# SinOncology/BreakID

Measured on AMD Instinct MI355X. Metric: M reads/s clustered+split-scanned, higher is better.
Workload: dtype int32/u8 (+f64 sd replay)

## Files before the change

### breakid_amd/abi.py

```python
import ctypes as C

import numpy as np

BK_OK = 0
BK_ERR_ARG, BK_ERR_HIP, BK_ERR_NO_DEVICE, BK_ERR_UNSORTED, BK_ERR_CIGAR, BK_ERR_IO, BK_ERR_LIMIT, BK_ERR_COLLISION = -1, -2, -3, -4, -5, -6, -7, -8
BK_MEM_HOST, BK_MEM_DEVICE = 0, 1
STAGE_SCAN, STAGE_ISO, STAGE_CLUSTERED, STAGE_SPLITS, STAGE_CLUSTERS, STAGE_GROUP_KEYS = range(6)

PAIR = np.dtype([("x", "<u4"), ("y", "<u4"), ("p1_pos", "<u4"), ("p2_pos", "<u4"), ("p1_tid", "<i4"),
                 ("p2_tid", "<i4"), ("p1_flag", "<u2"), ("p2_flag", "<u2"), ("p1_mapq", "u1"), ("p2_mapq", "u1"),
                 ("p1_rev", "u1"), ("p2_rev", "u1"), ("rec", "<u8"), ("id", "<u4"), ("cluster", "<i4"),
                 ("group", "<u4"), ("reserved", "<u4")])
SPLIT = np.dtype([("rec", "<u8"), ("tid", "<i4"), ("pos", "<i4"), ("endpos", "<i4"), ("reserved", "<u4"), ("qhash", "<u8"),
                  ("prim_chr", "<i4"), ("sec_chr", "<i4"), ("prim_start", "<u4"), ("prim_end", "<u4"),
                  ("prim_bp", "<u4"), ("sec_start", "<u4"), ("sec_end", "<u4"), ("sec_bp", "<u4"),
                  ("prim_cigar", "<u8"), ("sec_cigar", "<u8"), ("flags", "<u4"), ("qcheck", "<u4")])
CLUSTER = np.dtype([("group", "<u4"), ("id", "<i4"), ("p1_tid", "<i4"), ("p2_tid", "<i4"), ("p1_mean", "<u4"),
                    ("p2_mean", "<u4"), ("p1_min", "<u4"), ("p1_max", "<u4"), ("p2_min", "<u4"), ("p2_max", "<u4"),
                    ("p1_exact", "<u4"), ("p2_exact", "<i4"), ("n_drp", "<u4"), ("n_sr", "<u4"), ("depth1", "<u4"),
                    ("depth2", "<u4"), ("type_mask", "<u4"), ("flags", "<u4")])
GROUP_KEY = np.dtype([("p1_tid", "<i4"), ("p2_tid", "<i4")])
NORMAL_SUPPORT = np.dtype([("n_drp", "<u4"), ("n_sr", "<u4"), ("depth1", "<u4"), ("depth2", "<u4")])
REF_SUPPORT = np.dtype([("ref_pairs1", "<u4"), ("ref_pairs2", "<u4"), ("ref_reads1", "<u4"), ("ref_reads2", "<u4")])
JUNCTION = np.dtype([("pairs", "<u4", (4,)), ("splits", "<u4", (4,)), ("mapq_sum1", "<u8"), ("mapq_sum2", "<u8")])
assert JUNCTION.itemsize == 48
CLIP_LEFT, CLIP_RIGHT = 0, 1
CLIP_SUPPORT = np.dtype([("at", "<u4", (2, 2)), ("peak_pos", "<u4", (2, 2)), ("peak_n", "<u4", (2, 2)), ("events", "<u4", (2, 2))])
assert CLIP_SUPPORT.itemsize == 64
EV_PAIR, EV_SPLIT = 1, 2
EVIDENCE = np.dtype([("rec", "<u8"), ("qhash", "<u8"), ("qcheck", "<u4"), ("call", "<u4"), ("tid1", "<i4"), ("pos1", "<u4"), ("tid2", "<i4"),
                     ("pos2", "<u4"), ("flag1", "<u2"), ("flag2", "<u2"), ("mapq1", "u1"), ("mapq2", "u1"), ("kind", "u1"), ("sides", "u1")])
READ_KEY = np.dtype([("qhash", "<u8"), ("qcheck", "<u4"), ("tag", "<u4")])
assert EVIDENCE.itemsize == 48 and READ_KEY.itemsize == 16
assert PAIR.itemsize == 56 and SPLIT.itemsize == 88 and CLUSTER.itemsize == 72 and NORMAL_SUPPORT.itemsize == 16 and REF_SUPPORT.itemsize == 16

STAGE_DTYPE = {STAGE_SCAN: PAIR, STAGE_ISO: PAIR, STAGE_CLUSTERED: PAIR, STAGE_SPLITS: SPLIT,
               STAGE_CLUSTERS: CLUSTER, STAGE_GROUP_KEYS: GROUP_KEY}


class Soa(C.Structure):
    _fields_ = [("n", C.c_uint64), ("tid", C.c_void_p), ("pos", C.c_void_p), ("mtid", C.c_void_p),
                ("mpos", C.c_void_p), ("isize", C.c_void_p), ("flag", C.c_void_p), ("mapq", C.c_void_p),
                ("qhash", C.c_void_p), ("cigar_off", C.c_void_p), ("cigar", C.c_void_p),
                ("aux_off", C.c_void_p), ("aux", C.c_void_p), ("n_cigar_words", C.c_uint64),
                ("n_aux_bytes", C.c_uint64), ("qcheck", C.c_void_p), ("side", C.c_void_p)]


class Regions(C.Structure):
    _fields_ = [("tid", C.c_void_p), ("beg", C.c_void_p), ("end", C.c_void_p), ("n", C.c_uint64)]


SOA_COLS = [("tid", np.int32), ("pos", np.int32), ("mtid", np.int32), ("mpos", np.int32), ("isize", np.int32),
            ("flag", np.uint16), ("mapq", np.uint8), ("qhash", np.uint64), ("cigar_off", np.uint32),
            ("cigar", np.uint32), ("aux_off", np.uint32), ("aux", np.uint8)]


SOA_COLS_ALL = SOA_COLS + [("qcheck", np.uint32)]


def soa_from_numpy(cols) -> Soa:
    s = Soa()
    s.n = len(cols["tid"])
    for name, dt in SOA_COLS:
        a = cols[name]
        assert a.dtype == dt and a.flags["C_CONTIGUOUS"], name
        setattr(s, name, a.ctypes.data if a.size else 0)
    assert len(cols["cigar_off"]) == s.n + 1 and len(cols["aux_off"]) == s.n + 1
    s.n_cigar_words = int(cols["cigar_off"][-1]) if s.n else 0
    s.n_aux_bytes = int(cols["aux_off"][-1]) if s.n else 0
    q = cols.get("qcheck")
    if q is not None and s.n:
        assert q.dtype == np.uint32 and q.flags["C_CONTIGUOUS"] and len(q) == s.n
        s.qcheck = q.ctypes.data
    return s


def fetch_array(lib, handle, fn, stage):
    data = C.c_void_p()
    count = C.c_uint64()
    goff = C.POINTER(C.c_uint64)()
    ng = C.c_uint32()
    rc = fn(handle, stage, C.byref(data), C.byref(count), C.byref(goff), C.byref(ng))
    if rc != 0:
        raise RuntimeError("fetch(stage=%d) failed rc=%d" % (stage, rc))
    dt = STAGE_DTYPE[stage]
    n = count.value
    if n:
        buf = (C.c_char * (n * dt.itemsize)).from_address(data.value)
        arr = np.frombuffer(buf, dtype=dt, count=n).copy()
    else:
        arr = np.zeros(0, dt)
    off = None
    if ng.value or bool(goff):
        off = np.ctypeslib.as_array(goff, shape=(ng.value + 1,)).copy() if bool(goff) else None
    return arr, off


class ShardStats(C.Structure):
    _fields_ = [("isize_sum", C.c_uint64), ("isize_n", C.c_uint64), ("sumsq", C.c_double), ("vmax", C.c_uint32),
                ("max_span", C.c_uint32), ("n_cand", C.c_uint64), ("n_split", C.c_uint64)]


BUF_CANDIDATES, BUF_TUPLES, BUF_CLUSTERS = 0, 1, 2


def device_ptrs(cols):
    p = {k: cols[k].data_ptr() for k, _ in SOA_COLS}
    if "qcheck" in cols:
        p["qcheck"] = cols["qcheck"].data_ptr()
    if "side" in cols:
        p["side"] = cols["side"].data_ptr()
    return p
```

### breakid_amd/capi.py

```python
from __future__ import annotations

import ctypes as C
import math
import os
import subprocess

import numpy as np

from . import abi

_HERE = os.path.dirname(os.path.abspath(__file__))
LIB_PATH = os.path.join(_HERE, "libbreakid_hip.so")
_LIB = None


class BreakIDError(RuntimeError):
    def __init__(self, code, msg):
        super().__init__("libbreakid_hip error %d: %s" % (code, msg))
        self.code = code


def build(verbose=False):
    cmd = ["make", "-C", os.path.join(_HERE, "csrc"), "-j8"]
    r = subprocess.run(cmd, capture_output=not verbose, text=True)
    if r.returncode != 0:
        raise RuntimeError("building libbreakid_hip.so failed:\n" + (r.stdout or "")[-4000:] + (r.stderr or "")[-4000:])


EXPORTS = ["bk_init", "bk_prepare_process", "bk_free", "bk_last_error", "bk_set_stream", "bk_sync", "bk_get_stream", "bk_upload_records", "bk_exclude_regions", "bk_isize_stats",
           "bk_discordant_pairs", "bk_mask_and_cluster", "bk_split_evidence", "bk_cluster_summary",
           "bk_split_breakpoints", "bk_normal_support", "bk_ref_support", "bk_genotype_call", "bk_clip_support", "bk_base_depth", "bk_clip_rescue", "bk_junctions", "bk_junction_sides", "bk_vcf_breakend_alt", "bk_evidence", "bk_run", "bk_fetch", "bk_timing", "bk_timing_enable", "bk_timing_touched", "bk_group_stats", "bk_qname_hash", "bk_qname_check",
           "bk_bam_open", "bk_bam_header", "bk_bam_decode", "bk_bam_close", "bk_bam_extract", "bk_bam_names_free", "bk_bam_decode_device", "bk_bam_decode_device_part", "bk_bam_decode_device_ctx", "bk_bam_dev_free", "bk_feed_release_caches", "bk_debug_bgzf_inflate", "bk_debug_std_sort", "bk_sort_forms", "bk_debug_ahc", "bk_debug_points", "bk_debug_cigar", "bk_debug_vote", "bk_debug_region", "bk_shard_begin", "bk_shard_get_stats", "bk_shard_set_stats",
           "bk_shard_sd_local", "bk_shard_sd_finish", "bk_shard_buffer", "bk_shard_set_buffer", "bk_shard_group_sizes",
           "bk_shard_own_groups", "bk_shard_route_candidates", "bk_shard_group_keys", "bk_shard_route_pairs", "bk_shard_group_pairs", "bk_shard_bp_cov", "bk_shard_bp_vote", "bk_shard_bp_vote_slice", "bk_shard_bp_set_voted", "bk_shard_bp_depth", "bk_shard_bp_finish"]


def lib():
    global _LIB
    if _LIB is None:
        if not os.path.exists(LIB_PATH):
            raise BreakIDError(abi.BK_ERR_NO_DEVICE, "libbreakid_hip.so is not built (run __graft_entry__.build()); "
                                                     "there is no CPU fallback")
        try:
            import torch
        except Exception:
            pass
        L = C.CDLL(LIB_PATH)
        vp, u64p, dp = C.c_void_p, C.POINTER(C.c_uint64), C.POINTER(C.c_double)
        L.bk_init.argtypes = [C.c_int, vp, C.POINTER(C.c_char_p), C.c_int, C.POINTER(vp)]
        L.bk_free.argtypes = [vp]
        L.bk_last_error.restype = C.c_char_p
        L.bk_last_error.argtypes = [vp]
        L.bk_set_stream.argtypes = [vp, vp]
        L.bk_sync.argtypes = [vp]
        L.bk_upload_records.argtypes = [vp, C.POINTER(abi.Soa), C.c_int]
        L.bk_exclude_regions.argtypes = [vp, C.POINTER(abi.Regions), u64p]
        L.bk_isize_stats.argtypes = [vp, dp, dp]
        L.bk_discordant_pairs.argtypes = [vp, C.c_int, C.c_double, u64p, C.POINTER(C.c_uint32)]
        L.bk_mask_and_cluster.argtypes = [vp, C.c_double, C.c_int, u64p]
        L.bk_split_evidence.argtypes = [vp, u64p]
        L.bk_cluster_summary.argtypes = [vp, C.c_double, u64p]
        L.bk_split_breakpoints.argtypes = [vp, C.c_double, u64p]
        L.bk_run.argtypes = [vp, C.c_int, C.c_int, dp, u64p]
        L.bk_normal_support.argtypes = [vp, vp, C.c_double, C.POINTER(vp), u64p]
        L.bk_ref_support.argtypes = [vp, vp, C.c_int, C.c_int, C.c_double, C.POINTER(vp), u64p]
        L.bk_genotype_call.argtypes = [C.c_uint32, C.c_uint32, C.POINTER(C.c_uint8), C.POINTER(C.c_uint8), C.POINTER(C.c_float)]
        L.bk_clip_support.argtypes = [vp, vp, C.c_int, C.c_int, C.c_double, C.POINTER(vp), u64p]
        L.bk_base_depth.argtypes = [vp, vp, vp, C.c_uint64, C.POINTER(vp)]
        L.bk_clip_rescue.argtypes = [vp, vp, vp, C.c_uint32] + [C.POINTER(C.c_uint32)] * 4
        L.bk_junctions.argtypes = [vp, C.POINTER(vp), u64p]
        L.bk_junction_sides.argtypes = [vp, C.POINTER(C.c_uint8), C.POINTER(C.c_uint8), C.POINTER(C.c_uint8)]
        L.bk_vcf_breakend_alt.argtypes = [C.c_char, C.c_int, C.c_char_p, C.c_uint32, C.c_int, C.c_char_p, C.c_size_t]
        L.bk_evidence.argtypes = [vp, C.POINTER(vp), u64p, C.POINTER(C.POINTER(C.c_uint64))]
        L.bk_fetch.argtypes = [vp, C.c_int, C.POINTER(vp), u64p, C.POINTER(C.POINTER(C.c_uint64)), C.POINTER(C.c_uint32)]
        L.bk_timing.argtypes = [vp, C.POINTER(C.POINTER(C.c_char_p)), C.POINTER(C.POINTER(C.c_float)),
                                C.POINTER(C.POINTER(C.c_uint64)), C.POINTER(C.c_int)]
        L.bk_timing_enable.argtypes = [vp, C.c_int]
        L.bk_timing_touched.argtypes = [vp, C.POINTER(C.POINTER(C.c_uint64)), C.POINTER(C.c_int)]
        L.bk_debug_std_sort.argtypes = [vp, vp, vp, C.c_uint32, vp]
        L.bk_sort_forms.argtypes = [vp, u64p]
        L.bk_debug_ahc.argtypes = [vp, vp, vp, C.c_uint32, C.c_double, vp, vp, C.POINTER(C.c_uint32)]
        L.bk_debug_points.argtypes = [vp, C.c_int, vp, vp, C.c_uint32, C.c_double, vp, vp, C.POINTER(C.c_uint32)]
        L.bk_debug_cigar.argtypes = [vp, C.c_uint32, vp, vp, vp, vp, vp, vp, vp]
        L.bk_debug_vote.argtypes = [vp, vp, C.c_uint32, vp, C.c_uint32, C.c_int32, C.c_int32, vp]
        L.bk_debug_region.argtypes = [vp, C.c_int32, C.c_uint32, C.c_uint32, C.c_uint64, vp, C.c_uint32, C.POINTER(C.c_uint32), C.POINTER(C.c_uint32),
                                      C.POINTER(C.c_uint32)]
        L.bk_shard_begin.argtypes = [vp, C.c_uint64, C.c_int]
        L.bk_shard_get_stats.argtypes = [vp, C.POINTER(abi.ShardStats)]
        L.bk_shard_set_stats.argtypes = [vp, C.POINTER(abi.ShardStats)]
        L.bk_shard_sd_local.argtypes = [vp, u64p, C.POINTER(vp), u64p]
        L.bk_shard_sd_finish.argtypes = [vp, vp, C.c_uint64, C.c_uint64, dp, dp]
        L.bk_shard_buffer.argtypes = [vp, C.c_int, C.POINTER(vp), u64p, C.POINTER(C.c_uint32)]
        L.bk_shard_set_buffer.argtypes = [vp, C.c_int, vp, C.c_uint64]
        L.bk_shard_group_sizes.argtypes = [vp, C.POINTER(C.POINTER(C.c_uint64)), C.POINTER(C.c_uint32)]
        L.bk_shard_own_groups.argtypes = [vp, vp, C.c_uint32]
        L.bk_shard_route_candidates.argtypes = [vp, C.c_uint32, C.POINTER(vp), C.POINTER(C.POINTER(C.c_uint64))]
        L.bk_shard_group_keys.argtypes = [vp, C.POINTER(C.POINTER(C.c_uint32)), C.POINTER(C.c_uint32)]
        L.bk_shard_route_pairs.argtypes = [vp, vp, C.c_uint32, C.c_uint32, C.POINTER(vp), C.POINTER(C.POINTER(C.c_uint64))]
        L.bk_shard_group_pairs.argtypes = [vp, vp, C.c_uint64, vp, C.c_uint32]
        L.bk_shard_bp_cov.argtypes = [vp, C.c_double, C.POINTER(vp), u64p]
        L.bk_shard_bp_vote.argtypes = [vp, C.c_double, vp]
        L.bk_shard_bp_vote_slice.argtypes = [vp, C.c_double, vp, C.c_uint64, C.c_uint64, C.POINTER(vp), C.POINTER(vp)]
        L.bk_shard_bp_set_voted.argtypes = [vp, vp]
        L.bk_shard_bp_depth.argtypes = [vp, C.POINTER(vp), u64p]
        L.bk_shard_bp_finish.argtypes = [vp, vp]
        L.bk_qname_hash.restype = C.c_uint64
        L.bk_qname_hash.argtypes = [C.c_char_p, C.c_size_t]
        L.bk_qname_check.restype = C.c_uint32
        L.bk_qname_check.argtypes = [C.c_char_p, C.c_size_t]
        L.bk_bam_open.argtypes = [C.c_char_p, C.POINTER(vp), C.c_char_p, C.c_size_t]
        L.bk_bam_header.argtypes = [vp, C.POINTER(C.c_int), C.POINTER(C.POINTER(C.c_char_p)), C.POINTER(C.POINTER(C.c_uint32))]
        L.bk_bam_decode.argtypes = [vp, C.POINTER(abi.Soa), C.c_char_p, C.c_size_t]
        L.bk_bam_close.argtypes = [vp]
        L.bk_bam_extract.argtypes = [C.c_char_p, C.c_char_p, vp, C.c_uint64, C.POINTER(C.c_char_p), C.c_uint64, C.POINTER(vp), u64p, C.c_char_p, C.c_size_t]
        L.bk_bam_names_free.argtypes = [vp]
        L.bk_bam_names_free.restype = None
        L.bk_bam_decode_device.argtypes = [C.c_char_p, C.c_int, C.POINTER(vp), C.POINTER(abi.Soa), C.POINTER(C.c_int), C.POINTER(C.POINTER(C.c_char_p)),
                                           C.POINTER(C.POINTER(C.c_uint32)), C.c_char_p, C.c_size_t]
        L.bk_bam_decode_device_part.argtypes = [C.c_char_p, C.c_int, C.c_int, C.c_int, C.POINTER(vp), C.POINTER(abi.Soa), C.POINTER(C.c_int), C.POINTER(C.POINTER(C.c_char_p)),
                                           C.POINTER(C.POINTER(C.c_uint32)), C.c_char_p, C.c_size_t]
        L.bk_bam_dev_free.argtypes = [vp]
        L.bk_feed_release_caches.argtypes = []
        L.bk_feed_release_caches.restype = None
        L.bk_bam_decode_device_ctx.argtypes = [C.c_char_p, C.c_int, C.c_int, C.POINTER(vp), C.POINTER(vp), C.POINTER(C.c_int), C.POINTER(C.POINTER(C.c_char_p)),
                                               C.POINTER(C.POINTER(C.c_uint32)), C.c_char_p, C.c_size_t]
        L.bk_debug_bgzf_inflate.argtypes = [vp, C.c_uint64, vp, C.c_uint64, C.POINTER(C.c_uint64), C.POINTER(C.c_float), C.c_char_p, C.c_size_t]
        _LIB = L
    return _LIB


MULTI_LIB_PATH = os.path.join(_HERE, "libbreakid_rccl.so")
_MULTI = None
TRANSPORT_AUTO, TRANSPORT_RCCL, TRANSPORT_LOCAL = 0, 1, 2


def multi_lib():
    global _MULTI
    if _MULTI is None:
        lib()
        if not os.path.exists(MULTI_LIB_PATH):
            raise BreakIDError(abi.BK_ERR_NO_DEVICE, "libbreakid_rccl.so is not built (run __graft_entry__.build())")
        M = C.CDLL(MULTI_LIB_PATH)
        vp, dp = C.c_void_p, C.POINTER(C.c_double)
        M.bk_multi_run.argtypes = [C.POINTER(abi.Soa), vp, C.POINTER(C.c_char_p), C.c_int, C.c_int, C.c_int, C.c_int, C.c_int, dp, C.POINTER(C.c_uint64), C.POINTER(vp),
                                   C.c_char_p, C.c_size_t]
        M.bk_multi_stats.argtypes = [vp, dp, dp, C.POINTER(vp), C.POINTER(C.c_uint32)]
        M.bk_multi_free.argtypes = [vp]
        M.bk_multi_free.restype = None
        _MULTI = M
    return _MULTI


def multi_run(contigs, cols, n_gpus, transport=TRANSPORT_LOCAL, qual=20, fast=True):
    M = multi_lib()
    qc = cols.get("qcheck")
    cols = {k: np.ascontiguousarray(cols[k], dtype=dt) for k, dt in abi.SOA_COLS}
    if qc is not None:
        cols["qcheck"] = np.ascontiguousarray(qc, dtype=np.uint32)
    for k in ("cigar", "aux"):
        if cols[k].size == 0:
            cols[k] = np.zeros(1, cols[k].dtype)
    soa = abi.soa_from_numpy(cols)
    lens = np.asarray([l for _, l in contigs], dtype=np.uint32)
    names = (C.c_char_p * len(contigs))(*[n.encode() for n, _ in contigs])
    w, ncl, h = C.c_double(), C.c_uint64(), C.c_void_p()
    err = C.create_string_buffer(512)
    rc = M.bk_multi_run(C.byref(soa), lens.ctypes.data, names, len(contigs), int(n_gpus), int(transport), int(qual), int(fast), C.byref(w), C.byref(ncl), C.byref(h), err, 512)
    if rc != 0:
        raise BreakIDError(rc, err.value.decode())
    try:
        mean, sd = C.c_double(), C.c_double()
        rc = M.bk_multi_stats(h, C.byref(mean), C.byref(sd), None, None)
        if rc != 0:
            raise BreakIDError(rc, "bk_multi_stats")
        L = lib()
        clusters, _ = abi.fetch_array(L, h, lambda hh, st, d, c, g, ng: L.bk_fetch(hh, st, d, c, g, ng), abi.STAGE_CLUSTERS)
        return {"w": w.value, "n_clustered": ncl.value, "mean": mean.value, "sd": sd.value, "clusters": clusters}
    finally:
        M.bk_multi_free(h)


def w_from(mean, sd):
    times = 2
    return times * math.sqrt(times) * (mean + 3 * sd)


def genotype_call(alt, ref):
    gt, gq, vaf = C.c_uint8(), C.c_uint8(), C.c_float()
    rc = lib().bk_genotype_call(int(alt), int(ref), C.byref(gt), C.byref(gq), C.byref(vaf))
    if rc != 0:
        raise BreakIDError(rc, "bk_genotype_call")
    return gt.value, gq.value, np.float32(vaf.value)


def junction_sides(row):
    a = np.zeros(1, abi.JUNCTION)
    a[0] = row
    r1, r2, src = C.c_uint8(), C.c_uint8(), C.c_uint8()
    rc = lib().bk_junction_sides(a.ctypes.data, C.byref(r1), C.byref(r2), C.byref(src))
    if rc != 0:
        raise BreakIDError(rc, "bk_junction_sides")
    return r1.value, r2.value, src.value


def clip_rescue(cluster, junction, clip, min_support=3):
    c, j, s = np.zeros(1, abi.CLUSTER), np.zeros(1, abi.JUNCTION), np.zeros(1, abi.CLIP_SUPPORT)
    c[0], j[0], s[0] = cluster, junction, clip
    out = [C.c_uint32() for _ in range(4)]
    rc = lib().bk_clip_rescue(c.ctypes.data, j.ctypes.data, s.ctypes.data, int(min_support), *[C.byref(o) for o in out])
    if rc < 0:
        raise BreakIDError(rc, "bk_clip_rescue")
    return tuple(o.value for o in out) if rc == 1 else None


def vcf_breakend_alt(ref_base, own_right, mate_chr, mate_pos, mate_right, cap=None):
    chrom = mate_chr.encode()
    if cap is None:
        cap = len(chrom) + 32
    buf = C.create_string_buffer(max(int(cap), 1))
    rc = lib().bk_vcf_breakend_alt(ref_base.encode(), int(bool(own_right)), chrom, int(mate_pos), int(bool(mate_right)), buf, int(cap))
    if rc != 0:
        raise BreakIDError(rc, "bk_vcf_breakend_alt")
    return buf.value.decode()


class Context:

    def __init__(self, contigs, device=0):
        self.L = lib()
        self.contigs = list(contigs)
        lens = np.asarray([l for _, l in contigs], dtype=np.uint32)
        names = (C.c_char_p * len(contigs))(*[n.encode() for n, _ in contigs])
        h = C.c_void_p()
        rc = self.L.bk_init(device, lens.ctypes.data, names, len(contigs), C.byref(h))
        if rc != 0:
            raise BreakIDError(rc, (self.L.bk_last_error(None) or b"").decode())
        self.h = h
        self._keep = None

    def close(self):
        if self.h:
            self.L.bk_free(self.h)
            self.h = None

    def __del__(self):
        try:
            self.close()
        except Exception:
            pass

    def _check(self, rc):
        if rc != 0:
            raise BreakIDError(rc, (self.L.bk_last_error(self.h) or b"").decode())

    def set_stream(self, hip_stream_handle):
        self._check(self.L.bk_set_stream(self.h, C.c_void_p(hip_stream_handle)))

    def sync(self):
        self._check(self.L.bk_sync(self.h))

    def upload(self, cols):
        qc = cols.get("qcheck")
        cols = {k: np.ascontiguousarray(cols[k], dtype=dt) for k, dt in abi.SOA_COLS}
        if qc is not None:
            cols["qcheck"] = np.ascontiguousarray(qc, dtype=np.uint32)
        for k in ("cigar", "aux"):
            if cols[k].size == 0:
                cols[k] = np.zeros(1, cols[k].dtype)
        soa = abi.soa_from_numpy(cols)
        self._keep = (cols, soa)
        self._check(self.L.bk_upload_records(self.h, C.byref(soa), abi.BK_MEM_HOST))

    def attach_device_table(self, table):
        self._keep = table
        self._check(self.L.bk_upload_records(self.h, C.byref(table.soa), abi.BK_MEM_DEVICE))

    def upload_soa(self, handle):
        self._keep = handle
        self._check(self.L.bk_upload_records(self.h, C.byref(handle.soa), abi.BK_MEM_HOST))

    def attach_device(self, ptrs, n, n_cigar_words, n_aux_bytes):
        s = abi.Soa()
        s.n = n
        for name, _ in abi.SOA_COLS:
            setattr(s, name, ptrs[name])
        if ptrs.get("qcheck"):
            s.qcheck = ptrs["qcheck"]
        if ptrs.get("side"):
            s.side = ptrs["side"]
        s.n_cigar_words = n_cigar_words
        s.n_aux_bytes = n_aux_bytes
        self._keep = (ptrs, s)
        self._check(self.L.bk_upload_records(self.h, C.byref(s), abi.BK_MEM_DEVICE))

    def exclude_regions(self, tid, beg, end):
        tid, beg, end = (np.ascontiguousarray(a, np.int32).reshape(-1) for a in (tid, beg, end))
        if not len(tid) == len(beg) == len(end):
            raise ValueError("exclude_regions: tid, beg and end differ in length")
        r = abi.Regions(tid.ctypes.data, beg.ctypes.data, end.ctypes.data, len(tid))
        n = C.c_uint64()
        self._check(self.L.bk_exclude_regions(self.h, C.byref(r), C.byref(n)))
        return n.value

    def isize_stats(self):
        m, s = C.c_double(), C.c_double()
        self._check(self.L.bk_isize_stats(self.h, C.byref(m), C.byref(s)))
        return m.value, s.value

    def shard_begin(self, rec_base, qual=20):
        self._check(self.L.bk_shard_begin(self.h, int(rec_base), int(qual)))

    def shard_get_stats(self):
        st = abi.ShardStats()
        self._check(self.L.bk_shard_get_stats(self.h, C.byref(st)))
        return st

    def shard_set_stats(self, st):
        self._check(self.L.bk_shard_set_stats(self.h, C.byref(st)))

    def shard_sd_local(self):
        lt, ex, nex = C.c_uint64(), C.c_void_p(), C.c_uint64()
        self._check(self.L.bk_shard_sd_local(self.h, C.byref(lt), C.byref(ex), C.byref(nex)))
        return lt.value, ex.value, nex.value

    def shard_sd_finish(self, all_ex_ptr, n_all, l_grand):
        m, s = C.c_double(), C.c_double()
        self._check(self.L.bk_shard_sd_finish(self.h, C.c_void_p(all_ex_ptr or 0), int(n_all), int(l_grand), C.byref(m), C.byref(s)))
        return m.value, s.value

    def discordant_pairs(self, qual, w):
        n, g = C.c_uint64(), C.c_uint32()
        self._check(self.L.bk_discordant_pairs(self.h, qual, w, C.byref(n), C.byref(g)))
        return n.value, g.value

    def mask_and_cluster(self, w, fast):
        n = C.c_uint64()
        self._check(self.L.bk_mask_and_cluster(self.h, w, int(fast), C.byref(n)))
        return n.value

    def split_evidence(self):
        n = C.c_uint64()
        self._check(self.L.bk_split_evidence(self.h, C.byref(n)))
        return n.value

    def cluster_summary(self, w):
        n = C.c_uint64()
        self._check(self.L.bk_cluster_summary(self.h, w, C.byref(n)))
        return n.value

    def split_breakpoints(self, w, count=True):
        n = C.c_uint64()
        self._check(self.L.bk_split_breakpoints(self.h, w, C.byref(n) if count else None))
        return n.value

    def normal_support(self, normal, w):
        data, n = C.c_void_p(), C.c_uint64()
        self._check(self.L.bk_normal_support(self.h, normal.h, w, C.byref(data), C.byref(n)))
        if not n.value:
            return np.zeros(0, abi.NORMAL_SUPPORT)
        buf = (C.c_char * (n.value * abi.NORMAL_SUPPORT.itemsize)).from_address(data.value)
        return np.frombuffer(buf, dtype=abi.NORMAL_SUPPORT, count=n.value).copy()

    def junctions(self):
        data, n = C.c_void_p(), C.c_uint64()
        self._check(self.L.bk_junctions(self.h, C.byref(data), C.byref(n)))
        if not n.value:
            return np.zeros(0, abi.JUNCTION)
        buf = (C.c_char * (n.value * abi.JUNCTION.itemsize)).from_address(data.value)
        return np.frombuffer(buf, dtype=abi.JUNCTION, count=n.value).copy()

    def evidence(self):
        data, n, off = C.c_void_p(), C.c_uint64(), C.POINTER(C.c_uint64)()
        self._check(self.L.bk_evidence(self.h, C.byref(data), C.byref(n), C.byref(off)))
        rows = np.zeros(0, abi.EVIDENCE)
        if n.value:
            buf = (C.c_char * (n.value * abi.EVIDENCE.itemsize)).from_address(data.value)
            rows = np.frombuffer(buf, dtype=abi.EVIDENCE, count=n.value).copy()
        d2, ncl = C.c_void_p(), C.c_uint64()
        self._check(self.L.bk_fetch(self.h, abi.STAGE_CLUSTERS, C.byref(d2), C.byref(ncl), None, None))
        return rows, np.ctypeslib.as_array(off, shape=(ncl.value + 1,)).copy()

    def ref_support(self, records, mapq_min, anchor, w):
        data, n = C.c_void_p(), C.c_uint64()
        self._check(self.L.bk_ref_support(self.h, records.h, int(mapq_min), int(anchor), w, C.byref(data), C.byref(n)))
        if not n.value:
            return np.zeros(0, abi.REF_SUPPORT)
        buf = (C.c_char * (n.value * abi.REF_SUPPORT.itemsize)).from_address(data.value)
        return np.frombuffer(buf, dtype=abi.REF_SUPPORT, count=n.value).copy()

    def clip_support(self, records, mapq_min, min_clip, w):
        data, n = C.c_void_p(), C.c_uint64()
        self._check(self.L.bk_clip_support(self.h, records.h, int(mapq_min), int(min_clip), w, C.byref(data), C.byref(n)))
        if not n.value:
            return np.zeros(0, abi.CLIP_SUPPORT)
        buf = (C.c_char * (n.value * abi.CLIP_SUPPORT.itemsize)).from_address(data.value)
        return np.frombuffer(buf, dtype=abi.CLIP_SUPPORT, count=n.value).copy()

    def base_depth(self, tid, pos):
        tid = np.ascontiguousarray(tid, np.int32)
        pos = np.ascontiguousarray(pos, np.uint32)
        assert tid.shape == pos.shape and tid.ndim == 1
        data = C.c_void_p()
        self._check(self.L.bk_base_depth(self.h, tid.ctypes.data, pos.ctypes.data, len(tid), C.byref(data)))
        if not len(tid):
            return np.zeros(0, np.uint32)
        return np.ctypeslib.as_array(C.cast(data, C.POINTER(C.c_uint32)), shape=(len(tid),)).copy()

    def run(self, qual=20, fast=True):
        w, n = C.c_double(), C.c_uint64()
        self._check(self.L.bk_run(self.h, qual, int(fast), C.byref(w), C.byref(n)))
        return w.value, n.value

    def fetch(self, stage):
        def fn(h, st, d, c, g, ng):
            return self.L.bk_fetch(h, st, d, c, g, ng)
        try:
            return abi.fetch_array(self.L, self.h, fn, stage)
        except RuntimeError:
            self._check(-1 if not self.L.bk_last_error(self.h) else abi.BK_ERR_ARG)
            raise

    def debug_std_sort(self, key, group_off):
        key = np.ascontiguousarray(key, np.uint32)
        group_off = np.ascontiguousarray(group_off, np.uint64)
        perm = np.zeros(len(key), np.uint32)
        self._check(self.L.bk_debug_std_sort(self.h, key.ctypes.data, group_off.ctypes.data, len(group_off) - 1, perm.ctypes.data))
        return perm

    def sort_forms(self):
        out = (C.c_uint64 * 3)()
        self._check(self.L.bk_sort_forms(self.h, out))
        return tuple(int(v) for v in out)

    def debug_ahc(self, x, y, w):
        x = np.ascontiguousarray(x, np.uint32)
        y = np.ascontiguousarray(y, np.uint32)
        n = len(x)
        idx = np.zeros(max(n, 1), np.uint32)
        cl = np.zeros(max(n, 1), np.int32)
        m = C.c_uint32()
        self._check(self.L.bk_debug_ahc(self.h, x.ctypes.data, y.ctypes.data, n, float(w), idx.ctypes.data, cl.ctypes.data, C.byref(m)))
        return idx[:m.value].copy(), cl[:m.value].copy()

    def debug_points(self, mode, x, y, w):
        x = np.ascontiguousarray(x, np.uint32)
        y = np.ascontiguousarray(y, np.uint32)
        n = len(x)
        idx = np.zeros(max(n, 1), np.uint32)
        cl = np.zeros(max(n, 1), np.int32)
        m = C.c_uint32()
        self._check(self.L.bk_debug_points(self.h, {"mask": 0, "iso": 1, "fast": 2}[mode], x.ctypes.data, y.ctypes.data, n, float(w), idx.ctypes.data,
                                           cl.ctypes.data, C.byref(m)))
        return idx[:m.value].copy(), cl[:m.value].copy()

    def debug_cigar(self, rows):
        kind = np.asarray([1 if r[0] == "b" else 0 for r in rows], np.uint8)
        c1 = bytearray()
        o1 = [0]
        for r in rows:
            while r[0] == "b" and len(c1) % 4:
                c1 += b"\0"
                o1[-1] = len(c1)
            c1 += np.asarray(r[1], np.uint32).tobytes() if r[0] == "b" else r[1].encode()
            o1.append(len(c1))
        c2 = bytearray()
        o2 = [0]
        for r in rows:
            c2 += r[2].encode()
            o2.append(len(c2))
        o1a, o2a = np.asarray(o1, np.uint32), np.asarray(o2, np.uint32)
        b1 = np.frombuffer(bytes(c1) + b"\0" * 16, np.uint8)
        b2 = np.frombuffer(bytes(c2) + b"\0" * 16, np.uint8)
        e = np.asarray([r[3] for r in rows], np.int32)
        out = np.zeros((len(rows), 6), np.int32)
        self._check(self.L.bk_debug_cigar(self.h, len(rows), kind.ctypes.data, o1a.ctypes.data, b1.ctypes.data, o2a.ctypes.data, b2.ctypes.data, e.ctypes.data,
                                          out.ctypes.data))
        return out

    def debug_vote(self, s1, s2, p1_tid, p2_tid):
        s1 = np.ascontiguousarray(s1, abi.SPLIT)
        s2 = np.ascontiguousarray(s2, abi.SPLIT)
        out = np.zeros(3, np.int32)
        self._check(self.L.bk_debug_vote(self.h, s1.ctypes.data, len(s1), s2.ctypes.data, len(s2), p1_tid, p2_tid, out.ctypes.data))
        return tuple(int(v) for v in out)

    def debug_region(self, tid, start, end, depth_pos, cap=4096):
        out = np.zeros(cap, abi.SPLIT)
        n, cov, depth = C.c_uint32(), C.c_uint32(), C.c_uint32()
        self._check(self.L.bk_debug_region(self.h, tid, start, end, depth_pos, out.ctypes.data, cap, C.byref(n), C.byref(cov), C.byref(depth)))
        return out[:min(n.value, cap)].copy(), n.value, cov.value, depth.value

    def timing_enable(self, on=True):
        self._check(self.L.bk_timing_enable(self.h, int(on)))

    def timing(self):
        names = C.POINTER(C.c_char_p)()
        ms = C.POINTER(C.c_float)()
        by = C.POINTER(C.c_uint64)()
        n = C.c_int()
        self._check(self.L.bk_timing(self.h, C.byref(names), C.byref(ms), C.byref(by), C.byref(n)))
        return [(names[i].decode(), float(ms[i]), int(by[i])) for i in range(n.value)]

    def timing_touched(self):
        t = C.POINTER(C.c_uint64)()
        n = C.c_int()
        self._check(self.L.bk_timing_touched(self.h, C.byref(t), C.byref(n)))
        return [int(t[i]) for i in range(n.value)]


class DeviceBamTable:

    def __init__(self, L, h, soa, contigs):
        self.L, self.h, self.soa, self.contigs = L, h, soa, contigs

    def close(self):
        if self.h:
            self.L.bk_bam_dev_free(self.h)
            self.h = None


def decode_bam_device(path, device=0):
    L = lib()
    h = C.c_void_p()
    err = C.create_string_buffer(512)
    s = abi.Soa()
    nt = C.c_int()
    names = C.POINTER(C.c_char_p)()
    lens = C.POINTER(C.c_uint32)()
    rc = L.bk_bam_decode_device(path.encode(), device, C.byref(h), C.byref(s), C.byref(nt), C.byref(names), C.byref(lens), err, 512)
    if rc != 0:
        raise BreakIDError(rc, err.value.decode())
    contigs = [(names[i].decode(), int(lens[i])) for i in range(nt.value)]
    return DeviceBamTable(L, h, s, contigs)


def decode_bam_device_part(path, part, parts, device=0):
    L = lib()
    h = C.c_void_p()
    err = C.create_string_buffer(512)
    s = abi.Soa()
    nt = C.c_int()
    names = C.POINTER(C.c_char_p)()
    lens = C.POINTER(C.c_uint32)()
    rc = L.bk_bam_decode_device_part(path.encode(), device, part, parts, C.byref(h), C.byref(s), C.byref(nt), C.byref(names), C.byref(lens), err, 512)
    if rc != 0:
        raise BreakIDError(rc, err.value.decode())
    contigs = [(names[i].decode(), int(lens[i])) for i in range(nt.value)]
    return DeviceBamTable(L, h, s, contigs)


def decode_bam_device_ctx(path, qual=20, device=0):
    L = lib()
    hb, hc = C.c_void_p(), C.c_void_p()
    err = C.create_string_buffer(512)
    nt = C.c_int()
    names = C.POINTER(C.c_char_p)()
    lens = C.POINTER(C.c_uint32)()
    rc = L.bk_bam_decode_device_ctx(path.encode(), device, qual, C.byref(hb), C.byref(hc), C.byref(nt), C.byref(names), C.byref(lens), err, 512)
    if rc != 0:
        raise BreakIDError(rc, err.value.decode())
    contigs = [(names[i].decode(), int(lens[i])) for i in range(nt.value)]
    ctx = Context.__new__(Context)
    ctx.L, ctx.contigs, ctx.h = L, contigs, hc
    table = DeviceBamTable(L, hb, None, contigs)
    ctx._keep = table
    return ctx, table


def bam_extract(in_bam, out_bam, keys, tags):
    keys = np.ascontiguousarray(keys, abi.READ_KEY)
    tag_arr = (C.c_char_p * max(len(tags), 1))(*[t.encode() for t in tags])
    names, n = C.c_void_p(), C.c_uint64()
    err = C.create_string_buffer(512)
    L = lib()
    rc = L.bk_bam_extract(os.fsencode(in_bam), None if out_bam is None else os.fsencode(out_bam), keys.ctypes.data if len(keys) else None, len(keys),
                          tag_arr if len(tags) else None, len(tags), C.byref(names), C.byref(n), err, 512)
    if rc != 0:
        raise BreakIDError(rc, err.value.decode())
    try:
        out, p = [], names.value
        for _ in range(len(keys)):
            t = C.string_at(p)
            out.append(t.decode())
            p += len(t) + 1
    finally:
        L.bk_bam_names_free(names)
    return out, n.value


class BamTable:

    def __init__(self, L, h, soa):
        self.L, self.h, self.soa = L, h, soa
        n = soa.n
        self.nbytes = n * (4 * 5 + 2 + 1 + 8) + (n + 1) * 8 + soa.n_cigar_words * 4 + soa.n_aux_bytes

    def close(self):
        if self.h:
            self.L.bk_bam_close(self.h)
            self.h = None


def decode_bam(path, keep=False):
    L = lib()
    h = C.c_void_p()
    err = C.create_string_buffer(512)
    rc = L.bk_bam_open(path.encode(), C.byref(h), err, 512)
    if rc != 0:
        raise BreakIDError(rc, err.value.decode())
    try:
        nt = C.c_int()
        names = C.POINTER(C.c_char_p)()
        lens = C.POINTER(C.c_uint32)()
        L.bk_bam_header(h, C.byref(nt), C.byref(names), C.byref(lens))
        contigs = [(names[i].decode(), int(lens[i])) for i in range(nt.value)]
        s = abi.Soa()
        rc = L.bk_bam_decode(h, C.byref(s), err, 512)
        if rc != 0:
            raise BreakIDError(rc, err.value.decode())
        n = s.n
        sizes = {"cigar_off": n + 1, "aux_off": n + 1, "cigar": max(1, s.n_cigar_words), "aux": max(1, s.n_aux_bytes)}
        cols = {}
        for name, dt in abi.SOA_COLS_ALL:
            cnt = sizes.get(name, n)
            ptr = getattr(s, name)
            if cnt == 0 or not ptr:
                cols[name] = np.zeros(0, dt)
                continue
            buf = (C.c_char * (cnt * np.dtype(dt).itemsize)).from_address(ptr)
            cols[name] = np.frombuffer(buf, dtype=dt, count=cnt).copy()
        cols["cigar"] = cols["cigar"][: s.n_cigar_words]
        cols["aux"] = cols["aux"][: s.n_aux_bytes]
        if keep:
            t = BamTable(L, h, s)
            h = None
            return contigs, cols, t
        return contigs, cols
    finally:
        if h:
            L.bk_bam_close(h)
```

### breakid_amd/csrc/api.hip

```cpp
#include <algorithm>
#include <cmath>
#include <limits>
#include <cstring>
#include <numeric>

#include "bk_common.h"
#include "prims.h"
#include "stream.h"
#include "join.h"
#include "cluster.h"
#include "bp.h"
#include "normal.h"
#include "genotype.h"
#include "clip.h"
#include "junction.h"
#include "evidence.h"
#include "exclude.h"
#include "ahc.h"
#include "lanes.h"
#include "bgzf_gpu.h"

namespace
{
thread_local std::string g_init_error;

uint64_t fnv64(const std::string &s)
{
  uint64_t h = 0xCBF29CE484222325ull;
  for (unsigned char c : s)
  {
    h ^= c;
    h *= 0x100000001B3ull;
  }
  return h;
}
std::string chrom_id_to_name(int tid)
{
  if (tid == 23) return "chrY";
  if (tid == 22) return "chrX";
  if (tid >= 0 && tid < 22) return "chr" + std::to_string(tid + 1);
  return "";
}

struct StageTimer
{
  std::string name;
  hipEvent_t a = nullptr, b = nullptr;
  uint64_t bytes = 0;
  uint64_t touched = 0;
};
}

struct bk_ctx
{
  int device = 0;
  hipStream_t st = nullptr;
  bool own_stream = true;
  std::string err;
  int nt = 0;
  std::vector<uint32_t> tlen;
  std::vector<std::string> tname;
  std::vector<int32_t> hdr_id_host;
  DevBuf d_tprefix, d_nhash, d_nid, d_own, d_hdr;
  NameTableDev names{};

  bk_soa rec{};
  DevBuf col[13];
  DevBuf d_side;
  DevBuf xcol[13];
  bool have_records = false;
  bool streamed = false;

  DevBuf d_counters, d_sd, d_cand, d_split_raw, d_split, d_sa_list;
  StreamCounters hc{};
  SdState hsd{};
  bool stream_done = false, splits_sorted = false;
  int mapq_min = 20;
  int stream_mapq = -1;
  uint64_t cand_cap = 0, split_cap = 0, sa_cap = 0;
  uint64_t rec_base = 0;
  std::vector<uint64_t> route_counts;
  JoinBufs jb2;
  const Cand *ext_cand = nullptr;
  const bk_split *ext_split = nullptr;
  bk_cluster *ext_clusters = nullptr;
  std::vector<uint8_t> own_groups;
  const Cand *cand_ptr() const { return ext_cand ? ext_cand : d_cand.get<Cand>(); }
  const bk_split *split_raw_ptr() const { return ext_split ? ext_split : d_split_raw.get<bk_split>(); }
  bk_cluster *clusters_ptr() const { return ext_clusters ? ext_clusters : d_clusters.get<bk_cluster>(); }
  SdBufs sdb;
  double mean = 0, sd = 0;
  bool stats_done = false;

  JoinBufs jb;
  JoinResult jr;
  std::vector<uint32_t> gkey_host, glex_host, lex_to_num;
  std::vector<uint64_t> gstart_host;
  DevBuf d_glex, d_lex_to_num;

  ClusterStage stage;
  bool clustered = false;

  BpBufs bb;
  DevBuf d_clusters;
  uint64_t n_clusters = 0;

  bool joined = false, bp_done = false, shard = false;
  double join_w = 0;
  NormalBufs nb;
  std::vector<struct bk_normal_support> f_normal;
  RefBufs rb;
  std::vector<struct bk_ref_support> f_ref;
  ClipBufs cb;
  std::vector<struct bk_clip_support> f_clip;
  DevBuf d_bd_tid, d_bd_pos, d_bd_out, d_bd_samp;
  std::vector<uint32_t> f_base_depth;
  JunctionBufs jnb;
  std::vector<struct bk_junction> f_junction;
  bool summary_map = false;
  EvidenceBufs evb;
  std::vector<struct bk_evidence> f_evidence;
  std::vector<uint64_t> f_ev_off;

  std::vector<bk_pair> f_pairs[3];
  std::vector<uint64_t> f_off[3];
  std::vector<bk_split> f_splits;
  std::vector<bk_cluster> f_clusters;
  std::vector<int32_t> f_gkeys;
  std::vector<bk_group_stat> f_gstats;

  bool timing = false;
  std::vector<StageTimer> timers;
  Timing tout;

  void tick(const char *name, uint64_t bytes, bool begin, uint64_t touched = 0)
  {
    if (!timing) return;
    if (begin)
    {
      StageTimer t;
      t.name = name;
      t.bytes = bytes;
      t.touched = touched;
      HIP_CHECK(hipEventCreate(&t.a));
      HIP_CHECK(hipEventCreate(&t.b));
      HIP_CHECK(hipEventRecord(t.a, st));
      timers.push_back(t);
    }
    else
      HIP_CHECK(hipEventRecord(timers.back().b, st));
  }
};

static RecView rec_view(const bk_ctx *ctx)
{
  RecView r;
  r.n = ctx->rec.n;
  r.tid = ctx->rec.tid; r.pos = ctx->rec.pos; r.flag = ctx->rec.flag; r.mapq = ctx->rec.mapq;
  r.cigar_off = ctx->rec.cigar_off; r.cigar = ctx->rec.cigar;
  r.isize = ctx->rec.isize; r.aux_off = ctx->rec.aux_off;
  return r;
}

namespace
{
struct Scope
{
  bk_ctx *c;
  Scope(bk_ctx *c, const char *name, uint64_t bytes = 0, uint64_t touched = 0) : c(c) { c->tick(name, bytes, true, touched); }
  ~Scope()
  {
    try
    {
      c->tick("", 0, false);
    }
    catch (...)
    {
    }
  }
};

template <class F> int guarded(bk_ctx *ctx, F &&f)
{
  if (!ctx) return BK_ERR_ARG;
  try
  {
    HIP_CHECK(hipSetDevice(ctx->device));
    f();
    return BK_OK;
  }
  catch (const bk_error &e)
  {
    ctx->err = e.msg;
    return e.code;
  }
  catch (const std::exception &e)
  {
    ctx->err = e.what();
    return BK_ERR_HIP;
  }
}

template <class T> void rows_to_host(bk_ctx *ctx, const T *d_rows, uint64_t n, std::vector<T> &out)
{
  out.resize(n);
  if (n) HIP_CHECK(hipMemcpyAsync(out.data(), d_rows, n * sizeof(T), hipMemcpyDeviceToHost, ctx->st));
  HIP_CHECK(hipStreamSynchronize(ctx->st));
}

void build_name_tables(bk_ctx *c)
{
  const int nt = c->nt;
  std::map<std::string, int> ids;
  for (int i = 0; i < nt; ++i)
    if (!ids.count(c->tname[i])) ids[c->tname[i]] = i;
  if (!ids.count("")) ids[""] = nt;
  if (!ids.count("*")) ids["*"] = nt + 1;
  for (int t = 0; t < 24; ++t)
  {
    std::string s = chrom_id_to_name(t);
    if (!ids.count(s)) ids[s] = nt + 2 + t;
  }
  uint32_t cap = 64;
  while (cap < ids.size() * 4) cap <<= 1;
  std::vector<uint64_t> hash(cap, 0);
  std::vector<int32_t> idv(cap, -1);
  for (auto &kv : ids)
  {
    uint64_t h = fnv64(kv.first);
    if (h == 0) h = 1;
    uint32_t slot = (uint32_t) h & (cap - 1);
    while (hash[slot] != 0 && hash[slot] != h) slot = (slot + 1) & (cap - 1);
    if (hash[slot] == 0)
    {
      hash[slot] = h;
      idv[slot] = kv.second;
    }
  }
  std::vector<int32_t> own(std::max(nt, 1));
  for (int t = 0; t < nt; ++t) own[t] = ids[chrom_id_to_name(t)];
  c->hdr_id_host.assign(nt + 1, 0);
  c->hdr_id_host[0] = ids["*"];
  for (int t = 0; t < nt; ++t) c->hdr_id_host[t + 1] = ids[c->tname[t]];
  std::vector<uint32_t> prefix(nt + 1, 0);
  for (int t = 0; t < nt; ++t) prefix[t + 1] = prefix[t] + c->tlen[t];
  HIP_CHECK(hipMemcpy(c->d_nhash.as<uint64_t>(cap), hash.data(), cap * 8, hipMemcpyHostToDevice));
  HIP_CHECK(hipMemcpy(c->d_nid.as<int32_t>(cap), idv.data(), cap * 4, hipMemcpyHostToDevice));
  HIP_CHECK(hipMemcpy(c->d_own.as<int32_t>(own.size()), own.data(), own.size() * 4, hipMemcpyHostToDevice));
  HIP_CHECK(hipMemcpy(c->d_hdr.as<int32_t>(nt + 1), c->hdr_id_host.data(), (nt + 1) * 4, hipMemcpyHostToDevice));
  HIP_CHECK(hipMemcpy(c->d_tprefix.as<uint32_t>(nt + 1), prefix.data(), (nt + 1) * 4, hipMemcpyHostToDevice));
  c->names.hash = c->d_nhash.get<uint64_t>();
  c->names.id = c->d_nid.get<int32_t>();
  c->names.mask = cap - 1;
  c->names.own_id = c->d_own.get<int32_t>();
  c->names.n_targets = nt;
  c->names.empty_id = ids[""];
}

std::string rname(const bk_ctx *c, int tid) { return tid < 0 ? "*" : c->tname[tid]; }

StreamArgs stream_args(bk_ctx *c, uint64_t n)
{
  StreamArgs a{};
  a.n = n;
  a.q_begin = 0;
  a.rec_base = c->rec_base;
  a.tid = c->rec.tid; a.pos = c->rec.pos; a.mtid = c->rec.mtid; a.mpos = c->rec.mpos; a.isize = c->rec.isize;
  a.flag = c->rec.flag; a.mapq = c->rec.mapq; a.qhash = c->rec.qhash; a.qcheck = c->rec.qcheck;
  static const bool no_side = getenv("BREAKID_NO_SIDE") != nullptr;
  a.side = no_side && c->rec.qhash ? nullptr : c->rec.side;
  a.cigar_off = c->rec.cigar_off; a.cigar = c->rec.cigar; a.aux_off = c->rec.aux_off; a.aux = c->rec.aux;
  a.mapq_min = c->mapq_min;
  a.names = c->names;
  a.counters = c->d_counters.get<StreamCounters>();
  a.sd = c->d_sd.get<SdState>();
  a.cand = c->d_cand.get<Cand>();
  a.cand_cap = c->cand_cap;
  a.split = c->d_split_raw.get<bk_split>();
  a.split_cap = c->split_cap;
  a.sa_list = c->d_sa_list.get<uint32_t>();
  a.sa_cap = c->sa_cap;
  return a;
}
void stream_prepare(bk_ctx *c, uint64_t n_expected)
{
  c->streamed = true;
  c->cand_cap = std::max<uint64_t>(c->cand_cap, std::max<uint64_t>(1u << 16, n_expected / 8 + 1024));
  c->split_cap = std::max<uint64_t>(c->split_cap, std::max<uint64_t>(1u << 14, n_expected / 32 + 1024));
  c->sa_cap = std::max<uint64_t>(c->sa_cap, std::max<uint64_t>(1u << 14, n_expected / 16 + 1024));
  StreamCounters *dc = c->d_counters.as<StreamCounters>(1);
  SdState *dsd = c->d_sd.as<SdState>(1);
  HIP_CHECK(hipMemsetAsync(dc, 0, sizeof(StreamCounters), c->st));
  HIP_CHECK(hipMemsetAsync(dsd, 0, sizeof(SdState), c->st));
  (void) c->d_cand.as<Cand>(c->cand_cap);
  (void) c->d_split_raw.as<bk_split>(c->split_cap);
  (void) c->d_sa_list.as<uint32_t>(c->sa_cap);
}
bool stream_finish(bk_ctx *c)
{
  HIP_CHECK(hipMemcpyAsync(&c->hc, c->d_counters.get<StreamCounters>(), sizeof(StreamCounters), hipMemcpyDeviceToHost, c->st));
  HIP_CHECK(hipMemcpyAsync(&c->hsd, c->d_sd.get<SdState>(), sizeof(SdState), hipMemcpyDeviceToHost, c->st));
  HIP_CHECK(hipStreamSynchronize(c->st));
  if (c->hc.n_cand > c->cand_cap || c->hc.n_sa > c->sa_cap)
  {
    c->cand_cap = std::max<uint64_t>(c->cand_cap, c->hc.n_cand + 1024);
    c->sa_cap = std::max<uint64_t>(c->sa_cap, c->hc.n_sa + 1024);
    return false;
  }
  return true;
}
void stream_rare_path(bk_ctx *c)
{
  const uint64_t n = c->rec.n;
  if (c->timing && !c->timers.empty())
  {
    c->timers.back().bytes += 32ull * c->hc.n_cand + 4ull * c->hc.n_sa;
    c->timers.back().touched = 23ull * n + 4ull * c->rec.n_cigar_words + (c->rec.qcheck ? 60ull : 56ull) * c->hc.n_cand + 4ull * c->hc.n_sa;
  }
  if (c->hc.unsorted) throw bk_error(BK_ERR_UNSORTED, "records are not coordinate sorted (the reference requires an indexed, sorted BAM)");
  if (c->hc.n_sa > c->split_cap)
  {
    c->split_cap = c->hc.n_sa + 1024;
    (void) c->d_split_raw.as<bk_split>(c->split_cap);
  }
  StreamArgs a = stream_args(c, n);
  {
    Scope s(c, "k_split_records", c->rec.n_aux_bytes + 4ull * c->hc.n_sa);
    launch_split_records(a, c->hc.n_sa, c->st);
  }
  HIP_CHECK(hipMemcpyAsync(&c->hc, c->d_counters.get<StreamCounters>(), sizeof(StreamCounters), hipMemcpyDeviceToHost, c->st));
  HIP_CHECK(hipStreamSynchronize(c->st));
  if (c->timing && !c->timers.empty())
  {
    c->timers.back().bytes += 48ull * c->hc.n_split;
    c->timers.back().touched = c->timers.back().bytes + 40ull * c->hc.n_sa + 32ull * c->hc.n_split;
  }
  c->stream_done = true;
  c->stream_mapq = c->mapq_min;
  c->splits_sorted = false;
  c->stats_done = false;
}

void run_stream(bk_ctx *c)
{
  if (!c->have_records) throw bk_error(BK_ERR_ARG, "no records uploaded");
  const uint64_t n = c->rec.n;
  for (int attempt = 0; attempt < 3; ++attempt)
  {
    stream_prepare(c, n);
    {
      Scope s(c, "k_stream", 39ull * n + 4ull * c->rec.n_cigar_words);
      launch_stream(stream_args(c, n), c->st);
    }
    if (stream_finish(c)) break;
    if (c->timing && !c->timers.empty()) c->timers.pop_back();
    if (attempt == 2) throw bk_error(BK_ERR_LIMIT, "stream pass: output capacity");
  }
  stream_rare_path(c);
}

void ensure_splits_sorted(bk_ctx *c)
{
  if (c->splits_sorted) return;
  Scope s(c, "split_sort");
  bk_split *sorted = c->d_split.as<bk_split>(c->hc.n_split + 1);
  int bits = 0;
  if (!c->ext_split && c->rec_base == 0)
  {
    bits = 1;
    while (bits < 32 && (1ull << bits) < c->rec.n) ++bits;
  }
  sort_splits(const_cast<bk_split *>(c->split_raw_ptr()), c->hc.n_split, sorted, c->bb, c->st, bits);
  c->splits_sorted = true;
}
}

extern "C" {

void bk_prepare_process()
{
  static std::once_flag once;
  std::call_once(once, [] {
    const char *q = getenv("GPU_MAX_HW_QUEUES");
    stage_set_hw_queues(q ? atoi(q) : 4);
  });
}

int bk_init(int device, const uint32_t *target_len, const char *const *target_name, int n_targets, bk_ctx **out)
{
  {
    bk_prepare_process();
  }
  if (!out || n_targets < 0 || (n_targets && (!target_len || !target_name)))
  {
    g_init_error = "bk_init: bad arguments";
    return BK_ERR_ARG;
  }
  *out = nullptr;
  int ndev = 0;
  if (hipGetDeviceCount(&ndev) != hipSuccess || ndev <= 0 || device < 0 || device >= ndev)
  {
    g_init_error = "bk_init: no HIP device " + std::to_string(device) + " (this library has no CPU path)";
    return BK_ERR_NO_DEVICE;
  }
  hipDeviceProp_t prop;
  if (hipGetDeviceProperties(&prop, device) != hipSuccess || std::string(prop.gcnArchName).rfind("gfx950", 0) != 0)
  {
    g_init_error = std::string("bk_init: device is not gfx950 (") + prop.gcnArchName + "); kernels are built for MI355X only";
    return BK_ERR_NO_DEVICE;
  }
  bk_ctx *c = new bk_ctx();
  c->device = device;
  c->nt = n_targets;
  for (int i = 0; i < n_targets; ++i)
  {
    c->tlen.push_back(target_len[i]);
    c->tname.push_back(target_name[i]);
  }
  int rc = guarded(c, [&] {
    HIP_CHECK(hipStreamCreate(&c->st));
    build_name_tables(c);
  });
  if (rc != BK_OK)
  {
    g_init_error = c->err;
    delete c;
    return rc;
  }
  *out = c;
  return BK_OK;
}

void bk_free(bk_ctx *ctx)
{
  if (!ctx) return;
  (void) hipSetDevice(ctx->device);
  (void) hipStreamSynchronize(ctx->st);
  for (auto &t : ctx->timers)
  {
    if (t.a) (void) hipEventDestroy(t.a);
    if (t.b) (void) hipEventDestroy(t.b);
  }
  if (ctx->own_stream && ctx->st) (void) hipStreamDestroy(ctx->st);
  delete ctx;
}

const char *bk_last_error(const bk_ctx *ctx) { return ctx ? ctx->err.c_str() : g_init_error.c_str(); }

int bk_set_stream(bk_ctx *ctx, void *hip_stream)
{
  return guarded(ctx, [&] {
    if (ctx->own_stream && ctx->st) HIP_CHECK(hipStreamDestroy(ctx->st));
    ctx->st = (hipStream_t) hip_stream;
    ctx->own_stream = false;
  });
}
int bk_get_stream(bk_ctx *ctx, void **hip_stream)
{
  return guarded(ctx, [&] {
    if (!hip_stream) throw bk_error(BK_ERR_ARG, "bk_get_stream: null output");
    *hip_stream = (void *) ctx->st;
  });
}
int bk_sync(bk_ctx *ctx)
{
  return guarded(ctx, [&] { HIP_CHECK(hipStreamSynchronize(ctx->st)); });
}

int bk_upload_records(bk_ctx *ctx, const bk_soa *s, int mem_space)
{
  return guarded(ctx, [&] {
    if (!s) throw bk_error(BK_ERR_ARG, "bk_upload_records: null table");
    if (s->n > 0xFFFFFFF0ull) throw bk_error(BK_ERR_LIMIT, "more than 2^32 records in one context (shard across GPUs)");
    ctx->stream_done = ctx->stats_done = ctx->clustered = false;
    ctx->joined = ctx->bp_done = ctx->shard = false;
    ctx->ext_cand = nullptr;
    ctx->ext_split = nullptr;
    ctx->ext_clusters = nullptr;
    ctx->own_groups.clear();
    ctx->rec_base = 0;
    ctx->streamed = false;
    if (mem_space == BK_MEM_DEVICE)
    {
      hipPointerAttribute_t at;
      if (s->n && s->tid && hipPointerGetAttributes(&at, s->tid) == hipSuccess && at.type == hipMemoryTypeDevice && at.device != ctx->device)
        throw bk_error(BK_ERR_ARG, "bk_upload_records: BK_MEM_DEVICE table lives on device " + std::to_string(at.device) + ", context on device " +
                                       std::to_string(ctx->device));
      (void) hipGetLastError();
      for (const void *p : {(const void *) s->tid, (const void *) s->pos, (const void *) s->isize, (const void *) s->flag, (const void *) s->mapq, (const void *) s->cigar_off,
                            (const void *) s->aux_off})
        if (s->n && ((uintptr_t) p & 15u)) throw bk_error(BK_ERR_ARG, "bk_upload_records: BK_MEM_DEVICE columns must be 16-byte aligned");
      if (s->n && s->side && ((uintptr_t) s->side & 15u)) throw bk_error(BK_ERR_ARG, "bk_upload_records: BK_MEM_DEVICE side rows must be 16-byte aligned");
      ctx->rec = *s;
    }
    else
    {
      const uint64_t n = s->n;
      const void *src[13] = {s->tid, s->pos, s->mtid, s->mpos, s->isize, s->flag, s->mapq, s->qhash, s->cigar_off, s->cigar, s->aux_off, s->aux, s->qcheck};
      const size_t bytes[13] = {n * 4, n * 4, n * 4, n * 4, n * 4, n * 2, n, n * 8, (n + 1) * 4, s->n_cigar_words * 4, (n + 1) * 4, s->n_aux_bytes,
                                s->qcheck ? n * 4 : 0};
      void *dst[13];
      for (int k = 0; k < 13; ++k)
      {
        dst[k] = ctx->col[k].ensure(bytes[k] + 16);
        if (bytes[k]) HIP_CHECK(hipMemcpyAsync(dst[k], src[k], bytes[k], hipMemcpyHostToDevice, ctx->st));
      }
      HIP_CHECK(hipStreamSynchronize(ctx->st));
      bk_soa d = *s;
      d.tid = (const int32_t *) dst[0]; d.pos = (const int32_t *) dst[1]; d.mtid = (const int32_t *) dst[2]; d.mpos = (const int32_t *) dst[3];
      d.isize = (const int32_t *) dst[4]; d.flag = (const uint16_t *) dst[5]; d.mapq = (const uint8_t *) dst[6]; d.qhash = (const uint64_t *) dst[7];
      d.cigar_off = (const uint32_t *) dst[8]; d.cigar = (const uint32_t *) dst[9]; d.aux_off = (const uint32_t *) dst[10]; d.aux = (const uint8_t *) dst[11];
      d.qcheck = s->qcheck ? (const uint32_t *) dst[12] : nullptr;
      bk_side *side = ctx->d_side.as<bk_side>(n + 1);
      launch_make_side(d.qhash, d.mtid, d.mpos, d.qcheck, n, side, ctx->st);
      d.side = side;
      ctx->rec = d;
    }
    ctx->have_records = true;
  });
}

int bk_exclude_regions(bk_ctx *ctx, const bk_regions *r, uint64_t *n_removed)
{
  return guarded(ctx, [&] {
    if (!ctx->have_records || ctx->streamed || ctx->shard)
      throw bk_error(BK_ERR_ARG, "bk_exclude_regions: call it after bk_upload_records and before the stream pass (bk_isize_stats, bk_shard_begin, "
                                 "or a context of bk_bam_decode_device_ctx)");
    if (!r || (r->n && (!r->tid || !r->beg || !r->end))) throw bk_error(BK_ERR_ARG, "bk_exclude_regions: null interval list");
    const bk_soa &s = ctx->rec;
    if (s.n && (!s.tid || !s.pos || !s.mtid || !s.mpos || !s.isize || !s.flag || !s.mapq || !s.qhash || !s.cigar_off || !s.aux_off))
      throw bk_error(BK_ERR_ARG, "bk_exclude_regions: the table lacks a column");
    std::vector<std::vector<std::pair<int32_t, int32_t>>> by(ctx->nt);
    for (uint64_t k = 0; k < r->n; ++k)
    {
      const int32_t t = r->tid[k], b = r->beg[k], e = r->end[k];
      if (t < 0 || t >= ctx->nt || b < 0 || e <= b)
        throw bk_error(BK_ERR_ARG, "bk_exclude_regions: interval " + std::to_string(k) + " (tid " + std::to_string(t) + ", [" + std::to_string(b) + ", " +
                                       std::to_string(e) + ")): needs 0 <= tid < n_targets, 0 <= beg < end");
      by[t].emplace_back(b, e);
    }
    std::vector<uint32_t> off(ctx->nt + 1, 0);
    std::vector<int32_t> beg, end;
    for (int t = 0; t < ctx->nt; ++t)
    {
      auto &v = by[t];
      std::sort(v.begin(), v.end());
      for (auto &iv : v)
        if (beg.size() > off[t] && iv.first <= end.back())
          end.back() = std::max(end.back(), iv.second);
        else
        {
          beg.push_back(iv.first);
          end.push_back(iv.second);
        }
      off[t + 1] = (uint32_t) beg.size();
    }
    const bool owned = s.tid && s.tid == ctx->col[0].get<int32_t>();
    if (beg.empty() && owned)
    {
      if (n_removed) *n_removed = 0;
      return;
    }
    DevBuf d_off, d_beg, d_end;
    ExclRegions rg;
    rg.n_targets = ctx->nt;
    rg.off = d_off.as<uint32_t>(off.size());
    rg.beg = d_beg.as<int32_t>(beg.size() + 1);
    rg.end = d_end.as<int32_t>(end.size() + 1);
    HIP_CHECK(hipMemcpyAsync((void *) rg.off, off.data(), off.size() * 4, hipMemcpyHostToDevice, ctx->st));
    if (!beg.empty())
    {
      HIP_CHECK(hipMemcpyAsync((void *) rg.beg, beg.data(), beg.size() * 4, hipMemcpyHostToDevice, ctx->st));
      HIP_CHECK(hipMemcpyAsync((void *) rg.end, end.data(), end.size() * 4, hipMemcpyHostToDevice, ctx->st));
    }
    bk_soa out;
    const uint64_t n_before = s.n;
    exclude_compact(s, rg, ctx->xcol, out, ctx->st, [&](const char *name, uint64_t bytes, bool begin) { ctx->tick(name ? name : "", bytes, begin, bytes); });
    for (int k = 0; k < 13; ++k)
    {
      std::swap(ctx->col[k], ctx->xcol[k]);
      ctx->xcol[k].release();
    }
    {
      Scope sc(ctx, "make_side", (out.qcheck ? 56ull : 52ull) * out.n, (out.qcheck ? 56ull : 52ull) * out.n);
      bk_side *side = ctx->d_side.as<bk_side>(out.n + 1);
      launch_make_side(out.qhash, out.mtid, out.mpos, out.qcheck, out.n, side, ctx->st);
      out.side = side;
    }
    HIP_CHECK(hipStreamSynchronize(ctx->st));
    ctx->rec = out;
    if (n_removed) *n_removed = n_before - out.n;
  });
}

int bk_isize_stats(bk_ctx *ctx, double *mean, double *sd)
{
  return guarded(ctx, [&] {
    if (!ctx->stream_done) run_stream(ctx);
    if (!ctx->stats_done)
    {
      const double n = (double) ctx->hc.isize_n;
      const double m = (double) (long long) ctx->hc.isize_sum / n;
      ctx->mean = m;
      if (ctx->hc.isize_n == 0)
        ctx->sd = std::nan("");
      else
      {
        double sum_d = ctx->hsd.sumsq - 2.0 * m * (double) ctx->hc.isize_sum + n * m * m;
        if (!(sum_d > 0)) sum_d = 0;
        double da = (double) ctx->hsd.vmax - m, dmax = da * da + m * m;
        double bound = 2.0 * sum_d + 2.0 * n + 2.0 * dmax + 4.0;
        int k = std::ilogb(bound) + 1;
        double thr = k >= 51 ? 1.0e300 : std::ldexp(1.0, k - 53);
        {
          Scope s(ctx, "isize_sd", 0, 6ull * ctx->rec.n);
          launch_sd(ctx->rec.flag, ctx->rec.isize, ctx->rec.n, m, thr, ctx->d_sd.get<SdState>(), ctx->sdb, ctx->st);
        }
        HIP_CHECK(hipMemcpyAsync(&ctx->hsd, ctx->d_sd.get<SdState>(), sizeof(SdState), hipMemcpyDeviceToHost, ctx->st));
        HIP_CHECK(hipStreamSynchronize(ctx->st));
        ctx->sd = std::sqrt((double) ctx->hsd.t_final / n);
      }
      ctx->stats_done = true;
    }
    if (mean) *mean = ctx->mean;
    if (sd) *sd = ctx->sd;
  });
}

static void finish_groups(bk_ctx *ctx, const std::vector<uint32_t> *all_keys)
{
  const uint32_t ng = ctx->jr.n_groups;
  ctx->gkey_host.assign(ng, 0);
  ctx->gstart_host.assign(ng + 1, 0);
  if (ng)
  {
    HIP_CHECK(hipMemcpyAsync(ctx->gkey_host.data(), ctx->jr.gkey, ng * 4, hipMemcpyDeviceToHost, ctx->st));
    HIP_CHECK(hipMemcpyAsync(ctx->gstart_host.data(), ctx->jr.gstart, (ng + 1) * 8, hipMemcpyDeviceToHost, ctx->st));
    HIP_CHECK(hipStreamSynchronize(ctx->st));
  }
  auto key_name = [&](uint32_t k) {
    int t1 = (int) (k / (uint32_t) (ctx->nt + 1)) - 1, t2 = (int) (k % (uint32_t) (ctx->nt + 1)) - 1;
    return rname(ctx, t1) + "_" + rname(ctx, t2);
  };
  std::vector<std::string> keys(ng);
  for (uint32_t g = 0; g < ng; ++g) keys[g] = key_name(ctx->gkey_host[g]);
  ctx->lex_to_num.resize(ng);
  std::iota(ctx->lex_to_num.begin(), ctx->lex_to_num.end(), 0u);
  std::sort(ctx->lex_to_num.begin(), ctx->lex_to_num.end(), [&](uint32_t a, uint32_t b) { return keys[a] < keys[b]; });
  ctx->glex_host.assign(ng, 0);
  if (!all_keys)
    for (uint32_t l = 0; l < ng; ++l) ctx->glex_host[ctx->lex_to_num[l]] = l;
  else
  {
    std::vector<std::string> names;
    names.reserve(all_keys->size());
    for (uint32_t k : *all_keys) names.push_back(key_name(k));
    std::sort(names.begin(), names.end());
    names.erase(std::unique(names.begin(), names.end()), names.end());
    for (uint32_t g = 0; g < ng; ++g)
    {
      auto it = std::lower_bound(names.begin(), names.end(), keys[g]);
      if (it == names.end() || *it != keys[g]) throw bk_error(BK_ERR_ARG, "bk_shard_group_pairs: a local group is missing from the global key list");
      ctx->glex_host[g] = (uint32_t) (it - names.begin());
    }
  }
  uint32_t *dg = ctx->d_glex.as<uint32_t>((uint64_t) ng + 1), *dl = ctx->d_lex_to_num.as<uint32_t>((uint64_t) ng + 1);
  if (ng) HIP_CHECK(hipMemcpyAsync(dg, ctx->glex_host.data(), ng * 4, hipMemcpyHostToDevice, ctx->st));
  if (ng) HIP_CHECK(hipMemcpyAsync(dl, ctx->lex_to_num.data(), ng * 4, hipMemcpyHostToDevice, ctx->st));
  join_assign_ids(ctx->jr, dg, ctx->st);
}

int bk_discordant_pairs(bk_ctx *ctx, int mapq_min, double w, uint64_t *n_pairs, uint32_t *n_groups)
{
  return guarded(ctx, [&] {
    if (!ctx->stream_done || mapq_min != ctx->stream_mapq)
    {
      ctx->mapq_min = mapq_min;
      run_stream(ctx);
    }
    {
      Scope s(ctx, "mate_join");
      ctx->jb.rec_bits = -1;
      if (!ctx->ext_cand && ctx->rec_base == 0)
      {
        int bits = 1;
        while (bits < 32 && (1ull << bits) < ctx->rec.n) ++bits;
        ctx->jb.rec_bits = bits;
      }
      join_candidates(ctx->cand_ptr(), ctx->hc.n_cand, w, ctx->d_tprefix.get<uint32_t>(), ctx->nt, ctx->jb, ctx->st, ctx->jr);
    }
    finish_groups(ctx, nullptr);
    ctx->clustered = false;
    ctx->joined = true;
    ctx->bp_done = false;
    ctx->join_w = w;
    if (n_pairs) *n_pairs = ctx->jr.n_pairs;
    if (n_groups) *n_groups = ctx->jr.n_groups;
  });
}

int bk_mask_and_cluster(bk_ctx *ctx, double w, int fast, uint64_t *n_clustered)
{
  return guarded(ctx, [&] {
    const StageInput in{ctx->device, ctx->st, ctx->jr, ctx->gstart_host, ctx->own_groups,
                        [&](const char *name, const std::function<void()> &body) { Scope s(ctx, name); body(); }};
    ctx->summary_map = false;
    ctx->stage.run(in, w, fast);
    ctx->clustered = true;
    if (n_clustered) *n_clustered = ctx->stage.list.n;
  });
}

int bk_split_evidence(bk_ctx *ctx, uint64_t *n_tuples)
{
  return guarded(ctx, [&] {
    if (!ctx->stream_done) run_stream(ctx);
    ensure_splits_sorted(ctx);
    if (n_tuples) *n_tuples = ctx->hc.n_split;
  });
}

int bk_cluster_summary(bk_ctx *ctx, double w, uint64_t *n_clusters)
{
  return guarded(ctx, [&] {
    if (!ctx->clustered) throw bk_error(BK_ERR_ARG, "bk_cluster_summary: call bk_mask_and_cluster first");
    ctx->bp_done = false;
    if (ctx->stage.list.ng != ctx->jr.n_groups) throw bk_error(BK_ERR_HIP, "bk_cluster_summary: the clustered list and the join disagree on the groups (internal error)");
    Scope s(ctx, "cluster_summary");
    ctx->n_clusters = cluster_summary(ctx->jr.pairs, ctx->stage.list.idx.get<uint32_t>(), ctx->stage.list.gof.get<uint32_t>(), ctx->stage.d_cluster.get<uint32_t>(), ctx->stage.list.n,
                                      ctx->stage.list.ng, ctx->jr.gkey, ctx->d_glex.get<uint32_t>(), ctx->d_lex_to_num.get<uint32_t>(), ctx->nt, w, ctx->d_clusters, ctx->bb, ctx->st);
    ctx->summary_map = true;
    if (n_clusters) *n_clusters = ctx->n_clusters;
  });
}

int bk_split_breakpoints(bk_ctx *ctx, double w, uint64_t *n_valid)
{
  return guarded(ctx, [&] {
    ensure_splits_sorted(ctx);
    RecView r;
    r.n = ctx->rec.n;
    r.tid = ctx->rec.tid; r.pos = ctx->rec.pos; r.flag = ctx->rec.flag; r.mapq = ctx->rec.mapq;
    r.cigar_off = ctx->rec.cigar_off; r.cigar = ctx->rec.cigar;
    {
      Scope s(ctx, "split_breakpoints");
      split_breakpoints(r, ctx->d_split.get<bk_split>(), ctx->hc.n_split, ctx->clusters_ptr(), ctx->n_clusters, w, (int) ctx->hc.max_span,
                        ctx->d_hdr.get<int32_t>(), ctx->bb, ctx->st);
    }
    ctx->bp_done = true;
    if (n_valid) *n_valid = count_valid_clusters(ctx->clusters_ptr(), ctx->n_clusters, ctx->bb, ctx->st);
  });
}

static TupleTable tuple_table(const bk_ctx *ctx)
{
  return TupleTable{ctx->d_split.get<bk_split>(), ctx->hc.n_split, (int) ctx->hc.max_span, ctx->d_hdr.get<int32_t>(), ctx->names.own_id, ctx->nt, ctx->names.empty_id};
}
static JunctionPairs junction_pairs(const bk_ctx *ctx)
{
  JunctionPairs jp{};
  if (ctx->n_clusters)
  {
    jp.pairs = ctx->jr.pairs;
    jp.idx = ctx->stage.list.idx.get<uint32_t>();
    jp.gof = ctx->stage.list.gof.get<uint32_t>();
    jp.cl = ctx->stage.d_cluster.get<uint32_t>();
    jp.n = ctx->stage.list.n;
    jp.ng = ctx->stage.list.ng;
    jp.slotbase = ctx->bb.slotbase.get<uint32_t>();
    jp.keep = ctx->bb.keep.get<uint32_t>();
    jp.off = ctx->bb.off.get<uint32_t>();
  }
  return jp;
}
static void require_same_reference(const std::string &who, const char *role_a, const bk_ctx *a, const char *role_b, const bk_ctx *b)
{
  if (b->device != a->device)
    throw bk_error(BK_ERR_ARG, who + ": " + role_a + " (device " + std::to_string(a->device) + ") and " + role_b + " (device " + std::to_string(b->device) +
                                   ") contexts are on different devices");
  if (b != a && (b->nt != a->nt || b->tname != a->tname || b->tlen != a->tlen))
    throw bk_error(BK_ERR_ARG, who + ": " + role_a + " and " + role_b + " reference lists differ (names or lengths)");
}

int bk_normal_support(bk_ctx *tumor, bk_ctx *normal, double w, const struct bk_normal_support **out, uint64_t *count)
{
  if (!normal) return guarded(tumor, [&] { throw bk_error(BK_ERR_ARG, "bk_normal_support: null normal context"); });
  return guarded(tumor, [&] {
    if (!out || !count) throw bk_error(BK_ERR_ARG, "bk_normal_support: null output");
    if (tumor->shard || normal->shard) throw bk_error(BK_ERR_ARG, "bk_normal_support: sharded contexts (bk_shard_*) are not supported");
    if (!tumor->bp_done) throw bk_error(BK_ERR_ARG, "bk_normal_support: call bk_split_breakpoints on the tumour context first");
    if (!normal->stats_done || !normal->joined || !normal->splits_sorted)
      throw bk_error(BK_ERR_ARG, "bk_normal_support: call bk_isize_stats, bk_discordant_pairs and bk_split_evidence on the normal context first");
    if (tumor->join_w != w) throw bk_error(BK_ERR_ARG, "bk_normal_support: w is not the tumour's distance (its bk_discordant_pairs w)");
    if (normal->stream_mapq != tumor->stream_mapq || normal->join_w != w)
      throw bk_error(BK_ERR_ARG, "bk_normal_support: the normal's bk_discordant_pairs must use the tumour's mapq_min and w");
    require_same_reference("bk_normal_support", "tumour", tumor, "normal", normal);
    Scope s(tumor, "normal_support");
    HIP_CHECK(hipStreamSynchronize(normal->st));
    const NormalSide ns{normal->jr.pairs, normal->jr.n_pairs, tuple_table(normal), rec_view(normal)};
    const uint64_t ncl = tumor->n_clusters;
    struct bk_normal_support *d_res;
    normal_support(ns, tumor->clusters_ptr(), ncl, w, tumor->nb, tumor->st, &d_res);
    rows_to_host(tumor, d_res, ncl, tumor->f_normal);
    *out = tumor->f_normal.data();
    *count = ncl;
  });
}

int bk_ref_support(bk_ctx *calls, bk_ctx *records, int mapq_min, int anchor, double w, const struct bk_ref_support **out, uint64_t *count)
{
  if (!records) return guarded(calls, [&] { throw bk_error(BK_ERR_ARG, "bk_ref_support: null records context"); });
  return guarded(calls, [&] {
    if (!out || !count) throw bk_error(BK_ERR_ARG, "bk_ref_support: null output");
    if (calls->shard || records->shard) throw bk_error(BK_ERR_ARG, "bk_ref_support: sharded contexts (bk_shard_*) are not supported");
    if (!calls->bp_done) throw bk_error(BK_ERR_ARG, "bk_ref_support: call bk_split_breakpoints on the calls context first");
    if (!records->have_records || !records->stats_done) throw bk_error(BK_ERR_ARG, "bk_ref_support: call bk_isize_stats on the records context first");
    if (anchor < 0) throw bk_error(BK_ERR_ARG, "bk_ref_support: anchor must not be negative");
    if (mapq_min < 0) throw bk_error(BK_ERR_ARG, "bk_ref_support: mapq_min must not be negative");
    if (!(w >= 0.0 && w < 2147483648.0)) throw bk_error(BK_ERR_ARG, "bk_ref_support: w is out of range");
    require_same_reference("bk_ref_support", "calls", calls, "records", records);
    const bk_soa &t = records->rec;
    if (t.n && (!t.tid || !t.pos || !t.isize || !t.flag || !t.mapq || !t.cigar_off || !t.aux_off))
      throw bk_error(BK_ERR_ARG, "bk_ref_support: the record table lacks a column");
    const uint64_t ncl = calls->n_clusters;
    if (records != calls) HIP_CHECK(hipStreamSynchronize(records->st));
    struct bk_ref_support *d_res;
    RefStat *d_stat = nullptr;
    {
      Scope s(calls, "ref_support");
      ref_support(rec_view(records), (int) records->hc.max_span, calls->clusters_ptr(), ncl, mapq_min, anchor, w, calls->rb, calls->st, &d_res,
                  calls->timing ? &d_stat : nullptr);
    }
    std::vector<RefStat> stat(d_stat ? 2 * ncl : 0);
    if (!stat.empty()) HIP_CHECK(hipMemcpyAsync(stat.data(), d_stat, 2 * ncl * sizeof(RefStat), hipMemcpyDeviceToHost, calls->st));
    rows_to_host(calls, d_res, ncl, calls->f_ref);
    if (calls->timing && !calls->timers.empty())
    {
      uint64_t visited = 0, words = 0;
      for (const RefStat &x : stat)
      {
        visited += x.visited;
        words += x.words;
      }
      calls->timers.back().bytes = 19ull * visited;
      calls->timers.back().touched = 19ull * visited + 4ull * words + ncl * (2ull * sizeof(bk_cluster) + sizeof(struct bk_ref_support));
    }
    *out = calls->f_ref.data();
    *count = ncl;
  });
}

int bk_clip_support(bk_ctx *calls, bk_ctx *records, int mapq_min, int min_clip, double w, const struct bk_clip_support **out, uint64_t *count)
{
  if (!records) return guarded(calls, [&] { throw bk_error(BK_ERR_ARG, "bk_clip_support: null records context"); });
  return guarded(calls, [&] {
    if (!out || !count) throw bk_error(BK_ERR_ARG, "bk_clip_support: null output");
    if (calls->shard || records->shard) throw bk_error(BK_ERR_ARG, "bk_clip_support: sharded contexts (bk_shard_*) are not supported");
    if (!calls->bp_done) throw bk_error(BK_ERR_ARG, "bk_clip_support: call bk_split_breakpoints on the calls context first");
    if (!records->have_records || !records->stats_done) throw bk_error(BK_ERR_ARG, "bk_clip_support: call bk_isize_stats on the records context first");
    if (min_clip < 1) throw bk_error(BK_ERR_ARG, "bk_clip_support: min_clip must be at least 1");
    if (mapq_min < 0) throw bk_error(BK_ERR_ARG, "bk_clip_support: mapq_min must not be negative");
    if (!(w >= 0.0 && w < 2147483648.0)) throw bk_error(BK_ERR_ARG, "bk_clip_support: w is out of range");
    require_same_reference("bk_clip_support", "calls", calls, "records", records);
    const bk_soa &t = records->rec;
    if (t.n && (!t.tid || !t.pos || !t.flag || !t.mapq || !t.cigar_off || !t.aux_off)) throw bk_error(BK_ERR_ARG, "bk_clip_support: the record table lacks a column");
    const uint64_t ncl = calls->n_clusters;
    if (records != calls) HIP_CHECK(hipStreamSynchronize(records->st));
    struct bk_clip_support *d_res;
    ClipStat *d_stat = nullptr;
    {
      Scope s(calls, "clip_support");
      clip_support(rec_view(records), (int) records->hc.max_span, calls->clusters_ptr(), ncl, mapq_min, min_clip, w, calls->cb, calls->st, &d_res,
                   calls->timing ? &d_stat : nullptr);
    }
    std::vector<ClipStat> stat(d_stat ? 2 * ncl : 0);
    if (!stat.empty()) HIP_CHECK(hipMemcpyAsync(stat.data(), d_stat, 2 * ncl * sizeof(ClipStat), hipMemcpyDeviceToHost, calls->st));
    rows_to_host(calls, d_res, ncl, calls->f_clip);
    if (calls->timing && !calls->timers.empty())
    {
      uint64_t visited = 0, words = 0;
      for (const ClipStat &x : stat)
      {
        visited += x.visited;
        words += x.words;
      }
      calls->timers.back().bytes = 15ull * visited;
      calls->timers.back().touched = 15ull * visited + 4ull * words + ncl * (2ull * sizeof(bk_cluster) + sizeof(struct bk_clip_support));
    }
    *out = calls->f_clip.data();
    *count = ncl;
  });
}

int bk_base_depth(bk_ctx *records, const int32_t *tid, const uint32_t *pos, uint64_t n, const uint32_t **out)
{
  return guarded(records, [&] {
    if (!out || (n && (!tid || !pos))) throw bk_error(BK_ERR_ARG, "bk_base_depth: null argument");
    if (records->shard) throw bk_error(BK_ERR_ARG, "bk_base_depth: sharded contexts (bk_shard_*) are not supported");
    if (!records->have_records || !records->stats_done) throw bk_error(BK_ERR_ARG, "bk_base_depth: call bk_isize_stats first");
    const bk_soa &t = records->rec;
    if (t.n && (!t.tid || !t.pos || !t.flag || !t.mapq || !t.cigar_off)) throw bk_error(BK_ERR_ARG, "bk_base_depth: the record table lacks a column");
    records->f_base_depth.assign(n, 0u);
    if (n)
    {
      int32_t *d_tid = records->d_bd_tid.as<int32_t>(n);
      uint32_t *d_pos = records->d_bd_pos.as<uint32_t>(n), *d_out = records->d_bd_out.as<uint32_t>(n);
      HIP_CHECK(hipMemcpyAsync(d_tid, tid, n * 4, hipMemcpyHostToDevice, records->st));
      HIP_CHECK(hipMemcpyAsync(d_pos, pos, n * 4, hipMemcpyHostToDevice, records->st));
      {
        Scope s(records, "base_depth");
        base_depth_at(rec_view(records), d_tid, d_pos, n, (int) records->hc.max_span, records->d_bd_samp, records->st, d_out);
      }
      HIP_CHECK(hipMemcpyAsync(records->f_base_depth.data(), d_out, n * 4, hipMemcpyDeviceToHost, records->st));
      HIP_CHECK(hipStreamSynchronize(records->st));
    }
    *out = records->f_base_depth.data();
  });
}

int bk_genotype_call(uint32_t alt, uint32_t ref, uint8_t *gt, uint8_t *gq, float *vaf)
{
  if (!gt || !gq || !vaf) return BK_ERR_ARG;
  if ((uint64_t) alt + ref == 0)
  {
    *gt = 255;
    *gq = 0;
    *vaf = std::numeric_limits<float>::quiet_NaN();
    return BK_OK;
  }
  static const double c[3] = {-0x1.4d104d427de80p+0, -0x1.34413509f79ffp-2, -0x1.6cf9f8b075bd8p-6};
  const double k = (double) alt, r = (double) ref;
  double L[3];
  for (int g = 0; g < 3; ++g)
  {
    const double a = k * c[g], b = r * c[2 - g];
    L[g] = a + b;
  }
  int best = 0;
  for (int g = 1; g < 3; ++g)
    if (L[g] > L[best]) best = g;
  int second = -1;
  for (int g = 0; g < 3; ++g)
    if (g != best && (second < 0 || L[g] > L[second])) second = g;
  const double q = std::floor(10.0 * (L[best] - L[second]) + 0.5);
  *gt = (uint8_t) best;
  *gq = (uint8_t) (q < 99.0 ? q : 99.0);
  *vaf = (float) alt / (float) ((uint64_t) alt + ref);
  return BK_OK;
}

int bk_junctions(bk_ctx *ctx, const struct bk_junction **out, uint64_t *count)
{
  return guarded(ctx, [&] {
    if (!out || !count) throw bk_error(BK_ERR_ARG, "bk_junctions: null output");
    if (ctx->shard) throw bk_error(BK_ERR_ARG, "bk_junctions: sharded contexts (bk_shard_*) are not supported");
    if (!ctx->bp_done || !ctx->clustered || !ctx->summary_map) throw bk_error(BK_ERR_ARG, "bk_junctions: call bk_split_breakpoints first");
    const uint64_t ncl = ctx->n_clusters;
    const JunctionPairs jp = junction_pairs(ctx);
    struct bk_junction *d_res;
    uint32_t *d_vis;
    {
      Scope s(ctx, "junctions", jp.n * (12ull + 4ull));
      junctions(jp, tuple_table(ctx), ctx->clusters_ptr(), ncl, ctx->jnb, ctx->st, &d_res, &d_vis);
    }
    std::vector<uint32_t> vis(ctx->timing ? ncl : 0);
    if (!vis.empty()) HIP_CHECK(hipMemcpyAsync(vis.data(), d_vis, ncl * 4, hipMemcpyDeviceToHost, ctx->st));
    rows_to_host(ctx, d_res, ncl, ctx->f_junction);
    if (ctx->timing && !ctx->timers.empty())
    {
      uint64_t visited = 0;
      for (uint32_t v : vis) visited += v;
      ctx->timers.back().touched = jp.n * (12ull + 32ull) + visited * sizeof(bk_split) + ncl * (sizeof(bk_cluster) + 2ull * sizeof(struct bk_junction) + 4ull);
    }
    *out = ctx->f_junction.data();
    *count = ncl;
  });
}

int bk_evidence(bk_ctx *ctx, const struct bk_evidence **out, uint64_t *count, const uint64_t **call_off)
{
  return guarded(ctx, [&] {
    if (!out || !count || !call_off) throw bk_error(BK_ERR_ARG, "bk_evidence: null output");
    if (ctx->shard) throw bk_error(BK_ERR_ARG, "bk_evidence: sharded contexts (bk_shard_*) are not supported");
    if (!ctx->bp_done || !ctx->clustered || !ctx->summary_map) throw bk_error(BK_ERR_ARG, "bk_evidence: call bk_split_breakpoints first");
    const uint64_t ncl = ctx->n_clusters;
    const bk_soa &t = ctx->rec;
    if (ncl && (!ctx->have_records || !t.mapq || (!t.side && !t.qhash))) throw bk_error(BK_ERR_ARG, "bk_evidence: the record table lacks a column");
    const JunctionPairs jp = junction_pairs(ctx);
    EvidenceRecs er{t.n, t.side, t.qhash, t.qcheck, t.mapq};
    struct bk_evidence *d_rows;
    uint64_t *d_off;
    EvidenceStat *d_stat;
    {
      Scope s(ctx, "evidence", jp.n * (12ull + 4ull + 2ull * 12ull));
      evidence(jp, tuple_table(ctx), ctx->clusters_ptr(), ncl, er, ctx->evb, ctx->st, &d_rows, &d_off, &d_stat);
    }
    ctx->f_ev_off.assign(ncl + 1, 0);
    EvidenceStat stat{};
    HIP_CHECK(hipMemcpyAsync(ctx->f_ev_off.data(), d_off, (ncl + 1) * 8, hipMemcpyDeviceToHost, ctx->st));
    HIP_CHECK(hipMemcpyAsync(&stat, d_stat, sizeof stat, hipMemcpyDeviceToHost, ctx->st));
    HIP_CHECK(hipStreamSynchronize(ctx->st));
    if (stat.bad) throw bk_error(BK_ERR_HIP, "bk_evidence: the listing and the counts of bk_junctions disagree (internal error)");
    const uint64_t n = ctx->f_ev_off[ncl];
    rows_to_host(ctx, d_rows, n, ctx->f_evidence);
    if (ctx->timing && !ctx->timers.empty())
    {
      uint64_t n_pair_rows = 0;
      for (uint64_t i = 0; i < n; ++i) n_pair_rows += ctx->f_evidence[i].kind == BK_EV_PAIR;
      int bits = 1;
      while ((ncl >> bits) != 0) ++bits;
      const uint64_t passes = (uint64_t) (bits + 7) / 8;
      ctx->timers.back().touched = jp.n * (12ull + 32ull) + 2ull * stat.visited * sizeof(bk_split) + ncl * (2ull * sizeof(bk_cluster) + 2ull * sizeof(struct bk_junction) + 20ull) +
                                   jp.n * (12ull + 12ull + passes * 32ull + 12ull) + n_pair_rows * (64ull + 32ull) + (n - n_pair_rows) * 32ull +
                                   n * sizeof(struct bk_evidence);
    }
    *out = ctx->f_evidence.data();
    *count = n;
    *call_off = ctx->f_ev_off.data();
  });
}

int bk_junction_sides(const struct bk_junction *j, uint8_t *right1, uint8_t *right2, uint8_t *source)
{
  if (!j || !right1 || !right2 || !source) return BK_ERR_ARG;
  auto largest = [](const uint32_t *v) {
    int best = 0;
    for (int i = 1; i < 4; ++i)
      if (v[i] > v[best]) best = i;
    return v[best] ? best : -1;
  };
  int idx = largest(j->splits);
  *source = 2;
  if (idx < 0)
  {
    idx = largest(j->pairs);
    *source = 1;
  }
  if (idx < 0)
  {
    idx = 1;
    *source = 0;
  }
  *right1 = (uint8_t) (idx >> 1);
  *right2 = (uint8_t) (idx & 1);
  return BK_OK;
}

int bk_clip_rescue(const bk_cluster *c, const struct bk_junction *j, const struct bk_clip_support *s, uint32_t min_support, uint32_t *pos1, uint32_t *pos2, uint32_t *n1,
                   uint32_t *n2)
{
  if (!c || !j || !s || !pos1 || !pos2 || !n1 || !n2 || min_support == 0) return BK_ERR_ARG;
  if ((c->flags & 2u) || c->p1_tid < 0 || c->p2_tid < 0) return 0;
  uint8_t d1 = 0, d2 = 1, source = 0;
  bk_junction_sides(j, &d1, &d2, &source);
  if (s->peak_n[0][d1] < min_support || s->peak_n[1][d2] < min_support) return 0;
  *pos1 = s->peak_pos[0][d1];
  *pos2 = s->peak_pos[1][d2];
  *n1 = s->peak_n[0][d1];
  *n2 = s->peak_n[1][d2];
  return 1;
}

int bk_vcf_breakend_alt(char ref_base, int own_right, const char *mate_chr, uint32_t mate_pos, int mate_right, char *buf, size_t cap)
{
  if (!mate_chr || !buf) return BK_ERR_ARG;
  const char br = mate_right ? '[' : ']';
  const std::string mate = br + std::string(mate_chr) + ":" + std::to_string(mate_pos) + br;
  const std::string alt = own_right ? mate + ref_base : ref_base + mate;
  if (alt.size() + 1 > cap) return BK_ERR_ARG;
  std::memcpy(buf, alt.c_str(), alt.size() + 1);
  return BK_OK;
}

int bk_run(bk_ctx *ctx, int mapq_min, int fast, double *w_out, uint64_t *n_valid)
{
  if (!ctx) return BK_ERR_ARG;
  if (ctx->stream_done && mapq_min != ctx->stream_mapq) ctx->stream_done = false;
  ctx->mapq_min = mapq_min;
  double mean, sd;
  int rc = bk_isize_stats(ctx, &mean, &sd);
  if (rc) return rc;
  const int times = 2;
  const double w = times * std::sqrt(times) * (mean + 3 * sd);
  if (w_out) *w_out = w;
  if ((rc = bk_discordant_pairs(ctx, mapq_min, w, nullptr, nullptr))) return rc;
  if ((rc = bk_mask_and_cluster(ctx, w, fast, nullptr))) return rc;
  if ((rc = bk_split_evidence(ctx, nullptr))) return rc;
  if ((rc = bk_cluster_summary(ctx, w, nullptr))) return rc;
  if ((rc = bk_split_breakpoints(ctx, w, n_valid))) return rc;
  return BK_OK;
}

int bk_fetch(bk_ctx *ctx, int stage, const void **data, uint64_t *count, const uint64_t **group_off, uint32_t *n_groups)
{
  return guarded(ctx, [&] {
    if (!data || !count) throw bk_error(BK_ERR_ARG, "bk_fetch: null output");
    const uint32_t ng = ctx->jr.n_groups;
    if (group_off) *group_off = nullptr;
    if (n_groups) *n_groups = 0;
    auto fetch_list = [&](int slot, const uint32_t *d_idx, const uint64_t *d_goff, const uint32_t *d_cl, uint64_t n) {
      std::vector<bk_pair> all(ctx->jr.n_pairs);
      if (!all.empty()) HIP_CHECK(hipMemcpyAsync(all.data(), ctx->jr.pairs, all.size() * sizeof(bk_pair), hipMemcpyDeviceToHost, ctx->st));
      std::vector<uint32_t> idx(n), cl(d_cl ? n : 0);
      std::vector<uint64_t> goff(ng + 1, 0);
      if (n && d_idx) HIP_CHECK(hipMemcpyAsync(idx.data(), d_idx, n * 4, hipMemcpyDeviceToHost, ctx->st));
      if (n && d_cl) HIP_CHECK(hipMemcpyAsync(cl.data(), d_cl, n * 4, hipMemcpyDeviceToHost, ctx->st));
      if (ng && d_goff) HIP_CHECK(hipMemcpyAsync(goff.data(), d_goff, (ng + 1) * 8, hipMemcpyDeviceToHost, ctx->st));
      HIP_CHECK(hipStreamSynchronize(ctx->st));
      auto &out = ctx->f_pairs[slot];
      auto &off = ctx->f_off[slot];
      out.clear();
      off.assign(1, 0);
      for (uint32_t l = 0; l < ng; ++l)
      {
        uint32_t g = ctx->lex_to_num[l];
        for (uint64_t p = goff[g]; p < goff[g + 1]; ++p)
        {
          bk_pair pr = all[d_idx ? idx[p] : p];
          if (d_cl) pr.cluster = (int32_t) cl[p];
          out.push_back(pr);
        }
        off.push_back(out.size());
      }
      *data = out.data();
      *count = out.size();
      if (group_off) *group_off = off.data();
      if (n_groups) *n_groups = ng;
    };
    switch (stage)
    {
    case BK_STAGE_SCAN:
      fetch_list(0, nullptr, ctx->jr.gstart, nullptr, ctx->jr.n_pairs);
      break;
    case BK_STAGE_ISO:
      fetch_list(1, ctx->stage.iso_idx.get<uint32_t>(), ctx->stage.iso_goff.get<uint64_t>(), nullptr, ctx->stage.iso_n);
      break;
    case BK_STAGE_CLUSTERED:
      if (!ctx->clustered) throw bk_error(BK_ERR_ARG, "bk_fetch: not clustered yet");
      fetch_list(2, ctx->stage.list.idx.get<uint32_t>(), ctx->stage.list.goff.get<uint64_t>(), ctx->stage.d_cluster.get<uint32_t>(), ctx->stage.list.n);
      break;
    case BK_STAGE_SPLITS:
      ensure_splits_sorted(ctx);
      ctx->f_splits.resize(ctx->hc.n_split);
      if (ctx->hc.n_split)
        HIP_CHECK(hipMemcpyAsync(ctx->f_splits.data(), ctx->d_split.get<bk_split>(), ctx->hc.n_split * sizeof(bk_split), hipMemcpyDeviceToHost, ctx->st));
      HIP_CHECK(hipStreamSynchronize(ctx->st));
      *data = ctx->f_splits.data();
      *count = ctx->f_splits.size();
      break;
    case BK_STAGE_CLUSTERS:
      rows_to_host(ctx, ctx->clusters_ptr(), ctx->n_clusters, ctx->f_clusters);
      {
        auto by_group = [](const bk_cluster &a, const bk_cluster &b) { return a.group < b.group; };
        if (ctx->ext_clusters)
          std::stable_sort(ctx->f_clusters.begin(), ctx->f_clusters.end(), by_group);
        else if (!std::is_sorted(ctx->f_clusters.begin(), ctx->f_clusters.end(), by_group))
          throw bk_error(BK_ERR_HIP, "bk_fetch: the cluster table is not in group order (internal error)");
      }
      *data = ctx->f_clusters.data();
      *count = ctx->f_clusters.size();
      break;
    case BK_STAGE_GROUP_KEYS:
      ctx->f_gkeys.clear();
      for (uint32_t l = 0; l < ng; ++l)
      {
        uint32_t k = ctx->gkey_host[ctx->lex_to_num[l]];
        ctx->f_gkeys.push_back((int32_t) (k / (uint32_t) (ctx->nt + 1)) - 1);
        ctx->f_gkeys.push_back((int32_t) (k % (uint32_t) (ctx->nt + 1)) - 1);
      }
      *data = ctx->f_gkeys.data();
      *count = ng;
      break;
    default:
      throw bk_error(BK_ERR_ARG, "bk_fetch: unknown stage");
    }
  });
}

int bk_shard_begin(bk_ctx *ctx, uint64_t rec_base, int mapq_min)
{
  return guarded(ctx, [&] {
    ctx->rec_base = rec_base;
    ctx->shard = true;
    ctx->streamed = true;
    ctx->mapq_min = mapq_min;
    ctx->ext_cand = nullptr;
    ctx->ext_split = nullptr;
    ctx->ext_clusters = nullptr;
    run_stream(ctx);
  });
}

int bk_shard_get_stats(bk_ctx *ctx, bk_shard_stats *out)
{
  return guarded(ctx, [&] {
    if (!ctx->stream_done || !out) throw bk_error(BK_ERR_ARG, "bk_shard_get_stats: call bk_shard_begin first");
    out->isize_sum = ctx->hc.isize_sum;
    out->isize_n = ctx->hc.isize_n;
    out->sumsq = ctx->hsd.sumsq;
    out->vmax = ctx->hsd.vmax;
    out->max_span = ctx->hc.max_span;
    out->n_cand = ctx->hc.n_cand;
    out->n_split = ctx->hc.n_split;
  });
}

int bk_shard_set_stats(bk_ctx *ctx, const bk_shard_stats *total)
{
  return guarded(ctx, [&] {
    if (!ctx->stream_done || !total) throw bk_error(BK_ERR_ARG, "bk_shard_set_stats: call bk_shard_begin first");
    ctx->hc.isize_sum = total->isize_sum;
    ctx->hc.isize_n = total->isize_n;
    ctx->hsd.sumsq = total->sumsq;
    ctx->hsd.vmax = total->vmax;
    ctx->hc.max_span = total->max_span;
    ctx->stats_done = false;
  });
}

static void sd_mean_thr(bk_ctx *ctx, double &m, double &thr)
{
  const double n = (double) ctx->hc.isize_n;
  m = (double) (long long) ctx->hc.isize_sum / n;
  if (ctx->hc.isize_n == 0)
  {
    thr = 0;
    return;
  }
  double sum_d = ctx->hsd.sumsq - 2.0 * m * (double) ctx->hc.isize_sum + n * m * m;
  if (!(sum_d > 0)) sum_d = 0;
  double da = (double) ctx->hsd.vmax - m, dmax = da * da + m * m;
  double bound = 2.0 * sum_d + 2.0 * n + 2.0 * dmax + 4.0;
  int k = std::ilogb(bound) + 1;
  thr = k >= 51 ? 1.0e300 : std::ldexp(1.0, k - 53);
}

int bk_shard_sd_local(bk_ctx *ctx, uint64_t *l_total, void **ex_dev, uint64_t *n_ex)
{
  return guarded(ctx, [&] {
    if (!ctx->stream_done) throw bk_error(BK_ERR_ARG, "bk_shard_sd_local: call bk_shard_begin / bk_shard_set_stats first");
    double m, thr;
    sd_mean_thr(ctx, m, thr);
    unsigned long long lt = 0, ne = 0;
    launch_sd_local(ctx->rec.flag, ctx->rec.isize, ctx->rec.n, m, thr, ctx->sdb, ctx->st, &lt, &ne);
    HIP_CHECK(hipStreamSynchronize(ctx->st));
    if (l_total) *l_total = lt;
    if (n_ex) *n_ex = ne;
    if (ex_dev) *ex_dev = ctx->sdb.exceptions.p;
  });
}

int bk_shard_sd_finish(bk_ctx *ctx, const void *all_ex_dev, uint64_t n_all, uint64_t l_grand, double *mean, double *sd)
{
  return guarded(ctx, [&] {
    double m, thr;
    sd_mean_thr(ctx, m, thr);
    launch_sd_walk((const SdException *) all_ex_dev, n_all, l_grand, ctx->d_sd.get<SdState>(), ctx->st);
    HIP_CHECK(hipMemcpyAsync(&ctx->hsd.t_final, &ctx->d_sd.get<SdState>()->t_final, 8, hipMemcpyDeviceToHost, ctx->st));
    HIP_CHECK(hipStreamSynchronize(ctx->st));
    ctx->mean = m;
    ctx->sd = std::sqrt((double) ctx->hsd.t_final / (double) ctx->hc.isize_n);
    ctx->stats_done = true;
    if (mean) *mean = ctx->mean;
    if (sd) *sd = ctx->sd;
  });
}

int bk_shard_buffer(bk_ctx *ctx, int which, void **dev, uint64_t *count, uint32_t *elem_bytes)
{
  return guarded(ctx, [&] {
    if (!dev || !count || !elem_bytes) throw bk_error(BK_ERR_ARG, "bk_shard_buffer: null output");
    switch (which)
    {
    case BK_BUF_CANDIDATES: *dev = ctx->d_cand.p; *count = ctx->ext_cand ? 0 : ctx->hc.n_cand; *elem_bytes = sizeof(Cand); break;
    case BK_BUF_TUPLES: *dev = ctx->d_split_raw.p; *count = ctx->ext_split ? 0 : ctx->hc.n_split; *elem_bytes = sizeof(bk_split); break;
    case BK_BUF_CLUSTERS: *dev = ctx->d_clusters.p; *count = ctx->ext_clusters ? 0 : ctx->n_clusters; *elem_bytes = sizeof(bk_cluster); break;
    default: throw bk_error(BK_ERR_ARG, "bk_shard_buffer: unknown buffer");
    }
  });
}

int bk_shard_set_buffer(bk_ctx *ctx, int which, const void *dev, uint64_t count)
{
  return guarded(ctx, [&] {
    switch (which)
    {
    case BK_BUF_CANDIDATES: ctx->ext_cand = (const Cand *) dev; ctx->hc.n_cand = count; break;
    case BK_BUF_TUPLES: ctx->ext_split = (const bk_split *) dev; ctx->hc.n_split = count; ctx->splits_sorted = false; break;
    case BK_BUF_CLUSTERS: ctx->ext_clusters = (bk_cluster *) dev; ctx->n_clusters = count; break;
    default: throw bk_error(BK_ERR_ARG, "bk_shard_set_buffer: unknown buffer");
    }
  });
}

int bk_shard_group_sizes(bk_ctx *ctx, const uint64_t **starts, uint32_t *n_groups)
{
  return guarded(ctx, [&] {
    if (starts) *starts = ctx->gstart_host.data();
    if (n_groups) *n_groups = ctx->jr.n_groups;
  });
}

int bk_shard_own_groups(bk_ctx *ctx, const uint8_t *own, uint32_t n_groups)
{
  return guarded(ctx, [&] {
    if (n_groups != ctx->jr.n_groups) throw bk_error(BK_ERR_ARG, "bk_shard_own_groups: wrong group count");
    ctx->own_groups.assign(own, own + n_groups);
  });
}

int bk_shard_route_candidates(bk_ctx *ctx, uint32_t world, void **dev, const uint64_t **counts)
{
  return guarded(ctx, [&] {
    if (!ctx->stream_done || ctx->ext_cand) throw bk_error(BK_ERR_ARG, "bk_shard_route_candidates: needs this shard's own candidates (after bk_shard_begin)");
    if (!world || world > 4096 || !dev || !counts) throw bk_error(BK_ERR_ARG, "bk_shard_route_candidates: bad arguments");
    *dev = route_candidates(ctx->d_cand.get<Cand>(), ctx->hc.n_cand, world, ctx->jb, ctx->st, ctx->route_counts);
    *counts = ctx->route_counts.data();
  });
}

int bk_shard_group_keys(bk_ctx *ctx, const uint32_t **keys, uint32_t *n_groups)
{
  return guarded(ctx, [&] {
    if (keys) *keys = ctx->gkey_host.data();
    if (n_groups) *n_groups = ctx->jr.n_groups;
  });
}

int bk_shard_route_pairs(bk_ctx *ctx, const uint32_t *dest_of_group, uint32_t n_groups, uint32_t world, void **dev, const uint64_t **counts)
{
  return guarded(ctx, [&] {
    if (n_groups != ctx->jr.n_groups || !world || !dev || !counts || (n_groups && !dest_of_group)) throw bk_error(BK_ERR_ARG, "bk_shard_route_pairs: bad arguments");
    ctx->route_counts.assign(world, 0);
    for (uint32_t g = 0; g < n_groups; ++g)
    {
      if (dest_of_group[g] >= world) throw bk_error(BK_ERR_ARG, "bk_shard_route_pairs: destination out of range");
      ctx->route_counts[dest_of_group[g]] += ctx->gstart_host[g + 1] - ctx->gstart_host[g];
    }
    std::vector<uint64_t> base(world, 0), off(n_groups, 0);
    for (uint32_t d = 1; d < world; ++d) base[d] = base[d - 1] + ctx->route_counts[d - 1];
    for (uint32_t g = 0; g < n_groups; ++g)
    {
      off[g] = base[dest_of_group[g]];
      base[dest_of_group[g]] += ctx->gstart_host[g + 1] - ctx->gstart_host[g];
    }
    *dev = route_pairs(ctx->jr, off, ctx->jb, ctx->st);
    *counts = ctx->route_counts.data();
  });
}

int bk_shard_group_pairs(bk_ctx *ctx, const void *pairs_dev, uint64_t n, const uint32_t *all_keys, uint32_t n_all_keys)
{
  return guarded(ctx, [&] {
    if ((n && !pairs_dev) || (n_all_keys && !all_keys)) throw bk_error(BK_ERR_ARG, "bk_shard_group_pairs: null input");
    {
      Scope s(ctx, "group_pairs");
      ctx->jb2.rec_bits = -1;
      group_pairs((const bk_pair *) pairs_dev, n, ctx->nt, ctx->jb2, ctx->st, ctx->jr);
    }
    std::vector<uint32_t> keys(all_keys, all_keys + n_all_keys);
    finish_groups(ctx, &keys);
    ctx->own_groups.clear();
    ctx->clustered = false;
  });
}

int bk_shard_bp_cov(bk_ctx *ctx, double w, void **cov_dev, uint64_t *n)
{
  return guarded(ctx, [&] {
    uint32_t *cov = bp_cov_partial(rec_view(ctx), ctx->clusters_ptr(), ctx->n_clusters, w, (int) ctx->hc.max_span, ctx->bb, ctx->st);
    HIP_CHECK(hipStreamSynchronize(ctx->st));
    if (cov_dev) *cov_dev = cov;
    if (n) *n = 2 * ctx->n_clusters;
  });
}

int bk_shard_bp_vote(bk_ctx *ctx, double w, const void *cov_total_dev)
{
  return guarded(ctx, [&] {
    ensure_splits_sorted(ctx);
    bp_vote(ctx->d_split.get<bk_split>(), ctx->hc.n_split, ctx->clusters_ptr(), ctx->n_clusters, w, (int) ctx->hc.max_span, (const uint32_t *) cov_total_dev,
            ctx->d_hdr.get<int32_t>(), ctx->bb, ctx->st);
    HIP_CHECK(hipStreamSynchronize(ctx->st));
  });
}

int bk_shard_bp_vote_slice(bk_ctx *ctx, double w, const void *cov_total_dev, uint64_t lo, uint64_t hi, void **clusters_dev, void **voted_dev)
{
  return guarded(ctx, [&] {
    if (lo > hi || hi > ctx->n_clusters || !clusters_dev || !voted_dev) throw bk_error(BK_ERR_ARG, "bk_shard_bp_vote_slice: bad range");
    ensure_splits_sorted(ctx);
    bp_vote(ctx->d_split.get<bk_split>(), ctx->hc.n_split, ctx->clusters_ptr() + lo, hi - lo, w, (int) ctx->hc.max_span,
            cov_total_dev ? (const uint32_t *) cov_total_dev + 2 * lo : nullptr, ctx->d_hdr.get<int32_t>(), ctx->bb, ctx->st);
    HIP_CHECK(hipStreamSynchronize(ctx->st));
    *clusters_dev = ctx->clusters_ptr() + lo;
    *voted_dev = ctx->bb.voted.p;
  });
}

int bk_shard_bp_set_voted(bk_ctx *ctx, const void *voted_all_dev)
{
  return guarded(ctx, [&] {
    uint32_t *v = ctx->bb.voted.as<uint32_t>(ctx->n_clusters + 1);
    if (ctx->n_clusters && voted_all_dev != v)
      HIP_CHECK(hipMemcpyAsync(v, voted_all_dev, ctx->n_clusters * 4, hipMemcpyDeviceToDevice, ctx->st));
    HIP_CHECK(hipStreamSynchronize(ctx->st));
  });
}

int bk_shard_bp_depth(bk_ctx *ctx, void **depth_dev, uint64_t *n)
{
  return guarded(ctx, [&] {
    uint32_t *d = bp_depth_partial(rec_view(ctx), ctx->clusters_ptr(), ctx->n_clusters, (int) ctx->hc.max_span, ctx->bb, ctx->st);
    HIP_CHECK(hipStreamSynchronize(ctx->st));
    if (depth_dev) *depth_dev = d;
    if (n) *n = 2 * ctx->n_clusters;
  });
}

int bk_shard_bp_finish(bk_ctx *ctx, const void *depth_total_dev)
{
  return guarded(ctx, [&] {
    bp_finish(ctx->clusters_ptr(), ctx->n_clusters, (const uint32_t *) depth_total_dev, ctx->bb, ctx->st);
    HIP_CHECK(hipStreamSynchronize(ctx->st));
  });
}

int bk_debug_std_sort(bk_ctx *ctx, const uint32_t *key, const uint64_t *group_off, uint32_t n_groups, uint32_t *perm_out)
{
  return guarded(ctx, [&] {
    if (!key || !group_off || !perm_out) throw bk_error(BK_ERR_ARG, "bk_debug_std_sort: null argument");
    const uint64_t n = group_off[n_groups];
    DevBuf dk, dp, dgof, dgoff;
    std::vector<uint32_t> gof(n), iota(n);
    for (uint32_t g = 0; g < n_groups; ++g)
      for (uint64_t p = group_off[g]; p < group_off[g + 1]; ++p) gof[p] = g;
    std::iota(iota.begin(), iota.end(), 0u);
    HIP_CHECK(hipMemcpy(dk.as<uint32_t>(n + 1), key, n * 4, hipMemcpyHostToDevice));
    HIP_CHECK(hipMemcpy(dp.as<uint32_t>(n + 1), iota.data(), n * 4, hipMemcpyHostToDevice));
    HIP_CHECK(hipMemcpy(dgof.as<uint32_t>(n + 1), gof.data(), n * 4, hipMemcpyHostToDevice));
    HIP_CHECK(hipMemcpy(dgoff.as<uint64_t>((uint64_t) n_groups + 1), group_off, ((uint64_t) n_groups + 1) * 8, hipMemcpyHostToDevice));
    uint64_t max_group = 0;
    for (uint32_t g = 0; g < n_groups; ++g) max_group = std::max<uint64_t>(max_group, group_off[g + 1] - group_off[g]);
    ctx->stage.debug_sort(ctx->device, ctx->st, dk.get<uint32_t>(), dp.get<uint32_t>(), dgof.get<uint32_t>(), dgoff.get<uint64_t>(), n_groups, n, max_group);
    HIP_CHECK(hipMemcpyAsync(perm_out, dp.get<uint32_t>(), n * 4, hipMemcpyDeviceToHost, ctx->st));
    HIP_CHECK(hipStreamSynchronize(ctx->st));
  });
}

int bk_sort_forms(bk_ctx *ctx, uint64_t out[3])
{
  return guarded(ctx, [&] {
    if (!out) throw bk_error(BK_ERR_ARG, "bk_sort_forms: null output");
    ctx->stage.sort_forms(out);
  });
}

int bk_debug_ahc(bk_ctx *ctx, const uint32_t *x, const uint32_t *y, uint32_t n, double w, uint32_t *idx_out, int32_t *cluster_out, uint32_t *n_out)
{
  return guarded(ctx, [&] {
    if (!x || !y || !idx_out || !cluster_out || !n_out) throw bk_error(BK_ERR_ARG, "bk_debug_ahc: null argument");
    std::vector<bk_pair> hp(n);
    for (uint32_t i = 0; i < n; ++i)
    {
      memset(&hp[i], 0, sizeof(bk_pair));
      hp[i].x = x[i];
      hp[i].y = y[i];
    }
    DevBuf dp, dcl;
    PairList L;
    L.n = n;
    L.ng = 1;
    std::vector<uint32_t> iota(n), gof(n, 0);
    std::iota(iota.begin(), iota.end(), 0u);
    uint64_t goff[2] = {0, n};
    HIP_CHECK(hipMemcpy(dp.as<bk_pair>(n + 1), hp.data(), n * sizeof(bk_pair), hipMemcpyHostToDevice));
    HIP_CHECK(hipMemcpy(L.idx.as<uint32_t>(n + 1), iota.data(), n * 4, hipMemcpyHostToDevice));
    HIP_CHECK(hipMemcpy(L.gof.as<uint32_t>(n + 1), gof.data(), n * 4, hipMemcpyHostToDevice));
    HIP_CHECK(hipMemcpy(L.goff.as<uint64_t>(2), goff, 16, hipMemcpyHostToDevice));
    ahc_cluster_all(dp.get<bk_pair>(), L, w, dcl, ctx->stage.ab, ctx->stage.cb(), ctx->st);
    *n_out = (uint32_t) L.n;
    if (L.n)
    {
      HIP_CHECK(hipMemcpyAsync(idx_out, L.idx.get<uint32_t>(), L.n * 4, hipMemcpyDeviceToHost, ctx->st));
      HIP_CHECK(hipMemcpyAsync(cluster_out, dcl.get<uint32_t>(), L.n * 4, hipMemcpyDeviceToHost, ctx->st));
    }
    HIP_CHECK(hipStreamSynchronize(ctx->st));
  });
}

}

namespace
{
struct FeedLink
{
  int device = 0, mapq_min = 20;
  bk_ctx *ctx = nullptr;
  int rc = BK_OK;
  std::string err;
  uint64_t done = 0;
  bool prepared = false, overflow = false;
  hipEvent_t t0 = nullptr, t1 = nullptr;
  template <class F> void guard(F &&f)
  {
    if (rc != BK_OK) return;
    try
    {
      f();
    }
    catch (const bk_error &e)
    {
      rc = e.code;
      err = e.msg;
    }
  }
};
void link_header(void *u, int nt, const char *const *names, const uint32_t *lens)
{
  FeedLink *L = (FeedLink *) u;
  if (L->ctx || L->rc != BK_OK) return;
  L->rc = bk_init(L->device, lens, names, nt, &L->ctx);
  if (L->rc != BK_OK) L->err = bk_last_error(nullptr);
}
void link_reset(void *u)
{
  FeedLink *L = (FeedLink *) u;
  L->guard([&] {
    if (L->ctx) HIP_CHECK(hipStreamSynchronize(L->ctx->st));
    L->done = 0;
    L->prepared = false;
    L->overflow = false;
  });
}
void link_before_move(void *u)
{
  FeedLink *L = (FeedLink *) u;
  L->guard([&] {
    if (L->ctx) HIP_CHECK(hipStreamSynchronize(L->ctx->st));
  });
}
void link_chunk(void *u, const bk_soa *cols, uint64_t n_ready, uint64_t n_est, hipEvent_t ready)
{
  FeedLink *L = (FeedLink *) u;
  L->guard([&] {
    bk_ctx *c = L->ctx;
    if (!c || n_ready < (uint64_t) STREAM_V + 1) return;
    c->rec = *cols;
    c->have_records = true;
    c->mapq_min = L->mapq_min;
    if (!L->prepared)
    {
      stream_prepare(c, n_est + n_est / 4);
      L->prepared = true;
    }
    const uint64_t lim = (n_ready - 1) / STREAM_V * STREAM_V;
    if (lim <= L->done) return;
    HIP_CHECK(hipStreamWaitEvent(c->st, ready, 0));
    StreamArgs a = stream_args(c, lim);
    a.q_begin = L->done / STREAM_V;
    launch_stream(a, c->st);
    L->done = lim;
  });
}
}


extern "C" {

int bk_bam_decode_device_ctx(const char *path, int device, int mapq_min, bk_bam_dev **bam_out, bk_ctx **ctx_out, int *n_targets, const char *const **names,
                             const uint32_t **lens, char *err, size_t errlen)
{
  auto fail = [&](int code, const std::string &m) {
    if (err && errlen) snprintf(err, errlen, "%s", m.c_str());
    return code;
  };
  if (!path || !bam_out || !ctx_out) return fail(BK_ERR_ARG, "bk_bam_decode_device_ctx: null argument");
  *bam_out = nullptr;
  *ctx_out = nullptr;
  FeedLink L;
  L.device = device;
  L.mapq_min = mapq_min;
  FeedConsumer fc;
  fc.user = &L;
  fc.on_header = link_header;
  fc.on_chunk = link_chunk;
  fc.before_move = link_before_move;
  fc.on_reset = link_reset;
  bk_soa cols;
  bk_bam_dev *bam = nullptr;
  int rc = bam_decode_device_impl(path, device, &bam, &cols, n_targets, names, lens, err, errlen, &fc);
  if (rc == BK_OK && L.rc != BK_OK) rc = fail(L.rc, L.err);
  if (rc == BK_OK && !L.ctx) rc = fail(BK_ERR_IO, "bk_bam_decode_device_ctx: no header");
  if (rc != BK_OK)
  {
    if (L.ctx) bk_free(L.ctx);
    if (bam) bk_bam_dev_free(bam);
    return rc;
  }
  bk_ctx *c = L.ctx;
  rc = guarded(c, [&] {
    const uint64_t done = L.prepared ? L.done : 0;
    c->stream_done = c->stats_done = c->clustered = false;
    c->rec = cols;
    c->have_records = true;
    c->mapq_min = mapq_min;
    c->rec_base = 0;
    bool ok = false;
    if (L.prepared)
    {
      Scope s(c, "k_stream", 39ull * cols.n + 4ull * cols.n_cigar_words);
      StreamArgs a = stream_args(c, cols.n);
      a.q_begin = done / STREAM_V;
      launch_stream(a, c->st);
      ok = stream_finish(c);
    }
    if (ok)
      stream_rare_path(c);
    else
      run_stream(c);
    if (bk_debug("feed"))
      fprintf(stderr, "[feed/stream] stream pass %s: %llu of %llu records went through k_stream while the file was still arriving\n", ok ? "overlapped" : "after the feed",
              (unsigned long long) (ok ? done : 0), (unsigned long long) cols.n);
  });
  if (rc != BK_OK)
  {
    fail(rc, c->err);
    bk_free(c);
    bk_bam_dev_free(bam);
    return rc;
  }
  *bam_out = bam;
  *ctx_out = c;
  return BK_OK;
}

int bk_group_stats(bk_ctx *ctx, const bk_group_stat **out, uint32_t *n_groups)
{
  return guarded(ctx, [&] {
    if (!out || !n_groups) throw bk_error(BK_ERR_ARG, "bk_group_stats: null output");
    if (!ctx->clustered) throw bk_error(BK_ERR_ARG, "bk_group_stats: call bk_mask_and_cluster (and bk_cluster_summary) first");
    const uint32_t ng = ctx->jr.n_groups;
    std::vector<uint64_t> iso(ng + 1, 0), clu(ng + 1, 0);
    std::vector<uint32_t> kmax(ng + 1, 0);
    if (ng)
    {
      HIP_CHECK(hipMemcpyAsync(iso.data(), ctx->stage.iso_goff.get<uint64_t>(), ((uint64_t) ng + 1) * 8, hipMemcpyDeviceToHost, ctx->st));
      HIP_CHECK(hipMemcpyAsync(clu.data(), ctx->stage.list.goff.get<uint64_t>(), ((uint64_t) ng + 1) * 8, hipMemcpyDeviceToHost, ctx->st));
      if (ctx->stage.list.n && ctx->bb.kmax.p) HIP_CHECK(hipMemcpyAsync(kmax.data(), ctx->bb.kmax.get<uint32_t>(), (uint64_t) ng * 4, hipMemcpyDeviceToHost, ctx->st));
      HIP_CHECK(hipStreamSynchronize(ctx->st));
    }
    ctx->f_gstats.assign(ng, bk_group_stat{});
    for (uint32_t l = 0; l < ng; ++l)
    {
      const uint32_t g = ctx->lex_to_num[l];
      bk_group_stat &o = ctx->f_gstats[l];
      const uint32_t k = ctx->gkey_host[g];
      o.p1_tid = (int32_t) (k / (uint32_t) (ctx->nt + 1)) - 1;
      o.p2_tid = (int32_t) (k % (uint32_t) (ctx->nt + 1)) - 1;
      o.n_scan = ctx->gstart_host[g + 1] - ctx->gstart_host[g];
      o.n_isolated_removed = iso[g + 1] - iso[g];
      o.n_clustered = clu[g + 1] - clu[g];
      o.cluster_id_end = o.n_clustered ? kmax[g] : 0;
      o.ordinal = ctx->glex_host[g];
    }
    *out = ctx->f_gstats.data();
    *n_groups = ng;
  });
}

int bk_debug_points(bk_ctx *ctx, int mode, const uint32_t *x, const uint32_t *y, uint32_t n, double w, uint32_t *idx_out, int32_t *cluster_out, uint32_t *n_out)
{
  return guarded(ctx, [&] {
    if ((n && (!x || !y)) || !idx_out || !n_out || mode < 0 || mode > 2) throw bk_error(BK_ERR_ARG, "bk_debug_points: bad argument");
    std::vector<bk_pair> hp(n);
    for (uint32_t i = 0; i < n; ++i)
    {
      memset(&hp[i], 0, sizeof(bk_pair));
      hp[i].x = x[i];
      hp[i].y = y[i];
    }
    DevBuf dp, dcl, dgof, dgoff;
    PairList L;
    std::vector<uint32_t> gof(n, 0);
    uint64_t goff[2] = {0, n};
    if (n) HIP_CHECK(hipMemcpy(dp.as<bk_pair>(n + 1), hp.data(), n * sizeof(bk_pair), hipMemcpyHostToDevice));
    if (n) HIP_CHECK(hipMemcpy(dgof.as<uint32_t>(n + 1), gof.data(), n * 4, hipMemcpyHostToDevice));
    HIP_CHECK(hipMemcpy(dgoff.as<uint64_t>(2), goff, 16, hipMemcpyHostToDevice));
    const bk_pair *pairs = dp.as<bk_pair>(n + 1);
    remove_isolated_all(pairs, dgof.get<uint32_t>(), dgoff.get<uint64_t>(), 1, mode == 1 ? n : 0, w, L, ctx->stage.cb(), ctx->st);
    if (mode != 1)
    {
      L.n = n;
      L.ng = 1;
      std::vector<uint32_t> iota(n);
      std::iota(iota.begin(), iota.end(), 0u);
      if (n) HIP_CHECK(hipMemcpy(L.idx.as<uint32_t>(n + 1), iota.data(), n * 4, hipMemcpyHostToDevice));
      if (n) HIP_CHECK(hipMemcpy(L.gof.as<uint32_t>(n + 1), gof.data(), n * 4, hipMemcpyHostToDevice));
      HIP_CHECK(hipMemcpy(L.goff.as<uint64_t>(2), goff, 16, hipMemcpyHostToDevice));
      if (mode == 0)
        debug_mask_list(pairs, L, (long) w, ctx->stage.cb(), ctx->st);
      else
        fast_cluster_all(pairs, L, w, dcl, ctx->stage.cb(), ctx->st);
    }
    *n_out = (uint32_t) L.n;
    if (L.n)
    {
      HIP_CHECK(hipMemcpyAsync(idx_out, L.idx.get<uint32_t>(), L.n * 4, hipMemcpyDeviceToHost, ctx->st));
      if (mode == 2 && cluster_out) HIP_CHECK(hipMemcpyAsync(cluster_out, dcl.get<uint32_t>(), L.n * 4, hipMemcpyDeviceToHost, ctx->st));
    }
    HIP_CHECK(hipStreamSynchronize(ctx->st));
  });
}

int bk_debug_cigar(bk_ctx *ctx, uint32_t n, const uint8_t *kind, const uint32_t *c1_off, const uint8_t *c1, const uint32_t *c2_off, const uint8_t *c2, const int32_t *e,
                   int32_t *out6)
{
  return guarded(ctx, [&] {
    if (!n) return;
    if (!kind || !c1_off || !c1 || !c2_off || !c2 || !e || !out6) throw bk_error(BK_ERR_ARG, "bk_debug_cigar: null argument");
    DevBuf dk, d1o, d1, d2o, d2, de, dout;
    HIP_CHECK(hipMemcpy(dk.as<uint8_t>(n), kind, n, hipMemcpyHostToDevice));
    HIP_CHECK(hipMemcpy(d1o.as<uint32_t>(n + 1), c1_off, (n + 1) * 4, hipMemcpyHostToDevice));
    HIP_CHECK(hipMemcpy(d1.as<uint8_t>(c1_off[n] + 16), c1, c1_off[n], hipMemcpyHostToDevice));
    HIP_CHECK(hipMemcpy(d2o.as<uint32_t>(n + 1), c2_off, (n + 1) * 4, hipMemcpyHostToDevice));
    HIP_CHECK(hipMemcpy(d2.as<uint8_t>(c2_off[n] + 16), c2, c2_off[n], hipMemcpyHostToDevice));
    HIP_CHECK(hipMemcpy(de.as<int32_t>(n), e, n * 4, hipMemcpyHostToDevice));
    int32_t *o = dout.as<int32_t>(6ull * n);
    debug_cigar(dk.get<uint8_t>(), d1o.get<uint32_t>(), d1.get<uint8_t>(), d2o.get<uint32_t>(), d2.get<uint8_t>(), de.get<int32_t>(), n, o, ctx->st);
    HIP_CHECK(hipMemcpyAsync(out6, o, 24ull * n, hipMemcpyDeviceToHost, ctx->st));
    HIP_CHECK(hipStreamSynchronize(ctx->st));
  });
}

int bk_debug_vote(bk_ctx *ctx, const bk_split *side1, uint32_t n1, const bk_split *side2, uint32_t n2, int32_t p1_tid, int32_t p2_tid, int32_t *out3)
{
  return guarded(ctx, [&] {
    if ((n1 && !side1) || (n2 && !side2) || !out3) throw bk_error(BK_ERR_ARG, "bk_debug_vote: null argument");
    const uint32_t pos1 = 100000, pos2 = 300000;
    std::vector<bk_split> t;
    auto put = [&](const bk_split *src, uint32_t n, int32_t tid, uint32_t pos, uint64_t salt) {
      for (uint32_t i = 0; i < n + 2; ++i)
      {
        bk_split s;
        if (i < n)
          s = src[i];
        else
        {
          memset(&s, 0, sizeof s);
          s.qhash = 0xD00D000000000000ull + salt + i;
          s.prim_chr = s.sec_chr = -7;
        }
        s.tid = tid;
        s.pos = (int32_t) pos;
        s.endpos = (int32_t) pos + 50;
        t.push_back(s);
      }
    };
    put(side1, n1, p1_tid, pos1, 0);
    put(side2, n2, p2_tid, pos2, 1000);
    std::stable_sort(t.begin(), t.end(), [](const bk_split &a, const bk_split &b) { return (uint32_t) a.tid != (uint32_t) b.tid ? (uint32_t) a.tid < (uint32_t) b.tid : a.pos < b.pos; });
    for (size_t i = 0; i < t.size(); ++i) t[i].rec = i;
    bk_cluster c;
    memset(&c, 0, sizeof c);
    c.p1_tid = p1_tid;
    c.p2_tid = p2_tid;
    c.p1_mean = pos1 + 10;
    c.p2_mean = pos2 + 10;
    c.p1_exact = 0xFFFFFFFFu;
    c.p2_exact = -1;
    DevBuf dt, dc, dcov;
    HIP_CHECK(hipMemcpy(dt.as<bk_split>(t.size() + 1), t.data(), t.size() * sizeof(bk_split), hipMemcpyHostToDevice));
    HIP_CHECK(hipMemcpy(dc.as<bk_cluster>(2), &c, sizeof c, hipMemcpyHostToDevice));
    const uint32_t cov[2] = {5, 5};
    HIP_CHECK(hipMemcpy(dcov.as<uint32_t>(4), cov, 8, hipMemcpyHostToDevice));
    bp_vote(dt.get<bk_split>(), t.size(), dc.get<bk_cluster>(), 1, 1000.0, 200, dcov.get<uint32_t>(), ctx->d_hdr.get<int32_t>(), ctx->bb, ctx->st);
    uint32_t voted = 0;
    HIP_CHECK(hipMemcpyAsync(&voted, ctx->bb.voted.get<uint32_t>(), 4, hipMemcpyDeviceToHost, ctx->st));
    HIP_CHECK(hipMemcpyAsync(&c, dc.get<bk_cluster>(), sizeof c, hipMemcpyDeviceToHost, ctx->st));
    HIP_CHECK(hipStreamSynchronize(ctx->st));
    out3[0] = voted ? (int32_t) c.p1_exact : -1;
    out3[1] = voted ? c.p2_exact : -1;
    out3[2] = voted ? (int32_t) c.n_sr : 0;
  });
}

int bk_debug_region(bk_ctx *ctx, int32_t tid, uint32_t start, uint32_t end, uint64_t depth_pos, bk_split *out, uint32_t cap, uint32_t *n_out, uint32_t *cov_out,
                    uint32_t *depth_out)
{
  return guarded(ctx, [&] {
    if (!ctx->stream_done) run_stream(ctx);
    ensure_splits_sorted(ctx);
    DevBuf dout, dres;
    bk_split *o = dout.as<bk_split>((uint64_t) cap + 1);
    uint32_t *res = dres.as<uint32_t>(4);
    debug_region(rec_view(ctx), ctx->d_split.get<bk_split>(), ctx->hc.n_split, tid, start, end, (int) ctx->hc.max_span, depth_pos, o, cap, res, ctx->st);
    uint32_t h[4] = {0, 0, 0, 0};
    HIP_CHECK(hipMemcpyAsync(h, res, 16, hipMemcpyDeviceToHost, ctx->st));
    HIP_CHECK(hipStreamSynchronize(ctx->st));
    const uint32_t n = h[0] < cap ? h[0] : cap;
    if (n && out) HIP_CHECK(hipMemcpy(out, o, n * sizeof(bk_split), hipMemcpyDeviceToHost));
    if (n_out) *n_out = h[0];
    if (cov_out) *cov_out = h[1];
    if (depth_out) *depth_out = h[2];
  });
}

int bk_timing_enable(bk_ctx *ctx, int on)
{
  return guarded(ctx, [&] {
    ctx->timing = on != 0;
    for (auto &t : ctx->timers)
    {
      if (t.a) (void) hipEventDestroy(t.a);
      if (t.b) (void) hipEventDestroy(t.b);
    }
    ctx->timers.clear();
  });
}

int bk_timing(bk_ctx *ctx, const char *const **names, const float **ms, const uint64_t **bytes, int *n)
{
  return guarded(ctx, [&] {
    HIP_CHECK(hipStreamSynchronize(ctx->st));
    Timing &t = ctx->tout;
    t.names.clear(); t.ms.clear(); t.bytes.clear(); t.touched.clear(); t.cnames.clear();
    for (auto &s : ctx->timers)
    {
      float v = 0;
      HIP_CHECK(hipEventElapsedTime(&v, s.a, s.b));
      t.names.push_back(s.name);
      t.ms.push_back(v);
      t.bytes.push_back(s.bytes);
      t.touched.push_back(s.touched);
    }
    for (auto &s : t.names) t.cnames.push_back(s.c_str());
    if (names) *names = t.cnames.data();
    if (ms) *ms = t.ms.data();
    if (bytes) *bytes = t.bytes.data();
    if (n) *n = (int) t.names.size();
  });
}

int bk_timing_touched(bk_ctx *ctx, const uint64_t **touched, int *n)
{
  return guarded(ctx, [&] {
    if (touched) *touched = ctx->tout.touched.data();
    if (n) *n = (int) ctx->tout.touched.size();
  });
}

}
```

### breakid_amd/csrc/join.h

```cpp
#pragma once
#include "bk_common.h"
#include "prims.h"
#include <vector>

struct JoinBufs
{
  DevBuf counter, unsorted, okey, oval, key, val, pairs, gof, gflag, gscan, gstart, gkey, scan_tmp, route_cand, route_cnt, route_pairs, route_off, maxrec, key2, val2;
  prims::RadixBufs radix;
  int rec_bits = 32;
  int rec_bits_eff = 32;
};

struct JoinResult
{
  uint64_t n_pairs = 0;
  uint32_t n_groups = 0;
  bk_pair *pairs = nullptr;
  uint32_t *gof = nullptr;
  uint64_t *gstart = nullptr;
  uint32_t *gkey = nullptr;
};

void join_candidates(const Cand *cand, uint64_t n_cand, double w, const uint32_t *tprefix, int32_t nt, JoinBufs &b, hipStream_t st, JoinResult &res);
void join_assign_ids(JoinResult &res, const uint32_t *glex_dev, hipStream_t st);

Cand *route_candidates(const Cand *cand, uint64_t n, uint32_t world, JoinBufs &b, hipStream_t st, std::vector<uint64_t> &counts);
bk_pair *route_pairs(const JoinResult &jr, const std::vector<uint64_t> &off_of_group, JoinBufs &b, hipStream_t st);
void group_pairs(const bk_pair *raw, uint64_t np, int32_t nt, JoinBufs &b, hipStream_t st, JoinResult &res);
```

### breakid_amd/csrc/join.hip

```cpp
#include "bk_common.h"
#include "prims.h"
#include "join.h"

namespace
{
__global__ __launch_bounds__(256) void k_join_keys(const Cand *__restrict__ c, uint64_t n, uint64_t *__restrict__ key, uint32_t *__restrict__ val)
{
  uint64_t i = (uint64_t) blockIdx.x * blockDim.x + threadIdx.x;
  if (i < n)
  {
    key[i] = c[i].qhash;
    val[i] = (uint32_t) i;
  }
}

__global__ __launch_bounds__(256) void k_join_rec_keys(const Cand *__restrict__ c, uint64_t n, uint64_t *__restrict__ key, uint32_t *__restrict__ val)
{
  uint64_t i = (uint64_t) blockIdx.x * blockDim.x + threadIdx.x;
  if (i < n)
  {
    key[i] = c[i].rec;
    val[i] = (uint32_t) i;
  }
}
__global__ __launch_bounds__(256) void k_join_hash_of(const Cand *__restrict__ c, const uint32_t *__restrict__ order, uint64_t n, uint64_t *__restrict__ key, uint32_t *__restrict__ val)
{
  uint64_t i = (uint64_t) blockIdx.x * blockDim.x + threadIdx.x;
  if (i < n)
  {
    key[i] = c[order[i]].qhash;
    val[i] = order[i];
  }
}

__device__ __forceinline__ uint32_t gpos(const uint32_t *__restrict__ tprefix, int32_t nt, int32_t tid, int32_t pos)
{
  uint32_t base = tid <= 0 ? 0u : tprefix[tid < nt ? tid : nt];
  return base + (uint32_t) pos;
}

template <class F> __device__ __forceinline__ void join_run(const Cand *__restrict__ cand, const uint64_t *__restrict__ key, const uint32_t *__restrict__ val, uint64_t n, double w,
                                                            const uint32_t *__restrict__ tprefix, int32_t nt, uint32_t *__restrict__ err, uint64_t i, F &&append, bool ordered = false)
{
  if (i >= n) return;
  const uint64_t h = key[i];
  if (i > 0 && key[i - 1] == h) return;
  uint64_t e = i + 1;
  while (e < n && key[e] == h) ++e;
  const uint32_t len = (uint32_t) (e - i);
  if (len < 2) return;
  if (len > 4096 && !ordered)
  {
    atomicOr(err, 1u);
    return;
  }
  Cand r0 = {}, r1 = {};
  if (len == 2)
  {
    r0 = cand[val[i]];
    r1 = cand[val[i + 1]];
    if (r0.qcheck != r1.qcheck) atomicOr(err, 2u);
    if (r1.rec < r0.rec)
    {
      const Cand t = r0;
      r0 = r1;
      r1 = t;
    }
  }
  long long last_rec = -1;
  uint32_t buffered = 0xFFFFFFFFu;
  for (uint32_t step = 0; step < len; ++step)
  {
    uint32_t best = 0xFFFFFFFFu;
    if (len == 2)
      best = step;
    else if (ordered)
    {
      best = val[i + step];
      if (cand[best].qcheck != cand[val[i]].qcheck) atomicOr(err, 2u);
    }
    else
    {
      long long best_rec = 0x7fffffffffffffffLL;
      for (uint32_t k = 0; k < len; ++k)
      {
        uint32_t ci = val[i + k];
        if (step == 0 && cand[ci].qcheck != cand[val[i]].qcheck) atomicOr(err, 2u);
        long long r = cand[ci].rec;
        if (r > last_rec && r < best_rec)
        {
          best_rec = r;
          best = ci;
        }
      }
      last_rec = best_rec;
    }
    if (buffered == 0xFFFFFFFFu)
    {
      buffered = best;
      continue;
    }
    const Cand b = len == 2 ? r0 : cand[buffered], c = len == 2 ? r1 : cand[best];
    buffered = 0xFFFFFFFFu;
    int32_t bt = b.tid < 0 ? -1 : b.tid, ct = c.tid < 0 ? -1 : c.tid;
    long long dp = (long long) c.pos - (long long) b.pos;
    if (dp < 0) dp = -dp;
    if (!(bt != ct || (double) dp >= w)) continue;
    uint32_t c1 = gpos(tprefix, nt, c.tid, c.pos);
    uint32_t c2 = gpos(tprefix, nt, c.mtid, c.mpos);
    bk_pair p;
    if (c1 <= c2)
    {
      p.p1_flag = c.flag; p.p1_tid = ct; p.p1_pos = (uint32_t) ((long long) c.pos + 1); p.p1_mapq = c.mapq;
      p.x = c1; p.y = c2;
      p.p2_flag = b.flag; p.p2_tid = bt; p.p2_pos = (uint32_t) ((long long) b.pos + 1); p.p2_mapq = b.mapq;
    }
    else
    {
      p.p2_flag = c.flag; p.p2_tid = ct; p.p2_pos = (uint32_t) ((long long) c.pos + 1); p.p2_mapq = c.mapq;
      p.x = c2; p.y = c1;
      p.p1_flag = b.flag; p.p1_tid = bt; p.p1_pos = (uint32_t) ((long long) b.pos + 1); p.p1_mapq = b.mapq;
    }
    p.p1_rev = (p.p1_flag & 0x10) ? 1 : 0;
    p.p2_rev = (p.p2_flag & 0x10) ? 1 : 0;
    p.rec = c.rec;
    p.id = 0;
    p.cluster = -1;
    p.group = 0;
    p.reserved = 0;
    append(p);
  }
}


__global__ __launch_bounds__(256) void k_join_pairs(const Cand *__restrict__ cand, const uint64_t *__restrict__ key, const uint32_t *__restrict__ val, uint64_t n, double w,
                                                    const uint32_t *__restrict__ tprefix, int32_t nt, bk_pair *__restrict__ out, uint64_t *__restrict__ okey,
                                                    uint32_t *__restrict__ oval, unsigned long long cap, unsigned long long *__restrict__ counter,
                                                    uint32_t *__restrict__ err, int rbits, int ordered)
{
  __shared__ unsigned int s_cnt;
  __shared__ unsigned long long s_base;
  if (threadIdx.x == 0) s_cnt = 0;
  __syncthreads();
  bool have = false;
  bk_pair first_pair;
  auto append = [&](const bk_pair &p) {
    if (!have)
    {
      have = true;
      first_pair = p;
      return;
    }
    unsigned long long slot = atomicAdd(counter, 1ull);
    if (slot < cap)
    {
      out[slot] = p;
      uint64_t gk = (uint64_t) (uint32_t) (p.p1_tid + 1) * (uint64_t) (nt + 1) + (uint64_t) (uint32_t) (p.p2_tid + 1);
      okey[slot] = (gk << rbits) | p.rec;
      oval[slot] = (uint32_t) slot;
    }
  };
  const uint64_t i = (uint64_t) blockIdx.x * blockDim.x + threadIdx.x;
  join_run(cand, key, val, n, w, tprefix, nt, err, i, append, ordered != 0);
  unsigned int my = 0;
  if (have) my = atomicAdd(&s_cnt, 1u);
  __syncthreads();
  if (threadIdx.x == 0 && s_cnt) s_base = atomicAdd(counter, (unsigned long long) s_cnt);
  __syncthreads();
  if (have)
  {
    const unsigned long long slot = s_base + my;
    if (slot < cap)
    {
      const bk_pair &p = first_pair;
      out[slot] = p;
      uint64_t gk = (uint64_t) (uint32_t) (p.p1_tid + 1) * (uint64_t) (nt + 1) + (uint64_t) (uint32_t) (p.p2_tid + 1);
      okey[slot] = (gk << rbits) | p.rec;
      oval[slot] = (uint32_t) slot;
    }
  }
}

__global__ __launch_bounds__(256) void k_gather_pairs(const bk_pair *__restrict__ in, const uint32_t *__restrict__ perm, const uint64_t *__restrict__ key, uint64_t n,
                                                      bk_pair *__restrict__ out, uint32_t *__restrict__ gflag, int rbits)
{
  uint64_t i = (uint64_t) blockIdx.x * blockDim.x + threadIdx.x;
  if (i >= n) return;
  out[i] = in[perm[i]];
  gflag[i] = (i == 0 || (key[i] >> rbits) != (key[i - 1] >> rbits)) ? 1u : 0u;
}

__global__ __launch_bounds__(256) void k_group_starts(const uint32_t *__restrict__ gflag, const uint32_t *__restrict__ gscan, const uint64_t *__restrict__ key, uint64_t n,
                                                      uint64_t *__restrict__ gstart, uint32_t *__restrict__ gkey, uint32_t *__restrict__ gof, int rbits)
{
  uint64_t i = (uint64_t) blockIdx.x * blockDim.x + threadIdx.x;
  if (i >= n) return;
  uint32_t g = gscan[i] + gflag[i] - 1;
  gof[i] = g;
  if (gflag[i])
  {
    gstart[g] = i;
    gkey[g] = (uint32_t) (key[i] >> rbits);
  }
  if (i == n - 1) gstart[g + 1] = n;
}

__global__ __launch_bounds__(256) void k_assign_ids(bk_pair *__restrict__ pairs, const uint32_t *__restrict__ gof, const uint64_t *__restrict__ gstart,
                                                    const uint32_t *__restrict__ glex, uint64_t n)
{
  uint64_t i = (uint64_t) blockIdx.x * blockDim.x + threadIdx.x;
  if (i >= n) return;
  uint32_t g = gof[i];
  pairs[i].group = glex[g];
  pairs[i].id = (uint32_t) (i - gstart[g]);
}
__global__ __launch_bounds__(256) void k_max_rec_cand(const Cand *__restrict__ c, uint64_t n, unsigned long long *__restrict__ out)
{
  uint64_t i = (uint64_t) blockIdx.x * blockDim.x + threadIdx.x;
  unsigned long long v = i < n ? (unsigned long long) c[i].rec : 0ull;
  for (int d = 32; d >= 1; d >>= 1)
  {
    const unsigned long long o = __shfl_xor(v, d, 64);
    v = o > v ? o : v;
  }
  if ((threadIdx.x & 63) == 0 && v) atomicMax(out, v);
}
__global__ __launch_bounds__(256) void k_max_rec_pair(const bk_pair *__restrict__ p, uint64_t n, unsigned long long *__restrict__ out)
{
  uint64_t i = (uint64_t) blockIdx.x * blockDim.x + threadIdx.x;
  unsigned long long v = i < n ? (unsigned long long) p[i].rec : 0ull;
  for (int d = 32; d >= 1; d >>= 1)
  {
    const unsigned long long o = __shfl_xor(v, d, 64);
    v = o > v ? o : v;
  }
  if ((threadIdx.x & 63) == 0 && v) atomicMax(out, v);
}
__global__ __launch_bounds__(256) void k_pair_keys(const bk_pair *__restrict__ p, uint64_t n, int32_t nt, uint64_t *__restrict__ okey, uint32_t *__restrict__ oval, int rbits)
{
  uint64_t i = (uint64_t) blockIdx.x * blockDim.x + threadIdx.x;
  if (i >= n) return;
  uint64_t gk = (uint64_t) (uint32_t) (p[i].p1_tid + 1) * (uint64_t) (nt + 1) + (uint64_t) (uint32_t) (p[i].p2_tid + 1);
  okey[i] = (gk << rbits) | p[i].rec;
  oval[i] = (uint32_t) i;
}
__global__ __launch_bounds__(256) void k_route_pairs(const bk_pair *__restrict__ src, const uint32_t *__restrict__ gof, const uint64_t *__restrict__ gstart,
                                                     const uint64_t *__restrict__ off, uint64_t n, bk_pair *__restrict__ dst)
{
  uint64_t i = (uint64_t) blockIdx.x * blockDim.x + threadIdx.x;
  if (i >= n) return;
  const uint32_t g = gof[i];
  dst[off[g] + (i - gstart[g])] = src[i];
}
__global__ __launch_bounds__(256) void k_cand_dest(const Cand *__restrict__ c, uint64_t n, uint32_t world, uint64_t *__restrict__ key, uint32_t *__restrict__ val)
{
  uint64_t i = (uint64_t) blockIdx.x * blockDim.x + threadIdx.x;
  if (i >= n) return;
  key[i] = (uint32_t) ((c[i].qhash >> 17) % world);
  val[i] = (uint32_t) i;
}
__global__ __launch_bounds__(256) void k_dest_starts(const uint64_t *__restrict__ key, uint64_t n, unsigned long long *__restrict__ starts)
{
  uint64_t i = (uint64_t) blockIdx.x * blockDim.x + threadIdx.x;
  if (i >= n) return;
  if (i == 0 || key[i] != key[i - 1]) starts[key[i]] = i;
}
__global__ __launch_bounds__(256) void k_gather_cand(const Cand *__restrict__ in, const uint32_t *__restrict__ perm, uint64_t n, Cand *__restrict__ out)
{
  uint64_t i = (uint64_t) blockIdx.x * blockDim.x + threadIdx.x;
  if (i < n) out[i] = in[perm[i]];
}
}

constexpr uint32_t JOIN_FIX_MAX = 64;
__global__ __launch_bounds__(256) void k_join_fix_runs(uint64_t *__restrict__ key, uint32_t *__restrict__ val, uint64_t n, uint32_t *__restrict__ err)
{
  const uint64_t i = (uint64_t) blockIdx.x * blockDim.x + threadIdx.x;
  if (i >= n) return;
  const uint64_t k0 = key[i];
  const uint32_t hi = (uint32_t) (k0 >> 32);
  if (i > 0 && (uint32_t) (key[i - 1] >> 32) == hi) return;
  uint64_t e = i + 1;
  bool mixed = false;
  while (e < n)
  {
    const uint64_t k = key[e];
    if ((uint32_t) (k >> 32) != hi) break;
    mixed |= k != k0;
    ++e;
  }
  if (!mixed) return;
  const uint64_t len = e - i;
  if (len > JOIN_FIX_MAX)
  {
    atomicOr(err, 4u);
    return;
  }
  for (uint64_t a = 1; a < len; ++a)
  {
    const uint64_t kk = key[i + a];
    const uint32_t vv = val[i + a];
    uint64_t b = a;
    while (b > 0 && key[i + b - 1] > kk)
    {
      key[i + b] = key[i + b - 1];
      val[i + b] = val[i + b - 1];
      --b;
    }
    key[i + b] = kk;
    val[i + b] = vv;
  }
}

template <class T, class K> static int effective_rec_bits(const T *items, uint64_t n, K kernel, int32_t nt, JoinBufs &b, hipStream_t st)
{
  int bits = b.rec_bits;
  if (bits < 0)
  {
    unsigned long long *m = b.maxrec.as<unsigned long long>(1), h = 0;
    HIP_CHECK(hipMemsetAsync(m, 0, 8, st));
    if (n) hipLaunchKernelGGL(kernel, dim3(cdiv(n, 256)), dim3(256), 0, st, items, n, m);
    HIP_CHECK(hipMemcpyAsync(&h, m, 8, hipMemcpyDeviceToHost, st));
    HIP_CHECK(hipStreamSynchronize(st));
    bits = 1;
    while (bits < 63 && (1ull << bits) <= h) ++bits;
  }
  int gbits = 1;
  while ((1ull << gbits) < (uint64_t) (nt + 1) * (uint64_t) (nt + 1) && gbits < 32) ++gbits;
  if (bits + gbits > 64) throw bk_error(BK_ERR_LIMIT, "pair sort key: chromosome-pair key and record index need more than 64 bits");
  b.rec_bits_eff = bits;
  return bits;
}

static uint64_t join_raw_pairs(const Cand *cand, uint64_t n_cand, double w, const uint32_t *tprefix, int32_t nt, JoinBufs &b, hipStream_t st)
{
  if (n_cand > 0xFFFFFFF0ull) throw bk_error(BK_ERR_LIMIT, "more than 2^32 discordant candidates");
  const int rec_bits = effective_rec_bits(cand, n_cand, k_max_rec_cand, nt, b, st);
  unsigned long long *counter = b.counter.as<unsigned long long>(2);
  uint32_t *err = (uint32_t *) (counter + 1);
  HIP_CHECK(hipMemsetAsync(counter, 0, 16, st));
  uint64_t cap = n_cand / 2 + 1;
  bk_pair *unsorted = b.unsorted.as<bk_pair>(cap);
  uint64_t *okey = b.okey.as<uint64_t>(cap);
  uint32_t *oval = b.oval.as<uint32_t>(cap);
  unsigned long long host[2] = {0, 0};
  static const int first_attempt = getenv("BK_JOIN_ATTEMPT") ? std::max(0, std::min(2, atoi(getenv("BK_JOIN_ATTEMPT")))) : 0;
  for (int attempt = first_attempt; attempt < 3; ++attempt)
  {
    if (n_cand)
    {
      uint64_t *key = b.key.as<uint64_t>(n_cand);
      uint32_t *val = b.val.as<uint32_t>(n_cand);
      uint64_t *ks;
      uint32_t *vs;
      if (attempt < 2)
      {
        hipLaunchKernelGGL(k_join_keys, dim3(cdiv(n_cand, 256)), dim3(256), 0, st, cand, n_cand, key, val);
        prims::radix_sort_pairs(key, val, n_cand, attempt == 0 ? 32 : 0, 64, b.radix, st, &ks, &vs);
        if (attempt == 0) hipLaunchKernelGGL(k_join_fix_runs, dim3(cdiv(n_cand, 256)), dim3(256), 0, st, ks, vs, n_cand, err);
      }
      else
      {
        hipLaunchKernelGGL(k_join_rec_keys, dim3(cdiv(n_cand, 256)), dim3(256), 0, st, cand, n_cand, key, val);
        prims::radix_sort_pairs(key, val, n_cand, 0, rec_bits, b.radix, st, &ks, &vs);
        uint64_t *key2 = b.key2.as<uint64_t>(n_cand);
        uint32_t *val2 = b.val2.as<uint32_t>(n_cand);
        hipLaunchKernelGGL(k_join_hash_of, dim3(cdiv(n_cand, 256)), dim3(256), 0, st, cand, (const uint32_t *) vs, n_cand, key2, val2);
        prims::radix_sort_pairs(key2, val2, n_cand, 0, 64, b.radix, st, &ks, &vs);
      }
      hipLaunchKernelGGL(k_join_pairs, dim3(cdiv(n_cand, 256)), dim3(256), 0, st, cand, ks, vs, n_cand, w, tprefix, nt, unsorted, okey, oval,
                         (unsigned long long) cap, counter, err, rec_bits, attempt == 2 ? 1 : 0);
    }
    HIP_CHECK(hipMemcpyAsync(host, counter, 16, hipMemcpyDeviceToHost, st));
    HIP_CHECK(hipStreamSynchronize(st));
    if (attempt == 0 && ((uint32_t) host[1] & 4u))
    {
      HIP_CHECK(hipMemsetAsync(counter, 0, 16, st));
      continue;
    }
    if (attempt < 2 && ((uint32_t) host[1] & 1u) && !((uint32_t) host[1] & 2u))
    {
      HIP_CHECK(hipMemsetAsync(counter, 0, 16, st));
      attempt = 1;
      continue;
    }
    break;
  }
  if ((uint32_t) host[1] & 2u)
    throw bk_error(BK_ERR_COLLISION, "two different read names share one 64-bit name hash (their second hashes differ): the mate join would not be the reference's");
  if ((uint32_t) host[1] & 1u) throw bk_error(BK_ERR_HIP, "mate join: a run was refused although its candidates were sorted (internal error)");
  if (host[0] > cap) throw bk_error(BK_ERR_LIMIT, "pair capacity exceeded");
  return host[0];
}

static void group_sorted(const bk_pair *unsorted, uint64_t *okey, uint32_t *oval, uint64_t np, int32_t nt, JoinBufs &b, hipStream_t st, JoinResult &res)
{
  res = JoinResult();
  res.n_pairs = np;
  bk_pair *pairs = b.pairs.as<bk_pair>(np + 1);
  uint32_t *gof = b.gof.as<uint32_t>(np + 1);
  res.pairs = pairs;
  res.gof = gof;
  if (np == 0) return;
  int gbits = 1;
  while ((1ull << gbits) < (uint64_t) (nt + 1) * (uint64_t) (nt + 1) && gbits < 32) ++gbits;
  uint64_t *ks;
  uint32_t *vs;
  const int rbits = b.rec_bits_eff;
  prims::radix_sort_pairs(okey, oval, np, 0, rbits + gbits, b.radix, st, &ks, &vs);
  uint32_t *gflag = b.gflag.as<uint32_t>(np + 1);
  uint32_t *gscan = b.gscan.as<uint32_t>(np + 1);
  hipLaunchKernelGGL(k_gather_pairs, dim3(cdiv(np, 256)), dim3(256), 0, st, unsorted, vs, ks, np, pairs, gflag, rbits);
  prims::exclusive_scan<uint32_t>(gflag, gscan, np, b.scan_tmp, st);
  uint32_t ng = 0;
  HIP_CHECK(hipMemcpyAsync(&ng, gscan + np, 4, hipMemcpyDeviceToHost, st));
  HIP_CHECK(hipStreamSynchronize(st));
  res.n_groups = ng;
  uint64_t *gstart = b.gstart.as<uint64_t>((uint64_t) ng + 1);
  uint32_t *gkey = b.gkey.as<uint32_t>((uint64_t) ng + 1);
  hipLaunchKernelGGL(k_group_starts, dim3(cdiv(np, 256)), dim3(256), 0, st, gflag, gscan, ks, np, gstart, gkey, gof, rbits);
  res.gstart = gstart;
  res.gkey = gkey;
}

void join_candidates(const Cand *cand, uint64_t n_cand, double w, const uint32_t *tprefix, int32_t nt, JoinBufs &b, hipStream_t st, JoinResult &res)
{
  const uint64_t np = join_raw_pairs(cand, n_cand, w, tprefix, nt, b, st);
  group_sorted(b.unsorted.get<bk_pair>(), b.okey.get<uint64_t>(), b.oval.get<uint32_t>(), np, nt, b, st, res);
}

void group_pairs(const bk_pair *raw, uint64_t np, int32_t nt, JoinBufs &b, hipStream_t st, JoinResult &res)
{
  if (np > 0xFFFFFFF0ull) throw bk_error(BK_ERR_LIMIT, "more than 2^32 pairs");
  uint64_t *okey = b.okey.as<uint64_t>(np + 1);
  uint32_t *oval = b.oval.as<uint32_t>(np + 1);
  const int rec_bits = effective_rec_bits(raw, np, k_max_rec_pair, nt, b, st);
  if (np) hipLaunchKernelGGL(k_pair_keys, dim3(cdiv(np, 256)), dim3(256), 0, st, raw, np, nt, okey, oval, rec_bits);
  group_sorted(raw, okey, oval, np, nt, b, st, res);
}

Cand *route_candidates(const Cand *cand, uint64_t n, uint32_t world, JoinBufs &b, hipStream_t st, std::vector<uint64_t> &counts)
{
  counts.assign(world, 0);
  Cand *out = b.route_cand.as<Cand>(n + 1);
  if (n == 0) return out;
  if (n > 0xFFFFFFF0ull) throw bk_error(BK_ERR_LIMIT, "more than 2^32 discordant candidates");
  unsigned long long *dc = b.route_cnt.as<unsigned long long>(world);
  HIP_CHECK(hipMemsetAsync(dc, 0xFF, (size_t) world * 8, st));
  uint64_t *key = b.key.as<uint64_t>(n);
  uint32_t *val = b.val.as<uint32_t>(n);
  hipLaunchKernelGGL(k_cand_dest, dim3(cdiv(n, 256)), dim3(256), 0, st, cand, n, world, key, val);
  int bits = 1;
  while ((1u << bits) < world && bits < 31) ++bits;
  uint64_t *ks;
  uint32_t *vs;
  prims::radix_sort_pairs(key, val, n, 0, bits, b.radix, st, &ks, &vs);
  hipLaunchKernelGGL(k_gather_cand, dim3(cdiv(n, 256)), dim3(256), 0, st, cand, vs, n, out);
  hipLaunchKernelGGL(k_dest_starts, dim3(cdiv(n, 256)), dim3(256), 0, st, ks, n, dc);
  std::vector<uint64_t> starts(world + 1, n);
  HIP_CHECK(hipMemcpyAsync(starts.data(), dc, (size_t) world * 8, hipMemcpyDeviceToHost, st));
  HIP_CHECK(hipStreamSynchronize(st));
  for (uint32_t d = world; d-- > 0;)
    if (starts[d] == ~0ull) starts[d] = starts[d + 1];
  for (uint32_t d = 0; d < world; ++d) counts[d] = starts[d + 1] - starts[d];
  return out;
}

bk_pair *route_pairs(const JoinResult &jr, const std::vector<uint64_t> &off_of_group, JoinBufs &b, hipStream_t st)
{
  bk_pair *out = b.route_pairs.as<bk_pair>(jr.n_pairs + 1);
  if (jr.n_pairs == 0) return out;
  uint64_t *doff = b.route_off.as<uint64_t>((uint64_t) jr.n_groups + 1);
  HIP_CHECK(hipMemcpyAsync(doff, off_of_group.data(), (size_t) jr.n_groups * 8, hipMemcpyHostToDevice, st));
  hipLaunchKernelGGL(k_route_pairs, dim3(cdiv(jr.n_pairs, 256)), dim3(256), 0, st, jr.pairs, jr.gof, jr.gstart, doff, jr.n_pairs, out);
  HIP_CHECK(hipStreamSynchronize(st));
  return out;
}

void join_assign_ids(JoinResult &res, const uint32_t *glex_dev, hipStream_t st)
{
  if (res.n_pairs == 0) return;
  hipLaunchKernelGGL(k_assign_ids, dim3(cdiv(res.n_pairs, 256)), dim3(256), 0, st, res.pairs, res.gof, res.gstart, glex_dev, res.n_pairs);
}
```

### include/breakid_hip.h

```cpp
#ifndef BREAKID_HIP_H
#define BREAKID_HIP_H

#include <stdint.h>
#include <stddef.h>

#ifdef __cplusplus
extern "C" {
#endif

#define BK_OK 0
#define BK_ERR_ARG (-1)
#define BK_ERR_HIP (-2)
#define BK_ERR_NO_DEVICE (-3)
#define BK_ERR_UNSORTED (-4)
#define BK_ERR_CIGAR (-5)
#define BK_ERR_IO (-6)
#define BK_ERR_LIMIT (-7)
#define BK_ERR_COLLISION (-8)

#define BK_MEM_HOST 0
#define BK_MEM_DEVICE 1

typedef struct bk_ctx bk_ctx;

typedef struct bk_soa {
  uint64_t n;
  const int32_t *tid, *pos, *mtid, *mpos, *isize;
  const uint16_t *flag;
  const uint8_t *mapq;
  const uint64_t *qhash;
  const uint32_t *cigar_off;
  const uint32_t *cigar;
  const uint32_t *aux_off;
  const uint8_t *aux;
  uint64_t n_cigar_words;
  uint64_t n_aux_bytes;
  const uint32_t *qcheck;
  const struct bk_side *side;
} bk_soa;

typedef struct bk_side {
  uint64_t qhash;
  int32_t mtid, mpos;
  uint32_t qcheck;
  uint32_t reserved[3];
} bk_side;

typedef struct bk_pair {
  uint32_t x, y;
  uint32_t p1_pos, p2_pos;
  int32_t p1_tid, p2_tid;
  uint16_t p1_flag, p2_flag;
  uint8_t p1_mapq, p2_mapq, p1_rev, p2_rev;
  uint64_t rec;
  uint32_t id;
  int32_t cluster;
  uint32_t group;
  uint32_t reserved;
} bk_pair;

typedef struct bk_split {
  uint64_t rec;
  int32_t tid, pos, endpos;
  uint32_t reserved;
  uint64_t qhash;
  int32_t prim_chr, sec_chr;
  uint32_t prim_start, prim_end, prim_bp, sec_start, sec_end, sec_bp;
  uint64_t prim_cigar, sec_cigar;
  uint32_t flags;
  uint32_t qcheck;
} bk_split;

#define BK_TYPE_DIFF_CHR 1u
#define BK_TYPE_SAME_ORIENT 2u
#define BK_TYPE_ABS_REVERSE 4u
#define BK_TYPE_DEFAULT_ORIENT 8u

typedef struct bk_cluster {
  uint32_t group;
  int32_t id;
  int32_t p1_tid, p2_tid;
  uint32_t p1_mean, p2_mean, p1_min, p1_max, p2_min, p2_max;
  uint32_t p1_exact;
  int32_t p2_exact;
  uint32_t n_drp, n_sr;
  uint32_t depth1, depth2;
  uint32_t type_mask;
  uint32_t flags;
} bk_cluster;

#define BK_STAGE_SCAN 0
#define BK_STAGE_ISO 1
#define BK_STAGE_CLUSTERED 2
#define BK_STAGE_SPLITS 3
#define BK_STAGE_CLUSTERS 4
#define BK_STAGE_GROUP_KEYS 5

int bk_init(int device, const uint32_t *target_len, const char *const *target_name, int n_targets, bk_ctx **out);
void bk_prepare_process(void);
void bk_free(bk_ctx *ctx);
const char *bk_last_error(const bk_ctx *ctx);
int bk_set_stream(bk_ctx *ctx, void *hip_stream);
int bk_sync(bk_ctx *ctx);
int bk_get_stream(bk_ctx *ctx, void **hip_stream);

int bk_upload_records(bk_ctx *ctx, const bk_soa *cols, int mem_space);

typedef struct bk_regions {
  const int32_t *tid, *beg, *end;
  uint64_t n;
} bk_regions;
int bk_exclude_regions(bk_ctx *ctx, const bk_regions *r, uint64_t *n_removed);

int bk_isize_stats(bk_ctx *ctx, double *mean, double *sd);
int bk_discordant_pairs(bk_ctx *ctx, int mapq_min, double w, uint64_t *n_pairs, uint32_t *n_groups);
int bk_mask_and_cluster(bk_ctx *ctx, double w, int fast, uint64_t *n_clustered);
int bk_split_evidence(bk_ctx *ctx, uint64_t *n_tuples);
int bk_cluster_summary(bk_ctx *ctx, double w, uint64_t *n_clusters);
int bk_split_breakpoints(bk_ctx *ctx, double w, uint64_t *n_valid);

int bk_run(bk_ctx *ctx, int mapq_min, int fast, double *w_out, uint64_t *n_valid);

struct bk_normal_support { uint32_t n_drp, n_sr, depth1, depth2; };
int bk_normal_support(bk_ctx *tumor, bk_ctx *normal, double w, const struct bk_normal_support **out, uint64_t *count);

struct bk_ref_support { uint32_t ref_pairs1, ref_pairs2, ref_reads1, ref_reads2; };
int bk_ref_support(bk_ctx *calls, bk_ctx *records, int mapq_min, int anchor, double w, const struct bk_ref_support **out, uint64_t *count);
int bk_genotype_call(uint32_t alt, uint32_t ref, uint8_t *gt, uint8_t *gq, float *vaf);

struct bk_junction {
  uint32_t pairs[4];
  uint32_t splits[4];
  uint64_t mapq_sum1, mapq_sum2;
};
int bk_junctions(bk_ctx *ctx, const struct bk_junction **out, uint64_t *count);
int bk_junction_sides(const struct bk_junction *j, uint8_t *right1, uint8_t *right2, uint8_t *source);
int bk_vcf_breakend_alt(char ref_base, int own_right, const char *mate_chr, uint32_t mate_pos, int mate_right, char *buf, size_t cap);

struct bk_clip_support { uint32_t at[2][2], peak_pos[2][2], peak_n[2][2], events[2][2]; };
int bk_clip_support(bk_ctx *calls, bk_ctx *records, int mapq_min, int min_clip, double w, const struct bk_clip_support **out, uint64_t *count);
int bk_base_depth(bk_ctx *records, const int32_t *tid, const uint32_t *pos, uint64_t n, const uint32_t **out);
int bk_clip_rescue(const bk_cluster *c, const struct bk_junction *j, const struct bk_clip_support *s, uint32_t min_support, uint32_t *pos1, uint32_t *pos2, uint32_t *n1,
                   uint32_t *n2);

#define BK_EV_PAIR 1
#define BK_EV_SPLIT 2
struct bk_evidence {
  uint64_t rec;
  uint64_t qhash;
  uint32_t qcheck;
  uint32_t call;
  int32_t tid1; uint32_t pos1;
  int32_t tid2; uint32_t pos2;
  uint16_t flag1, flag2;
  uint8_t mapq1, mapq2;
  uint8_t kind;
  uint8_t sides;
};
int bk_evidence(bk_ctx *ctx, const struct bk_evidence **out, uint64_t *count, const uint64_t **call_off);

int bk_fetch(bk_ctx *ctx, int stage, const void **data, uint64_t *count, const uint64_t **group_off, uint32_t *n_groups);

typedef struct bk_group_stat {
  int32_t p1_tid, p2_tid;
  uint64_t n_scan, n_isolated_removed, n_clustered;
  uint32_t cluster_id_end;
  uint32_t ordinal;
} bk_group_stat;
int bk_group_stats(bk_ctx *ctx, const bk_group_stat **out, uint32_t *n_groups);

int bk_timing(bk_ctx *ctx, const char *const **names, const float **ms, const uint64_t **bytes, int *n);
int bk_timing_enable(bk_ctx *ctx, int on);
int bk_timing_touched(bk_ctx *ctx, const uint64_t **touched, int *n);

typedef struct bk_shard_stats {
  uint64_t isize_sum, isize_n;
  double sumsq;
  uint32_t vmax, max_span;
  uint64_t n_cand, n_split;
} bk_shard_stats;
#define BK_BUF_CANDIDATES 0
#define BK_BUF_TUPLES 1
#define BK_BUF_CLUSTERS 2
int bk_shard_begin(bk_ctx *ctx, uint64_t rec_base, int mapq_min);
int bk_shard_get_stats(bk_ctx *ctx, bk_shard_stats *out);
int bk_shard_set_stats(bk_ctx *ctx, const bk_shard_stats *total);
int bk_shard_sd_local(bk_ctx *ctx, uint64_t *l_total, void **ex_dev, uint64_t *n_ex);
int bk_shard_sd_finish(bk_ctx *ctx, const void *all_ex_dev, uint64_t n_all, uint64_t l_grand, double *mean, double *sd);
int bk_shard_buffer(bk_ctx *ctx, int which, void **dev, uint64_t *count, uint32_t *elem_bytes);
int bk_shard_set_buffer(bk_ctx *ctx, int which, const void *dev, uint64_t count);
int bk_shard_group_sizes(bk_ctx *ctx, const uint64_t **starts, uint32_t *n_groups);
int bk_shard_own_groups(bk_ctx *ctx, const uint8_t *own, uint32_t n_groups);
int bk_shard_route_candidates(bk_ctx *ctx, uint32_t world, void **dev, const uint64_t **counts);
int bk_shard_group_keys(bk_ctx *ctx, const uint32_t **keys, uint32_t *n_groups);
int bk_shard_route_pairs(bk_ctx *ctx, const uint32_t *dest_of_group, uint32_t n_groups, uint32_t world, void **dev, const uint64_t **counts);
int bk_shard_group_pairs(bk_ctx *ctx, const void *pairs_dev, uint64_t n, const uint32_t *all_keys, uint32_t n_all_keys);
int bk_shard_bp_cov(bk_ctx *ctx, double w, void **cov_dev, uint64_t *n);
int bk_shard_bp_vote(bk_ctx *ctx, double w, const void *cov_total_dev);
int bk_shard_bp_vote_slice(bk_ctx *ctx, double w, const void *cov_total_dev, uint64_t lo, uint64_t hi, void **clusters_dev, void **voted_dev);
int bk_shard_bp_set_voted(bk_ctx *ctx, const void *voted_all_dev);
int bk_shard_bp_depth(bk_ctx *ctx, void **depth_dev, uint64_t *n);
int bk_shard_bp_finish(bk_ctx *ctx, const void *depth_total_dev);

int bk_debug_std_sort(bk_ctx *ctx, const uint32_t *key, const uint64_t *group_off, uint32_t n_groups, uint32_t *perm_out);

int bk_sort_forms(bk_ctx *ctx, uint64_t out[3]);

int bk_debug_ahc(bk_ctx *ctx, const uint32_t *x, const uint32_t *y, uint32_t n, double w, uint32_t *idx_out, int32_t *cluster_out, uint32_t *n_out);

int bk_debug_points(bk_ctx *ctx, int mode, const uint32_t *x, const uint32_t *y, uint32_t n, double w, uint32_t *idx_out, int32_t *cluster_out, uint32_t *n_out);
int bk_debug_cigar(bk_ctx *ctx, uint32_t n, const uint8_t *kind, const uint32_t *c1_off, const uint8_t *c1, const uint32_t *c2_off, const uint8_t *c2, const int32_t *e,
                   int32_t *out6);
int bk_debug_vote(bk_ctx *ctx, const bk_split *side1, uint32_t n1, const bk_split *side2, uint32_t n2, int32_t p1_tid, int32_t p2_tid, int32_t *out3);
int bk_debug_region(bk_ctx *ctx, int32_t tid, uint32_t start, uint32_t end, uint64_t depth_pos, bk_split *out, uint32_t cap, uint32_t *n_out, uint32_t *cov_out,
                    uint32_t *depth_out);

typedef struct bk_bam bk_bam;
uint64_t bk_qname_hash(const char *name, size_t len);
uint32_t bk_qname_check(const char *name, size_t len);
int bk_bam_open(const char *path, bk_bam **out, char *err, size_t errlen);
int bk_bam_header(const bk_bam *b, int *n_targets, const char *const **names, const uint32_t **lens);
int bk_bam_decode(bk_bam *b, bk_soa *out, char *err, size_t errlen);
void bk_bam_close(bk_bam *b);
typedef struct bk_read_key { uint64_t qhash; uint32_t qcheck; uint32_t tag; } bk_read_key;
int bk_bam_extract(const char *in_bam, const char *out_bam, const bk_read_key *keys, uint64_t n_keys, const char *const *tags, uint64_t n_tags, char **names_out,
                   uint64_t *n_written, char *err, size_t errlen);
void bk_bam_names_free(char *names);

typedef struct bk_bam_dev bk_bam_dev;
int bk_bam_decode_device(const char *path, int device, bk_bam_dev **out, bk_soa *cols, int *n_targets, const char *const **names, const uint32_t **lens,
                         char *err, size_t errlen);
int bk_bam_decode_device_part(const char *path, int device, int part, int parts, bk_bam_dev **out, bk_soa *cols, int *n_targets, const char *const **names,
                              const uint32_t **lens, char *err, size_t errlen);
void bk_bam_dev_free(bk_bam_dev *h);
void bk_feed_release_caches(void);
int bk_bam_decode_device_ctx(const char *path, int device, int mapq_min, bk_bam_dev **bam_out, bk_ctx **ctx_out, int *n_targets, const char *const **names,
                             const uint32_t **lens, char *err, size_t errlen);
int bk_debug_bgzf_inflate(const void *file, uint64_t n, void *out, uint64_t out_cap, uint64_t *out_len, float *kernel_ms, char *err, size_t errlen);

#ifdef __cplusplus
}
#endif
#endif
```

Before: 11760.

## Join mates via hash-bucket partition and shared-memory hash table instead of sorting

```diff
diff --git a/breakid_amd/abi.py b/breakid_amd/abi.py
--- a/breakid_amd/abi.py
+++ b/breakid_amd/abi.py
@@ -6,6 +6,8 @@
 BK_ERR_ARG, BK_ERR_HIP, BK_ERR_NO_DEVICE, BK_ERR_UNSORTED, BK_ERR_CIGAR, BK_ERR_IO, BK_ERR_LIMIT, BK_ERR_COLLISION = -1, -2, -3, -4, -5, -6, -7, -8
 BK_MEM_HOST, BK_MEM_DEVICE = 0, 1
 STAGE_SCAN, STAGE_ISO, STAGE_CLUSTERED, STAGE_SPLITS, STAGE_CLUSTERS, STAGE_GROUP_KEYS = range(6)
+JOIN_FORMS = ("buckets", "upper_half_sort", "whole_hash_sort", "record_order")
+JOIN_BUCKETS, JOIN_UPPER_HALF, JOIN_WHOLE_HASH, JOIN_RECORD_ORDER = range(4)
 
 PAIR = np.dtype([("x", "<u4"), ("y", "<u4"), ("p1_pos", "<u4"), ("p2_pos", "<u4"), ("p1_tid", "<i4"),
                  ("p2_tid", "<i4"), ("p1_flag", "<u2"), ("p2_flag", "<u2"), ("p1_mapq", "u1"), ("p2_mapq", "u1"),
diff --git a/breakid_amd/capi.py b/breakid_amd/capi.py
--- a/breakid_amd/capi.py
+++ b/breakid_amd/capi.py
@@ -30,7 +30,7 @@
 EXPORTS = ["bk_init", "bk_prepare_process", "bk_free", "bk_last_error", "bk_set_stream", "bk_sync", "bk_get_stream", "bk_upload_records", "bk_exclude_regions", "bk_isize_stats",
            "bk_discordant_pairs", "bk_mask_and_cluster", "bk_split_evidence", "bk_cluster_summary",
            "bk_split_breakpoints", "bk_normal_support", "bk_ref_support", "bk_genotype_call", "bk_clip_support", "bk_base_depth", "bk_clip_rescue", "bk_junctions", "bk_junction_sides", "bk_vcf_breakend_alt", "bk_evidence", "bk_run", "bk_fetch", "bk_timing", "bk_timing_enable", "bk_timing_touched", "bk_group_stats", "bk_qname_hash", "bk_qname_check",
-           "bk_bam_open", "bk_bam_header", "bk_bam_decode", "bk_bam_close", "bk_bam_extract", "bk_bam_names_free", "bk_bam_decode_device", "bk_bam_decode_device_part", "bk_bam_decode_device_ctx", "bk_bam_dev_free", "bk_feed_release_caches", "bk_debug_bgzf_inflate", "bk_debug_std_sort", "bk_sort_forms", "bk_debug_ahc", "bk_debug_points", "bk_debug_cigar", "bk_debug_vote", "bk_debug_region", "bk_shard_begin", "bk_shard_get_stats", "bk_shard_set_stats",
+           "bk_bam_open", "bk_bam_header", "bk_bam_decode", "bk_bam_close", "bk_bam_extract", "bk_bam_names_free", "bk_bam_decode_device", "bk_bam_decode_device_part", "bk_bam_decode_device_ctx", "bk_bam_dev_free", "bk_feed_release_caches", "bk_debug_bgzf_inflate", "bk_debug_std_sort", "bk_sort_forms", "bk_join_forms", "bk_debug_ahc", "bk_debug_points", "bk_debug_cigar", "bk_debug_vote", "bk_debug_region", "bk_shard_begin", "bk_shard_get_stats", "bk_shard_set_stats",
            "bk_shard_sd_local", "bk_shard_sd_finish", "bk_shard_buffer", "bk_shard_set_buffer", "bk_shard_group_sizes",
            "bk_shard_own_groups", "bk_shard_route_candidates", "bk_shard_group_keys", "bk_shard_route_pairs", "bk_shard_group_pairs", "bk_shard_bp_cov", "bk_shard_bp_vote", "bk_shard_bp_vote_slice", "bk_shard_bp_set_voted", "bk_shard_bp_depth", "bk_shard_bp_finish"]
 
@@ -79,6 +79,7 @@
         L.bk_timing_touched.argtypes = [vp, C.POINTER(C.POINTER(C.c_uint64)), C.POINTER(C.c_int)]
         L.bk_debug_std_sort.argtypes = [vp, vp, vp, C.c_uint32, vp]
         L.bk_sort_forms.argtypes = [vp, u64p]
+        L.bk_join_forms.argtypes = [vp, u64p]
         L.bk_debug_ahc.argtypes = [vp, vp, vp, C.c_uint32, C.c_double, vp, vp, C.POINTER(C.c_uint32)]
         L.bk_debug_points.argtypes = [vp, C.c_int, vp, vp, C.c_uint32, C.c_double, vp, vp, C.POINTER(C.c_uint32)]
         L.bk_debug_cigar.argtypes = [vp, C.c_uint32, vp, vp, vp, vp, vp, vp, vp]
@@ -432,6 +433,11 @@
         self._check(self.L.bk_sort_forms(self.h, out))
         return tuple(int(v) for v in out)
 
+    def join_forms(self):
+        out = (C.c_uint64 * len(abi.JOIN_FORMS))()
+        self._check(self.L.bk_join_forms(self.h, out))
+        return tuple(int(v) for v in out)
+
     def debug_ahc(self, x, y, w):
         x = np.ascontiguousarray(x, np.uint32)
         y = np.ascontiguousarray(y, np.uint32)
diff --git a/breakid_amd/csrc/api.hip b/breakid_amd/csrc/api.hip
--- a/breakid_amd/csrc/api.hip
+++ b/breakid_amd/csrc/api.hip
@@ -627,7 +627,7 @@
   });
 }
 
-static void finish_groups(bk_ctx *ctx, const std::vector<uint32_t> *all_keys)
+static void finish_groups(bk_ctx *ctx, JoinBufs &jb, const std::vector<uint32_t> *all_keys)
 {
   const uint32_t ng = ctx->jr.n_groups;
   ctx->gkey_host.assign(ng, 0);
@@ -667,7 +667,7 @@
   uint32_t *dg = ctx->d_glex.as<uint32_t>((uint64_t) ng + 1), *dl = ctx->d_lex_to_num.as<uint32_t>((uint64_t) ng + 1);
   if (ng) HIP_CHECK(hipMemcpyAsync(dg, ctx->glex_host.data(), ng * 4, hipMemcpyHostToDevice, ctx->st));
   if (ng) HIP_CHECK(hipMemcpyAsync(dl, ctx->lex_to_num.data(), ng * 4, hipMemcpyHostToDevice, ctx->st));
-  join_assign_ids(ctx->jr, dg, ctx->st);
+  join_gather_pairs(ctx->jr, dg, jb, ctx->st);
 }
 
 int bk_discordant_pairs(bk_ctx *ctx, int mapq_min, double w, uint64_t *n_pairs, uint32_t *n_groups)
@@ -688,8 +688,8 @@
         ctx->jb.rec_bits = bits;
       }
       join_candidates(ctx->cand_ptr(), ctx->hc.n_cand, w, ctx->d_tprefix.get<uint32_t>(), ctx->nt, ctx->jb, ctx->st, ctx->jr);
-    }
-    finish_groups(ctx, nullptr);
+      finish_groups(ctx, ctx->jb, nullptr);
+    }
     ctx->clustered = false;
     ctx->joined = true;
     ctx->bp_done = false;
@@ -1357,9 +1357,9 @@
       Scope s(ctx, "group_pairs");
       ctx->jb2.rec_bits = -1;
       group_pairs((const bk_pair *) pairs_dev, n, ctx->nt, ctx->jb2, ctx->st, ctx->jr);
-    }
-    std::vector<uint32_t> keys(all_keys, all_keys + n_all_keys);
-    finish_groups(ctx, &keys);
+      std::vector<uint32_t> keys(all_keys, all_keys + n_all_keys);
+      finish_groups(ctx, ctx->jb2, &keys);
+    }
     ctx->own_groups.clear();
     ctx->clustered = false;
   });
@@ -1453,6 +1453,14 @@
   return guarded(ctx, [&] {
     if (!out) throw bk_error(BK_ERR_ARG, "bk_sort_forms: null output");
     ctx->stage.sort_forms(out);
+  });
+}
+
+int bk_join_forms(bk_ctx *ctx, uint64_t out[4])
+{
+  return guarded(ctx, [&] {
+    if (!out) throw bk_error(BK_ERR_ARG, "bk_join_forms: null output");
+    for (int k = 0; k < 4; ++k) out[k] = ctx->jb.forms[k];
   });
 }
 
diff --git a/breakid_amd/csrc/join.h b/breakid_amd/csrc/join.h
--- a/breakid_amd/csrc/join.h
+++ b/breakid_amd/csrc/join.h
@@ -5,10 +5,13 @@
 
 struct JoinBufs
 {
-  DevBuf counter, unsorted, okey, oval, key, val, pairs, gof, gflag, gscan, gstart, gkey, scan_tmp, route_cand, route_cnt, route_pairs, route_off, maxrec, key2, val2;
+  DevBuf counter, unsorted, okey, oval, key, val, pairs, gof, gflag, gscan, gstart, gkey, scan_tmp, route_cand, route_cnt, route_pairs, route_off, maxrec, key2, val2, bucket_rows, bucket_hist;
   prims::RadixBufs radix;
   int rec_bits = 32;
   int rec_bits_eff = 32;
+  const bk_pair *gather_src = nullptr;
+  const uint32_t *gather_perm = nullptr;
+  uint64_t forms[4] = {0, 0, 0, 0};
 };
 
 struct JoinResult
@@ -22,7 +25,7 @@
 };
 
 void join_candidates(const Cand *cand, uint64_t n_cand, double w, const uint32_t *tprefix, int32_t nt, JoinBufs &b, hipStream_t st, JoinResult &res);
-void join_assign_ids(JoinResult &res, const uint32_t *glex_dev, hipStream_t st);
+void join_gather_pairs(JoinResult &res, const uint32_t *glex_dev, JoinBufs &b, hipStream_t st);
 
 Cand *route_candidates(const Cand *cand, uint64_t n, uint32_t world, JoinBufs &b, hipStream_t st, std::vector<uint64_t> &counts);
 bk_pair *route_pairs(const JoinResult &jr, const std::vector<uint64_t> &off_of_group, JoinBufs &b, hipStream_t st);
diff --git a/breakid_amd/csrc/join.hip b/breakid_amd/csrc/join.hip
--- a/breakid_amd/csrc/join.hip
+++ b/breakid_amd/csrc/join.hip
@@ -1,3 +1,4 @@
+#include <cstddef>
 #include "bk_common.h"
 #include "prims.h"
 #include "join.h"
@@ -37,6 +38,36 @@
 {
   uint32_t base = tid <= 0 ? 0u : tprefix[tid < nt ? tid : nt];
   return base + (uint32_t) pos;
+}
+
+__device__ __forceinline__ bool pair_of(const Cand &b, const Cand &c, double w, const uint32_t *__restrict__ tprefix, int32_t nt, bk_pair &p)
+{
+  int32_t bt = b.tid < 0 ? -1 : b.tid, ct = c.tid < 0 ? -1 : c.tid;
+  long long dp = (long long) c.pos - (long long) b.pos;
+  if (dp < 0) dp = -dp;
+  if (!(bt != ct || (double) dp >= w)) return false;
+  uint32_t c1 = gpos(tprefix, nt, c.tid, c.pos);
+  uint32_t c2 = gpos(tprefix, nt, c.mtid, c.mpos);
+  if (c1 <= c2)
+  {
+    p.p1_flag = c.flag; p.p1_tid = ct; p.p1_pos = (uint32_t) ((long long) c.pos + 1); p.p1_mapq = c.mapq;
+    p.x = c1; p.y = c2;
+    p.p2_flag = b.flag; p.p2_tid = bt; p.p2_pos = (uint32_t) ((long long) b.pos + 1); p.p2_mapq = b.mapq;
+  }
+  else
+  {
+    p.p2_flag = c.flag; p.p2_tid = ct; p.p2_pos = (uint32_t) ((long long) c.pos + 1); p.p2_mapq = c.mapq;
+    p.x = c2; p.y = c1;
+    p.p1_flag = b.flag; p.p1_tid = bt; p.p1_pos = (uint32_t) ((long long) b.pos + 1); p.p1_mapq = b.mapq;
+  }
+  p.p1_rev = (p.p1_flag & 0x10) ? 1 : 0;
+  p.p2_rev = (p.p2_flag & 0x10) ? 1 : 0;
+  p.rec = c.rec;
+  p.id = 0;
+  p.cluster = -1;
+  p.group = 0;
+  p.reserved = 0;
+  return true;
 }
 
 template <class F> __device__ __forceinline__ void join_run(const Cand *__restrict__ cand, const uint64_t *__restrict__ key, const uint32_t *__restrict__ val, uint64_t n, double w,
@@ -102,32 +133,8 @@
     }
     const Cand b = len == 2 ? r0 : cand[buffered], c = len == 2 ? r1 : cand[best];
     buffered = 0xFFFFFFFFu;
-    int32_t bt = b.tid < 0 ? -1 : b.tid, ct = c.tid < 0 ? -1 : c.tid;
-    long long dp = (long long) c.pos - (long long) b.pos;
-    if (dp < 0) dp = -dp;
-    if (!(bt != ct || (double) dp >= w)) continue;
-    uint32_t c1 = gpos(tprefix, nt, c.tid, c.pos);
-    uint32_t c2 = gpos(tprefix, nt, c.mtid, c.mpos);
     bk_pair p;
-    if (c1 <= c2)
-    {
-      p.p1_flag = c.flag; p.p1_tid = ct; p.p1_pos = (uint32_t) ((long long) c.pos + 1); p.p1_mapq = c.mapq;
-      p.x = c1; p.y = c2;
-      p.p2_flag = b.flag; p.p2_tid = bt; p.p2_pos = (uint32_t) ((long long) b.pos + 1); p.p2_mapq = b.mapq;
-    }
-    else
-    {
-      p.p2_flag = c.flag; p.p2_tid = ct; p.p2_pos = (uint32_t) ((long long) c.pos + 1); p.p2_mapq = c.mapq;
-      p.x = c2; p.y = c1;
-      p.p1_flag = b.flag; p.p1_tid = bt; p.p1_pos = (uint32_t) ((long long) b.pos + 1); p.p1_mapq = b.mapq;
-    }
-    p.p1_rev = (p.p1_flag & 0x10) ? 1 : 0;
-    p.p2_rev = (p.p2_flag & 0x10) ? 1 : 0;
-    p.rec = c.rec;
-    p.id = 0;
-    p.cluster = -1;
-    p.group = 0;
-    p.reserved = 0;
+    if (!pair_of(b, c, w, tprefix, nt, p)) continue;
     append(p);
   }
 }
@@ -181,13 +188,214 @@
   }
 }
 
-__global__ __launch_bounds__(256) void k_gather_pairs(const bk_pair *__restrict__ in, const uint32_t *__restrict__ perm, const uint64_t *__restrict__ key, uint64_t n,
-                                                      bk_pair *__restrict__ out, uint32_t *__restrict__ gflag, int rbits)
-{
-  uint64_t i = (uint64_t) blockIdx.x * blockDim.x + threadIdx.x;
-  if (i >= n) return;
-  out[i] = in[perm[i]];
+constexpr int PART_THREADS = 1024;
+constexpr uint32_t PART_BLOCKS = 256;
+constexpr int BKT_MAX_BITS = 14;
+constexpr int BKT_THREADS = 256;
+constexpr uint32_t BKT_CAP = 4096;
+constexpr uint32_t BKT_TABLE = 2 * BKT_CAP;
+constexpr uint32_t BKT_LONG = 128;
+constexpr uint32_t BKT_EMPTY = 0xFFFFFFFFu;
+constexpr uint32_t BKT_SLOT = 0x1FFFu;
+
+__device__ __forceinline__ uint32_t bucket_of(uint64_t h, int bits) { return bits ? (uint32_t) (h >> (64 - bits)) : 0u; }
+
+__global__ __launch_bounds__(PART_THREADS) void k_bucket_hist(const Cand *__restrict__ c, uint64_t n, uint64_t chunk, int bits, uint32_t *__restrict__ ghist)
+{
+  extern __shared__ uint32_t s_bins[];
+  const uint32_t nbk = 1u << bits;
+  for (uint32_t k = threadIdx.x; k < nbk; k += PART_THREADS) s_bins[k] = 0;
+  __syncthreads();
+  const uint64_t lo = (uint64_t) blockIdx.x * chunk, hi = lo + chunk < n ? lo + chunk : n;
+  for (uint64_t i = lo + threadIdx.x; i < hi; i += PART_THREADS) atomicAdd(&s_bins[bucket_of(c[i].qhash, bits)], 1u);
+  __syncthreads();
+  for (uint32_t k = threadIdx.x; k < nbk; k += PART_THREADS) ghist[(uint64_t) k * gridDim.x + blockIdx.x] = s_bins[k];
+}
+
+__global__ __launch_bounds__(PART_THREADS) void k_bucket_scatter(const Cand *__restrict__ c, uint64_t n, uint64_t chunk, int bits, const uint32_t *__restrict__ goff,
+                                                                 Cand *__restrict__ out)
+{
+  extern __shared__ uint32_t s_bins[];
+  const uint32_t nbk = 1u << bits;
+  for (uint32_t k = threadIdx.x; k < nbk; k += PART_THREADS) s_bins[k] = goff[(uint64_t) k * gridDim.x + blockIdx.x];
+  __syncthreads();
+  const uint64_t lo = (uint64_t) blockIdx.x * chunk, hi = lo + chunk < n ? lo + chunk : n;
+  for (uint64_t i = lo + threadIdx.x; i < hi; i += PART_THREADS)
+  {
+    const uint64_t *__restrict__ src = (const uint64_t *) (c + i);
+    const uint64_t w0 = src[0], w1 = src[1], w2 = src[2], w3 = src[3], w4 = src[4];
+    const uint32_t pos = atomicAdd(&s_bins[bucket_of(w0, bits)], 1u);
+    uint64_t *__restrict__ dst = (uint64_t *) (out + pos);
+    dst[0] = w0; dst[1] = w1; dst[2] = w2; dst[3] = w3; dst[4] = w4;
+  }
+}
+static_assert(offsetof(Cand, qhash) == 0, "k_bucket_scatter takes the hash from the first word of a row");
+
+__global__ __launch_bounds__(256) void k_bucket_max(const uint32_t *__restrict__ goff, uint32_t nblk, uint32_t nbk, unsigned long long *__restrict__ out)
+{
+  const uint32_t k = blockIdx.x * blockDim.x + threadIdx.x;
+  if (k < nbk) atomicMax(out, (unsigned long long) (goff[(uint64_t) (k + 1) * nblk] - goff[(uint64_t) k * nblk]));
+}
+
+__global__ __launch_bounds__(BKT_THREADS) void k_bucket_join(const Cand *__restrict__ rows, const uint32_t *__restrict__ goff, uint32_t nblk, double w,
+                                                             const uint32_t *__restrict__ tprefix, int32_t nt, bk_pair *__restrict__ out, uint64_t *__restrict__ okey,
+                                                             uint32_t *__restrict__ oval, unsigned long long cap, unsigned long long *__restrict__ counter,
+                                                             uint32_t *__restrict__ err, int rbits)
+{
+  __shared__ uint64_t s_hash[BKT_CAP];
+  __shared__ uint32_t s_table[BKT_TABLE];
+  __shared__ uint32_t s_plist[BKT_CAP / 2];
+  __shared__ uint16_t s_long[BKT_LONG];
+  __shared__ uint32_t s_np, s_nlong, s_n, s_cnt, s_pos;
+  __shared__ unsigned long long s_base;
+  const uint32_t tid = threadIdx.x;
+  const uint32_t lo = goff[(uint64_t) blockIdx.x * nblk], n = goff[(uint64_t) (blockIdx.x + 1) * nblk] - lo;
+  if (n < 2) return;
+  if (n > BKT_CAP)
+  {
+    if (tid == 0) atomicOr(err, 4u);
+    return;
+  }
+  const Cand *__restrict__ row = rows + lo;
+  for (uint32_t k = tid; k < BKT_TABLE; k += BKT_THREADS) s_table[k] = BKT_EMPTY;
+  for (uint32_t s = tid; s < n; s += BKT_THREADS) s_hash[s] = row[s].qhash;
+  if (tid == 0) s_np = s_nlong = s_cnt = s_pos = 0;
+  __syncthreads();
+  for (uint32_t s = tid; s < n; s += BKT_THREADS)
+  {
+    const uint64_t h = s_hash[s];
+    uint32_t idx = ((uint32_t) (h ^ (h >> 29)) * 0x9E3779B1u) >> 19;
+    for (;;)
+    {
+      uint32_t cur = atomicCAS(&s_table[idx], BKT_EMPTY, s);
+      if (cur == BKT_EMPTY) break;
+      if (s_hash[cur & BKT_SLOT] == h)
+      {
+        for (;;)
+        {
+          const uint32_t state = cur >> 26;
+          if (state >= 2) break;
+          const uint32_t nw = state == 0 ? (cur | (s << 13) | (1u << 26)) : ((cur & 0x03FFFFFFu) | (2u << 26));
+          const uint32_t old = atomicCAS(&s_table[idx], cur, nw);
+          if (old == cur) break;
+          cur = old;
+        }
+        break;
+      }
+      idx = (idx + 1) & (BKT_TABLE - 1);
+    }
+  }
+  __syncthreads();
+  for (uint32_t k = tid; k < BKT_TABLE; k += BKT_THREADS)
+  {
+    const uint32_t e = s_table[k];
+    if (e == BKT_EMPTY) continue;
+    const uint32_t state = e >> 26;
+    if (state == 1)
+      s_plist[atomicAdd(&s_np, 1u)] = e & 0x03FFFFFFu;
+    else if (state == 2)
+    {
+      const uint32_t k2 = atomicAdd(&s_nlong, 1u);
+      if (k2 < BKT_LONG) s_long[k2] = (uint16_t) (e & BKT_SLOT);
+    }
+  }
+  __syncthreads();
+  const uint32_t nlong = s_nlong;
+  if (nlong > BKT_LONG)
+  {
+    if (tid == 0) atomicOr(err, 4u);
+    return;
+  }
+  uint32_t *recs = s_table;
+  uint16_t *list = (uint16_t *) (s_table + BKT_CAP);
+  uint16_t *order = list + BKT_CAP;
+  for (uint32_t l = 0; l < nlong; ++l)
+  {
+    const uint32_t owner = s_long[l];
+    const uint64_t h = s_hash[owner];
+    if (tid == 0) s_n = 0;
+    __syncthreads();
+    for (uint32_t s = tid; s < n; s += BKT_THREADS)
+      if (s_hash[s] == h)
+      {
+        const uint32_t k = atomicAdd(&s_n, 1u);
+        list[k] = (uint16_t) s;
+        recs[k] = (uint32_t) row[s].rec;
+        if (row[s].qcheck != row[owner].qcheck) atomicOr(err, 2u);
+      }
+    __syncthreads();
+    const uint32_t len = s_n;
+    for (uint32_t i = tid; i < len; i += BKT_THREADS)
+    {
+      const uint32_t ri = recs[i];
+      uint32_t rank = 0;
+      for (uint32_t j = 0; j < len; ++j) rank += (recs[j] < ri || (recs[j] == ri && j < i)) ? 1u : 0u;
+      order[rank] = list[i];
+    }
+    __syncthreads();
+    for (uint32_t k = tid; k < len / 2; k += BKT_THREADS) s_plist[atomicAdd(&s_np, 1u)] = (uint32_t) order[2 * k] | ((uint32_t) order[2 * k + 1] << 13);
+    __syncthreads();
+  }
+  const uint32_t np = s_np;
+  auto test = [&](uint32_t e, bk_pair &p) {
+    Cand b = row[e & BKT_SLOT], c = row[(e >> 13) & BKT_SLOT];
+    if (b.qcheck != c.qcheck) atomicOr(err, 2u);
+    if (c.rec < b.rec)
+    {
+      const Cand t = b;
+      b = c;
+      c = t;
+    }
+    return pair_of(b, c, w, tprefix, nt, p);
+  };
+  uint32_t mine = 0;
+  for (uint32_t i = tid; i < np; i += BKT_THREADS)
+  {
+    bk_pair p;
+    if (test(s_plist[i], p))
+    {
+      s_plist[i] |= 0x80000000u;
+      ++mine;
+    }
+  }
+  if (mine) atomicAdd(&s_cnt, mine);
+  __syncthreads();
+  if (tid == 0 && s_cnt) s_base = atomicAdd(counter, (unsigned long long) s_cnt);
+  __syncthreads();
+  for (uint32_t i = tid; i < np; i += BKT_THREADS)
+  {
+    const uint32_t e = s_plist[i];
+    if (!(e & 0x80000000u)) continue;
+    bk_pair p;
+    (void) test(e, p);
+    const unsigned long long slot = s_base + atomicAdd(&s_pos, 1u);
+    if (slot < cap)
+    {
+      out[slot] = p;
+      uint64_t gk = (uint64_t) (uint32_t) (p.p1_tid + 1) * (uint64_t) (nt + 1) + (uint64_t) (uint32_t) (p.p2_tid + 1);
+      okey[slot] = (gk << rbits) | p.rec;
+      oval[slot] = (uint32_t) slot;
+    }
+  }
+}
+
+__global__ __launch_bounds__(256) void k_group_flags(const uint64_t *__restrict__ key, uint64_t n, uint32_t *__restrict__ gflag, int rbits)
+{
+  uint64_t i = (uint64_t) blockIdx.x * blockDim.x + threadIdx.x;
+  if (i >= n) return;
   gflag[i] = (i == 0 || (key[i] >> rbits) != (key[i - 1] >> rbits)) ? 1u : 0u;
+}
+
+__global__ __launch_bounds__(256) void k_gather_pairs(const bk_pair *__restrict__ in, const uint32_t *__restrict__ perm, const uint32_t *__restrict__ gof,
+                                                      const uint64_t *__restrict__ gstart, const uint32_t *__restrict__ glex, uint64_t n, bk_pair *__restrict__ out)
+{
+  uint64_t i = (uint64_t) blockIdx.x * blockDim.x + threadIdx.x;
+  if (i >= n) return;
+  bk_pair p = in[perm[i]];
+  const uint32_t g = gof[i];
+  p.group = glex[g];
+  p.id = (uint32_t) (i - gstart[g]);
+  out[i] = p;
 }
 
 __global__ __launch_bounds__(256) void k_group_starts(const uint32_t *__restrict__ gflag, const uint32_t *__restrict__ gscan, const uint64_t *__restrict__ key, uint64_t n,
@@ -205,15 +413,6 @@
   if (i == n - 1) gstart[g + 1] = n;
 }
 
-__global__ __launch_bounds__(256) void k_assign_ids(bk_pair *__restrict__ pairs, const uint32_t *__restrict__ gof, const uint64_t *__restrict__ gstart,
-                                                    const uint32_t *__restrict__ glex, uint64_t n)
-{
-  uint64_t i = (uint64_t) blockIdx.x * blockDim.x + threadIdx.x;
-  if (i >= n) return;
-  uint32_t g = gof[i];
-  pairs[i].group = glex[g];
-  pairs[i].id = (uint32_t) (i - gstart[g]);
-}
 __global__ __launch_bounds__(256) void k_max_rec_cand(const Cand *__restrict__ c, uint64_t n, unsigned long long *__restrict__ out)
 {
   uint64_t i = (uint64_t) blockIdx.x * blockDim.x + threadIdx.x;
@@ -329,6 +528,15 @@
   while ((1ull << gbits) < (uint64_t) (nt + 1) * (uint64_t) (nt + 1) && gbits < 32) ++gbits;
   if (bits + gbits > 64) throw bk_error(BK_ERR_LIMIT, "pair sort key: chromosome-pair key and record index need more than 64 bits");
   b.rec_bits_eff = bits;
+  return bits;
+}
+
+static int bucket_bits(uint64_t n)
+{
+  if (const char *e = getenv("BK_JOIN_BUCKET_BITS"))
+    if (*e) return std::max(0, std::min(BKT_MAX_BITS, atoi(e)));
+  int bits = 0;
+  while (bits < BKT_MAX_BITS && (n >> bits) > BKT_CAP / 2) ++bits;
   return bits;
 }
 
@@ -345,9 +553,34 @@
   uint32_t *oval = b.oval.as<uint32_t>(cap);
   unsigned long long host[2] = {0, 0};
   static const int first_attempt = getenv("BK_JOIN_ATTEMPT") ? std::max(0, std::min(2, atoi(getenv("BK_JOIN_ATTEMPT")))) : 0;
+  static const bool debug = bk_debug("join");
+  const bool bucketed = b.rec_bits >= 0;
+  int form = 0, bits = 0;
+  unsigned long long largest = 0;
   for (int attempt = first_attempt; attempt < 3; ++attempt)
   {
-    if (n_cand)
+    form = attempt == 0 ? (bucketed ? 0 : 1) : attempt + 1;
+    if (n_cand && attempt == 0 && bucketed)
+    {
+      bits = bucket_bits(n_cand);
+      const uint32_t nbk = 1u << bits, nblk = std::max(1u, std::min(PART_BLOCKS, cdiv(n_cand, 16384)));
+      const uint64_t chunk = (n_cand + nblk - 1) / nblk;
+      uint32_t *hist = b.bucket_hist.as<uint32_t>((uint64_t) nbk * nblk + 1);
+      Cand *rows = b.bucket_rows.as<Cand>(n_cand);
+      hipLaunchKernelGGL(k_bucket_hist, dim3(nblk), dim3(PART_THREADS), (size_t) nbk * 4, st, cand, n_cand, chunk, bits, hist);
+      prims::exclusive_scan<uint32_t>(hist, hist, (uint64_t) nbk * nblk, b.scan_tmp, st);
+      hipLaunchKernelGGL(k_bucket_scatter, dim3(nblk), dim3(PART_THREADS), (size_t) nbk * 4, st, cand, n_cand, chunk, bits, (const uint32_t *) hist, rows);
+      hipLaunchKernelGGL(k_bucket_join, dim3(nbk), dim3(BKT_THREADS), 0, st, (const Cand *) rows, (const uint32_t *) hist, nblk, w, tprefix, nt, unsorted, okey, oval,
+                         (unsigned long long) cap, counter, err, rec_bits);
+      if (debug)
+      {
+        unsigned long long *m = b.maxrec.as<unsigned long long>(1);
+        HIP_CHECK(hipMemsetAsync(m, 0, 8, st));
+        hipLaunchKernelGGL(k_bucket_max, dim3(cdiv(nbk, 256)), dim3(256), 0, st, (const uint32_t *) hist, nblk, nbk, m);
+        HIP_CHECK(hipMemcpyAsync(&largest, m, 8, hipMemcpyDeviceToHost, st));
+      }
+    }
+    else if (n_cand)
     {
       uint64_t *key = b.key.as<uint64_t>(n_cand);
       uint32_t *val = b.val.as<uint32_t>(n_cand);
@@ -373,6 +606,9 @@
     }
     HIP_CHECK(hipMemcpyAsync(host, counter, 16, hipMemcpyDeviceToHost, st));
     HIP_CHECK(hipStreamSynchronize(st));
+    if (debug && form == 0)
+      fprintf(stderr, "[join] candidates %llu: B = %d, %u buckets, largest %llu rows (a workgroup holds %u)%s\n", (unsigned long long) n_cand, bits, 1u << bits, largest,
+              BKT_CAP, ((uint32_t) host[1] & 4u) ? ": a bucket does not fit" : "");
     if (attempt == 0 && ((uint32_t) host[1] & 4u))
     {
       HIP_CHECK(hipMemsetAsync(counter, 0, 16, st));
@@ -386,6 +622,9 @@
     }
     break;
   }
+  static const char *const form_name[4] = {"buckets", "upper-half sort", "whole-hash sort", "record order"};
+  if (debug) fprintf(stderr, "[join] candidates %llu -> %llu pairs by %s\n", (unsigned long long) n_cand, host[0], form_name[form]);
+  ++b.forms[form];
   if ((uint32_t) host[1] & 2u)
     throw bk_error(BK_ERR_COLLISION, "two different read names share one 64-bit name hash (their second hashes differ): the mate join would not be the reference's");
   if ((uint32_t) host[1] & 1u) throw bk_error(BK_ERR_HIP, "mate join: a run was refused although its candidates were sorted (internal error)");
@@ -393,7 +632,7 @@
   return host[0];
 }
 
-static void group_sorted(const bk_pair *unsorted, uint64_t *okey, uint32_t *oval, uint64_t np, int32_t nt, JoinBufs &b, hipStream_t st, JoinResult &res)
+static void group_index(const bk_pair *unsorted, uint64_t *okey, uint32_t *oval, uint64_t np, int32_t nt, JoinBufs &b, hipStream_t st, JoinResult &res)
 {
   res = JoinResult();
   res.n_pairs = np;
@@ -401,6 +640,8 @@
   uint32_t *gof = b.gof.as<uint32_t>(np + 1);
   res.pairs = pairs;
   res.gof = gof;
+  b.gather_src = unsorted;
+  b.gather_perm = nullptr;
   if (np == 0) return;
   int gbits = 1;
   while ((1ull << gbits) < (uint64_t) (nt + 1) * (uint64_t) (nt + 1) && gbits < 32) ++gbits;
@@ -408,9 +649,10 @@
   uint32_t *vs;
   const int rbits = b.rec_bits_eff;
   prims::radix_sort_pairs(okey, oval, np, 0, rbits + gbits, b.radix, st, &ks, &vs);
+  b.gather_perm = vs;
   uint32_t *gflag = b.gflag.as<uint32_t>(np + 1);
   uint32_t *gscan = b.gscan.as<uint32_t>(np + 1);
-  hipLaunchKernelGGL(k_gather_pairs, dim3(cdiv(np, 256)), dim3(256), 0, st, unsorted, vs, ks, np, pairs, gflag, rbits);
+  hipLaunchKernelGGL(k_group_flags, dim3(cdiv(np, 256)), dim3(256), 0, st, (const uint64_t *) ks, np, gflag, rbits);
   prims::exclusive_scan<uint32_t>(gflag, gscan, np, b.scan_tmp, st);
   uint32_t ng = 0;
   HIP_CHECK(hipMemcpyAsync(&ng, gscan + np, 4, hipMemcpyDeviceToHost, st));
@@ -426,7 +668,7 @@
 void join_candidates(const Cand *cand, uint64_t n_cand, double w, const uint32_t *tprefix, int32_t nt, JoinBufs &b, hipStream_t st, JoinResult &res)
 {
   const uint64_t np = join_raw_pairs(cand, n_cand, w, tprefix, nt, b, st);
-  group_sorted(b.unsorted.get<bk_pair>(), b.okey.get<uint64_t>(), b.oval.get<uint32_t>(), np, nt, b, st, res);
+  group_index(b.unsorted.get<bk_pair>(), b.okey.get<uint64_t>(), b.oval.get<uint32_t>(), np, nt, b, st, res);
 }
 
 void group_pairs(const bk_pair *raw, uint64_t np, int32_t nt, JoinBufs &b, hipStream_t st, JoinResult &res)
@@ -436,7 +678,7 @@
   uint32_t *oval = b.oval.as<uint32_t>(np + 1);
   const int rec_bits = effective_rec_bits(raw, np, k_max_rec_pair, nt, b, st);
   if (np) hipLaunchKernelGGL(k_pair_keys, dim3(cdiv(np, 256)), dim3(256), 0, st, raw, np, nt, okey, oval, rec_bits);
-  group_sorted(raw, okey, oval, np, nt, b, st, res);
+  group_index(raw, okey, oval, np, nt, b, st, res);
 }
 
 Cand *route_candidates(const Cand *cand, uint64_t n, uint32_t world, JoinBufs &b, hipStream_t st, std::vector<uint64_t> &counts)
@@ -477,8 +719,11 @@
   return out;
 }
 
-void join_assign_ids(JoinResult &res, const uint32_t *glex_dev, hipStream_t st)
+void join_gather_pairs(JoinResult &res, const uint32_t *glex_dev, JoinBufs &b, hipStream_t st)
 {
   if (res.n_pairs == 0) return;
-  hipLaunchKernelGGL(k_assign_ids, dim3(cdiv(res.n_pairs, 256)), dim3(256), 0, st, res.pairs, res.gof, res.gstart, glex_dev, res.n_pairs);
-}
+  hipLaunchKernelGGL(k_gather_pairs, dim3(cdiv(res.n_pairs, 256)), dim3(256), 0, st, b.gather_src, b.gather_perm, (const uint32_t *) res.gof, (const uint64_t *) res.gstart, glex_dev,
+                     res.n_pairs, res.pairs);
+  b.gather_src = nullptr;
+  b.gather_perm = nullptr;
+}
diff --git a/include/breakid_hip.h b/include/breakid_hip.h
--- a/include/breakid_hip.h
+++ b/include/breakid_hip.h
@@ -206,6 +206,8 @@
 
 int bk_sort_forms(bk_ctx *ctx, uint64_t out[3]);
 
+int bk_join_forms(bk_ctx *ctx, uint64_t out[4]);
+
 int bk_debug_ahc(bk_ctx *ctx, const uint32_t *x, const uint32_t *y, uint32_t n, double w, uint32_t *idx_out, int32_t *cluster_out, uint32_t *n_out);
 
 int bk_debug_points(bk_ctx *ctx, int mode, const uint32_t *x, const uint32_t *y, uint32_t n, double w, uint32_t *idx_out, int32_t *cluster_out, uint32_t *n_out);
```

New measurement: 11980, median of 6. 1.02x the previous value.
